# pyannote/pyannote-video

Hardware: AMD Instinct MI355X
Metric: frames/sec end-to-end detect->embed->cluster, 1080p@25fps (higher is better)
Workload: dtype f32 (detector scores, embedder) / f64 (tracker, clustering) / u8 frames; an f16 screening pass with a proven error bound decides which windows the detector's exact f32 chain is evaluated for -- results identical to dense f32 scoring (`dense_scoring`)

## Files before the change

### include/pvface.h

```cpp
#ifndef PVFACE_H
#define PVFACE_H
#include <stdint.h>
#include <stddef.h>

#ifdef __cplusplus
extern "C" {
#endif

typedef uint64_t pvf_handle;
typedef struct { int32_t left, top, right, bottom; } pvf_rect_i32;

const char* pvf_last_error(void);
int32_t pvf_version(void);
int32_t pvf_device_count(int32_t* n);
int32_t pvf_ctx_create(int32_t device, pvf_handle* ctx);
int32_t pvf_ctx_create_prio(int32_t device, int32_t priority_class, pvf_handle* ctx);
int32_t pvf_ctx_destroy(pvf_handle ctx);
int32_t pvf_sync(pvf_handle ctx);

int32_t pvf_load_detector(pvf_handle ctx, const char* path);
int32_t pvf_load_shape_predictor(pvf_handle ctx, const char* path);
int32_t pvf_load_embedder(pvf_handle ctx, const char* path);
int32_t pvf_model_tensor(const char* path, int32_t kind, const char* name, void* out, int64_t cap_bytes, int64_t* nbytes);
int32_t pvf_set_tracker_tables(pvf_handle ctx, const double* mask64, const double* mask_scale, const double* tw64,
                               const double* tw32, double alpha_pow_m16, double ln_alpha);

int32_t pvf_frame_upload(pvf_handle ctx, const uint8_t* rgb, int32_t h, int32_t w, int64_t row_stride_bytes, pvf_handle* frame);
int32_t pvf_frame_wrap_device(pvf_handle ctx, const void* dev_rgb, int32_t h, int32_t w, pvf_handle* frame);
int32_t pvf_frame_release(pvf_handle ctx, pvf_handle frame);
int32_t pvf_frame_release_many(pvf_handle ctx, const pvf_handle* frames, int32_t n);
int32_t pvf_frame_pool_trim(pvf_handle ctx, int64_t keep_bytes, int64_t* pooled_bytes);
int32_t pvf_mem_info(pvf_handle ctx, int64_t* free_bytes, int64_t* total_bytes);
int32_t pvf_frame_device_ptr(pvf_handle ctx, pvf_handle frame, const void** dev_rgb);

int32_t pvf_ingest_create(pvf_handle ctx, int32_t h, int32_t w, int32_t depth, pvf_handle* ring);
int32_t pvf_ingest_destroy(pvf_handle ctx, pvf_handle ring);
int32_t pvf_ingest_acquire(pvf_handle ctx, pvf_handle ring, int32_t* slot, uint8_t** host_rgb);
int32_t pvf_ingest_submit(pvf_handle ctx, pvf_handle ring, int32_t slot, pvf_handle* frame);
int32_t pvf_ingest_wait(pvf_handle ctx, pvf_handle ring);
#define PVF_YUV_BT709 1
#define PVF_YUV_FULL_RANGE 2
int32_t pvf_ingest_create_yuv(pvf_handle ctx, int32_t h, int32_t w, int32_t depth, int32_t layout, int32_t flags, pvf_handle* ring);
int32_t pvf_frame_from_yuv(pvf_handle ctx, const uint8_t* y, int64_t y_pitch, const uint8_t* u, const uint8_t* v, int64_t c_pitch,
                           int32_t c_step, int32_t h, int32_t w, int32_t layout, int32_t flags, pvf_handle* frame);
int32_t pvf_frame_resize(pvf_handle ctx, pvf_handle frame, int32_t out_w, int32_t out_h, pvf_handle* out);

#define PVF_PRIM_RECT 0
#define PVF_PRIM_LINE 1
#define PVF_PRIM_TEXT 2
#define PVF_RENDER_MAX_PRIMS 4096
#define PVF_RENDER_MAX_RUN 64
#define PVF_RENDER_MAX_TEXT (1 << 20)
#define PVF_RENDER_MAX_SCALE 64
#define PVF_RENDER_MAX_BATCH 1024
typedef struct { int32_t type, a, b, c, d; uint32_t colour; int32_t scale, reserved; } pvf_prim;
int32_t pvf_render_batch(pvf_handle ctx, const pvf_handle* frames, int32_t n, int32_t out_w, int32_t out_h, int32_t flags,
                         const int32_t* start, const pvf_prim* prims, const uint8_t* text, int64_t text_bytes,
                         uint8_t* out, int32_t out_on_device);
int32_t pvf_egress_create(pvf_handle ctx, int32_t out_w, int32_t out_h, int32_t depth, int32_t flags, pvf_handle* ring);
int32_t pvf_egress_destroy(pvf_handle ctx, pvf_handle ring);
int32_t pvf_egress_submit(pvf_handle ctx, pvf_handle ring, pvf_handle frame, const pvf_prim* prims, int32_t n_prims,
                          const uint8_t* text, int64_t text_bytes, int32_t* slot);
int32_t pvf_egress_wait(pvf_handle ctx, pvf_handle ring, int32_t slot, const uint8_t** host_planes);
int32_t pvf_egress_release(pvf_handle ctx, pvf_handle ring, int32_t slot);
int32_t pvf_debug_render_rgb(pvf_handle ctx, pvf_handle frame, int32_t out_w, int32_t out_h, const pvf_prim* prims, int32_t n_prims,
                             const uint8_t* text, int64_t text_bytes, uint8_t* rgb);

int32_t pvf_detect(pvf_handle ctx, pvf_handle frame, int32_t upsample, double adjust_threshold,
                   pvf_rect_i32* out, float* scores, int32_t cap, int32_t* n);
int32_t pvf_detect_batch(pvf_handle ctx, const pvf_handle* frames, int32_t n_frames, int32_t upsample,
                         double adjust_threshold, pvf_rect_i32* out, float* scores, int32_t* counts,
                         int32_t cap_per_frame);
int32_t pvf_detect_many(pvf_handle ctx, const pvf_handle* frames, int32_t n_frames, int32_t batch, int32_t upsample,
                        double adjust_threshold, pvf_rect_i32* out, float* scores, int32_t* counts, int32_t cap);

int32_t pvf_detector_screening(pvf_handle ctx, int32_t on, int32_t list_cap);
int32_t pvf_detector_screening_stats(pvf_handle ctx, int64_t* batches, int64_t* listed, int64_t* retries, double* bounds, double* pipe_err);

int32_t pvf_embedder_split(pvf_handle ctx, int32_t on);
int32_t pvf_embedder_split_stats(pvf_handle ctx, int64_t* faces, int64_t* reruns, double* pipe_err);

int32_t pvf_tracker_create(pvf_handle ctx, pvf_handle* trk);
int32_t pvf_tracker_create_many(pvf_handle ctx, int32_t n, pvf_handle* trks);
int32_t pvf_tracker_destroy_many(pvf_handle ctx, const pvf_handle* trks, int32_t n);
int32_t pvf_tracker_clone_many(pvf_handle ctx, const pvf_handle* src, int32_t n, pvf_handle* dst);
int32_t pvf_tracker_destroy(pvf_handle ctx, pvf_handle trk);
int32_t pvf_tracker_start(pvf_handle ctx, pvf_handle trk, pvf_handle frame, const double box[4]);
int32_t pvf_tracker_update(pvf_handle ctx, pvf_handle trk, pvf_handle frame, double* psr);
int32_t pvf_tracker_position(pvf_handle ctx, pvf_handle trk, double box[4]);
int32_t pvf_tracker_start_many(pvf_handle ctx, const pvf_handle* trks, const pvf_handle* frames,
                               const double* boxes , int32_t n);
int32_t pvf_tracker_update_many(pvf_handle ctx, const pvf_handle* trks, const pvf_handle* frames, int32_t n,
                                double* psr , double* boxes_out );
int32_t pvf_tracker_update_many_deferred(pvf_handle ctx, const pvf_handle* trks, const pvf_handle* frames, int32_t n,
                                         double* psr, double* boxes_out);
int32_t pvf_tracker_commit_many(pvf_handle ctx, const pvf_handle* trks, const pvf_handle* frames, int32_t n);

int32_t pvf_overlap_matrix(const double* a, int32_t na, const double* b, int32_t nb, double ratio, double* out);
int32_t pvf_associate(const double* trackers, int32_t n_trackers, const double* detections, int32_t n_detections,
                      double min_overlap_ratio, int32_t* det_of_tracker);
int32_t pvf_munkres(const double* cost, int32_t n, int32_t* row_to_col);

int32_t pvf_landmarks(pvf_handle ctx, const pvf_handle* frames, const pvf_rect_i32* boxes, int32_t n,
                      int32_t* pts );
int32_t pvf_embed(pvf_handle ctx, const pvf_handle* frames, const int32_t* pts , int32_t n,
                  float* out );
int32_t pvf_landmarks_embed(pvf_handle ctx, const pvf_handle* frames, const pvf_rect_i32* boxes, int32_t n,
                            int32_t* pts , float* out );
int32_t pvf_embed_chips(pvf_handle ctx, const uint8_t* chips, int32_t n, float* out );
int32_t pvf_face_chips(pvf_handle ctx, const pvf_handle* frames, const int32_t* pts, int32_t n, uint8_t* chips );

int32_t pvf_pair_mean_dist(pvf_handle ctx, const double* X, int32_t N, int32_t dim, const int32_t* row_start,
                           int32_t T, double* D);
int32_t pvf_pair_mean_dist_metric(pvf_handle ctx, const double* X, int32_t N, int32_t dim, const int32_t* row_start,
                                  int32_t T, int32_t metric, double* D);
int32_t pvf_lane_create(int32_t n_frames, const int32_t* det_counts , const double* det_boxes ,
                        int32_t direction, double min_confidence, double min_overlap_ratio, int32_t deferring, pvf_handle* lane);
int32_t pvf_lane_destroy(pvf_handle lane);
int32_t pvf_lane_feed_plan(pvf_handle lane, int32_t p0, int32_t n_p, const uint8_t* has_update, const uint64_t* handles, const double* psr,
                           const double* pos);
int32_t pvf_lane_advance(pvf_handle lane, const double* reply_psr, const double* reply_pos, int32_t n_reply, int32_t* request,
                         uint64_t* req_handles, int32_t* req_frames, int32_t cap, int32_t* n_req, int32_t* plan_from);
int32_t pvf_lane_take_dead(pvf_handle lane, uint64_t* out, int32_t cap, int32_t* n);
int32_t pvf_lane_edges(pvf_handle lane, int32_t* n_edges, int32_t* u_frame_kind, double* u_box, int32_t* v_frame_kind, double* v_box,
                       double* conf, int32_t cap);
int32_t pvf_shot_tracks(pvf_handle lane_forward, pvf_handle lane_backward, const double* times, int32_t n_frames, double max_gap,
                        int32_t* rows, int32_t cap, int32_t* n_rows, int32_t* track_start, int32_t track_cap, int32_t* n_tracks);
int32_t pvf_track_rows(const int32_t* boxes, int64_t n, int32_t det_width, int32_t det_height, int32_t width, int32_t height,
                       double* file_box, int32_t* pixel_box);
int32_t pvf_round_decimals(const double* in, int64_t n, int32_t decimals, double* out);

int32_t pvf_pair_mean_dist_rows(pvf_handle ctx, const double* X, int32_t N, int32_t dim, const int32_t* row_start, int32_t T,
                                int32_t track0, int32_t track1, double* D);
int32_t pvf_pair_upper_rows(pvf_handle ctx, const double* X, int32_t N, int32_t dim, const int32_t* row_start, int32_t T,
                            int32_t track0, int32_t track1, double* D);
int32_t pvf_cluster_dist(pvf_handle ctx, const double* D, const int32_t* row_start, int32_t T, double threshold,
                         int32_t* labels, double* merge_log, int32_t* n_merges);
int32_t pvf_cluster_upper(pvf_handle ctx, const double* U, int32_t on_device, const int32_t* row_start, int32_t T, double threshold,
                          int32_t* labels, double* merge_log, int32_t* n_merges);
int32_t pvf_cluster_tracks(pvf_handle ctx, const double* X, int32_t N, int32_t dim, const int32_t* row_start,
                           int32_t T, double threshold, int32_t* labels, double* merge_log, int32_t* n_merges);
int32_t pvf_cluster_tracks_f32(pvf_handle ctx, const float* emb, int64_t row_stride_bytes, int32_t n_src, int32_t emb_on_device,
                               const int32_t* order, int32_t N, int32_t decimals, const int32_t* row_start, int32_t T, int32_t metric,
                               double threshold, int32_t* labels, double* merge_log, int32_t* n_merges);
int32_t pvf_pair_upper_rows_f32(pvf_handle ctx, const float* emb, int64_t row_stride_bytes, int32_t n_src, int32_t emb_on_device,
                                const int32_t* order, int32_t N, int32_t decimals, const int32_t* row_start, int32_t T,
                                int32_t track0, int32_t track1, double* rows_out, int32_t out_on_device);

int32_t pvf_format_rows(const double* t, const int64_t* identifier, const double* values, int64_t n_rows, int32_t n_cols,
                        int32_t decimals, char* out, int64_t cap, int64_t* written);

int32_t pvf_round_rows(const float* x, int64_t n, int32_t decimals, double* out);

int32_t pvf_parse_rows(const char* text, int64_t len, double* out, int64_t cap, int64_t* n_rows, int32_t* n_cols);

int32_t pvf_prof_enable(pvf_handle ctx, int32_t on);
int32_t pvf_prof_reset(pvf_handle ctx);
int32_t pvf_prof_get(pvf_handle ctx, const char* family, double* total_ms, int64_t* launches);

int32_t pvf_debug_pyramid_level(pvf_handle ctx, pvf_handle frame, int32_t upsample, int32_t level,
                                uint8_t* out, int32_t* h, int32_t* w);
int32_t pvf_debug_pyramid_batch(pvf_handle ctx, const pvf_handle* frames, int32_t n, int32_t upsample);
int32_t pvf_debug_level_features(pvf_handle ctx, pvf_handle frame, int32_t upsample, int32_t level,
                                 float* out, int32_t* fh, int32_t* fw);
int32_t pvf_debug_level_plan(pvf_handle ctx, pvf_handle frame, int32_t upsample, int32_t level, int32_t* out8);
int32_t pvf_debug_fhog(pvf_handle ctx, const uint8_t* img, int32_t h, int32_t w, int32_t cell, int32_t pad_r,
                       int32_t pad_c, float* out, int32_t* fh, int32_t* fw);
int32_t pvf_debug_detect_raw(pvf_handle ctx, pvf_handle frame, int32_t upsample, double adjust, float* scores,
                             int32_t* meta , int32_t cap, int32_t* n);
int32_t pvf_debug_detect_raw_many(pvf_handle ctx, const pvf_handle* frames, int32_t n_frames, int32_t batch, int32_t upsample,
                                  double adjust, int32_t* counts, int32_t* rows, int64_t cap, int64_t* total);
int32_t pvf_debug_extract_chip(pvf_handle ctx, pvf_handle frame, const double rect[4], double cs, double sn,
                               int32_t rows, int32_t cols, uint8_t* out);
int32_t pvf_debug_tracker_state(pvf_handle ctx, pvf_handle trk, double* F, double* A, double* B);
int32_t pvf_debug_tracker_scale_state(pvf_handle ctx, pvf_handle trk, double* As, double* Bs);
int32_t pvf_debug_embed_stage(pvf_handle ctx, const uint8_t* chips, int32_t n, int32_t split, int32_t stage, float* out, int32_t dims[3],
                              int32_t* flags);
int32_t pvf_debug_conv(pvf_handle ctx, const int32_t geom[18], const float* in, const float* w, const float* bias, const float* gamma,
                       const float* beta, const float* skip, int32_t split, int32_t force_generic, float* out, int32_t* flags);
int32_t pvf_debug_embed_head(pvf_handle ctx, const float* x, int32_t n, int32_t hw, float* out);

int32_t pvf_shot_dfd(pvf_handle ctx, const pvf_handle* frames, int32_t n, int32_t width, int32_t height, const float* tables,
                     double* dfd, uint8_t* gray_out, float* flow_out);

int32_t pvf_orb_extract(pvf_handle ctx, const pvf_handle* frames, int32_t n, int32_t width, int32_t height, int32_t cap,
                        int32_t* counts, float* keypoints, uint8_t* descriptors);
int32_t pvf_orb_match_counts(pvf_handle ctx, const uint8_t* descriptors, const int32_t* rows, int32_t n_sets, int32_t cap,
                             const int32_t* pairs, int64_t n_pairs, int32_t* counts);

#ifdef __cplusplus
}
#endif
#endif
```

### pyannote-video_amd/csrc/api.hip

```cpp
#include "pvf_internal.h"
#include <algorithm>
#include <cmath>
#include <cstdlib>
#include <string>
#include <thread>

#define API_BEGIN try {
#define API_END                                                        \
    return 0;                                                          \
    }                                                                  \
    catch (const std::exception& e) { pvf_set_error(e.what()); return -1; } \
    catch (...) { pvf_set_error("unknown error"); return -2; }

#define ENTER(c, h)                                                \
    Ctx* c = pvf_ctx(h);                                           \
    std::lock_guard<std::recursive_mutex> _api_lock(c->api_mu);    \
    HIP_CHECK(hipSetDevice(c->device))
#define ENTER_DET(c, h)                                            \
    Ctx* c = pvf_ctx(h);                                           \
    std::lock_guard<std::recursive_mutex> _det_lock(c->det_mu);    \
    HIP_CHECK(hipSetDevice(c->device))
#define ENTER_BOTH(c, h)                                           \
    Ctx* c = pvf_ctx(h);                                           \
    std::lock_guard<std::recursive_mutex> _det_lock(c->det_mu);    \
// ... 47 lines not shown
extern "C" int32_t pvf_embedder_split(pvf_handle h, int32_t on)
{
    API_BEGIN
    ENTER(c, h);
    c->emb_split = on != 0;
    API_END
}

extern "C" int32_t pvf_embedder_split_stats(pvf_handle h, int64_t* faces, int64_t* reruns, double* pipe_err)
{
    API_BEGIN
    ENTER(c, h);
    if (faces) *faces = c->emb_split_faces;
    if (reruns) *reruns = c->emb_reruns;
    if (pipe_err) *pipe_err = c->emb_pipe_err;
    API_END
}

extern "C" int32_t pvf_detect_batch(pvf_handle h, const pvf_handle* frames, int32_t n_frames, int32_t upsample, double adjust,
                                    pvf_rect_i32* out, float* scores, int32_t* counts, int32_t cap)
{
    API_BEGIN
    ENTER_DET(c, h);
    PVF_REQUIRE(n_frames > 0 && frames && out && counts && cap > 0, "pvf_detect_batch: bad arguments");
    PVF_REQUIRE(upsample >= 0 && upsample <= 2, "pvf_detect_batch: upsample must be 0..2");
    std::vector<Frame> fr(n_frames);
    for (int i = 0; i < n_frames; ++i) fr[i] = c->frame(frames[i]);
    std::vector<std::vector<RawDet>> raw;
    with_candidate_room(c, [&]() { det_run_batch(c, fr, upsample, adjust, raw); });
    std::vector<RawDet> kept;
    for (int i = 0; i < n_frames; ++i) {
        det_nms(c->det, raw[i], kept);
        const int n = std::min<int>((int)kept.size(), cap);
        counts[i] = n;
        for (int k = 0; k < n; ++k) {
            out[(size_t)i * cap + k] = pvf_rect_i32{kept[k].l, kept[k].t, kept[k].rr, kept[k].b};
            if (scores) scores[(size_t)i * cap + k] = kept[k].score;
        }
    }
    API_END
}

extern "C" int32_t pvf_detect_many(pvf_handle h, const pvf_handle* frames, int32_t n_frames, int32_t batch, int32_t upsample, double adjust,
                                   pvf_rect_i32* out, float* scores, int32_t* counts, int32_t cap)
{
    API_BEGIN
    ENTER_DET(c, h);
    PVF_REQUIRE(n_frames > 0 && batch > 0 && frames && out && counts && cap > 0, "pvf_detect_many: bad arguments");
    PVF_REQUIRE(upsample >= 0 && upsample <= 2, "pvf_detect_many: upsample must be 0..2");
    std::vector<Frame> fr(n_frames);
    for (int i = 0; i < n_frames; ++i) fr[i] = c->frame(frames[i]);
    std::vector<std::vector<RawDet>> kept_all;
    with_candidate_room(c, [&]() { det_run_many(c, fr, batch, upsample, adjust, kept_all, true); });
    for (int i = 0; i < n_frames; ++i) {
        const std::vector<RawDet>& kept = kept_all[i];
        const int n = std::min<int>((int)kept.size(), cap);
        counts[i] = n;
        for (int k = 0; k < n; ++k) {
            out[(size_t)i * cap + k] = pvf_rect_i32{kept[k].l, kept[k].t, kept[k].rr, kept[k].b};
            if (scores) scores[(size_t)i * cap + k] = kept[k].score;
        }
    }
    API_END
}

extern "C" int32_t pvf_detect(pvf_handle h, pvf_handle frame, int32_t upsample, double adjust, pvf_rect_i32* out, float* scores,
                              int32_t cap, int32_t* n)
{
    int32_t cnt = 0;
    const int32_t rc = pvf_detect_batch(h, &frame, 1, upsample, adjust, out, scores, &cnt, cap);
    if (rc == 0 && n) *n = cnt;
    return rc;
}

extern "C" int32_t pvf_debug_detect_raw(pvf_handle h, pvf_handle frame, int32_t upsample, double adjust, float* scores, int32_t* meta,
                                        int32_t cap, int32_t* n)
{
    API_BEGIN
    ENTER_DET(c, h);
    std::vector<Frame> fr{c->frame(frame)};
    std::vector<std::vector<RawDet>> raw;
    with_candidate_room(c, [&]() { det_run_batch(c, fr, upsample, adjust, raw); });
    const int k = std::min<int>((int)raw[0].size(), cap);
    *n = (int)raw[0].size();
    for (int i = 0; i < k; ++i) {
        const RawDet& d = raw[0][i];
        scores[i] = d.score;
        int32_t* m = meta + (size_t)i * 8;
        m[0] = d.filter; m[1] = d.level; m[2] = d.r; m[3] = d.c; m[4] = d.l; m[5] = d.t; m[6] = d.rr; m[7] = d.b;
    }
    API_END
}

extern "C" int32_t pvf_debug_detect_raw_many(pvf_handle h, const pvf_handle* frames, int32_t n_frames, int32_t batch, int32_t upsample, double adjust,
                                             int32_t* counts, int32_t* rows, int64_t cap, int64_t* total)
{
    API_BEGIN
    ENTER_DET(c, h);
    PVF_REQUIRE(n_frames > 0 && batch > 0 && frames && counts && total && (rows || cap == 0), "pvf_debug_detect_raw_many: bad arguments");
    PVF_REQUIRE(upsample >= 0 && upsample <= 2, "pvf_debug_detect_raw_many: upsample must be 0..2");
    std::vector<Frame> fr(n_frames);
    for (int i = 0; i < n_frames; ++i) fr[i] = c->frame(frames[i]);
    std::vector<std::vector<RawDet>> raw;
    with_candidate_room(c, [&]() { det_run_many(c, fr, batch, upsample, adjust, raw, false); });
    int64_t k = 0;
    for (int i = 0; i < n_frames; ++i) {
        counts[i] = (int32_t)raw[i].size();
        for (const RawDet& d : raw[i]) {
            if (k < cap) {
                int32_t* m = rows + (size_t)k * 5;
                m[0] = d.level; m[1] = d.filter; m[2] = d.r; m[3] = d.c;
                memcpy(&m[4], &d.score, 4);
            }
            ++k;
        }
    }
    *total = k;
    API_END
}

extern "C" int32_t pvf_debug_pyramid_level(pvf_handle h, pvf_handle frame, int32_t upsample, int32_t level, uint8_t* out, int32_t* oh,
                                           int32_t* ow)
{
    API_BEGIN
    ENTER_DET(c, h);
    std::vector<uint8_t> buf;
    int hh = 0, ww = 0;
    det_pyramid_level(c, c->frame(frame), upsample, level, out ? &buf : nullptr, &hh, &ww);
    *oh = hh; *ow = ww;
    if (out) memcpy(out, buf.data(), buf.size());
    API_END
}

extern "C" int32_t pvf_debug_pyramid_batch(pvf_handle h, const pvf_handle* frames, int32_t n, int32_t upsample)
{
    API_BEGIN
    ENTER_DET(c, h);
    PVF_REQUIRE(frames && n > 0, "pvf_debug_pyramid_batch: bad arguments");
    std::vector<Frame> fr;
    for (int i = 0; i < n; ++i) fr.push_back(c->frame(frames[i]));
    det_pyramid_batch(c, fr, upsample);
    API_END
}

extern "C" int32_t pvf_debug_level_features(pvf_handle h, pvf_handle frame, int32_t upsample, int32_t level, float* out, int32_t* fh, int32_t* fw)
{
    API_BEGIN
    ENTER_DET(c, h);
    std::vector<float> buf;
    int a = 0, b = 0;
    det_level_features(c, c->frame(frame), upsample, level, out ? &buf : nullptr, &a, &b);
    *fh = a; *fw = b;
    if (out) memcpy(out, buf.data(), buf.size() * sizeof(float));
    API_END
}

extern "C" int32_t pvf_debug_level_plan(pvf_handle h, pvf_handle frame, int32_t upsample, int32_t level, int32_t* out8)
{
    API_BEGIN
    ENTER_DET(c, h);
    PVF_REQUIRE(out8 != nullptr, "pvf_debug_level_plan: out8 is NULL");
    det_level_plan(c, c->frame(frame), upsample, level, out8);
    API_END
}

extern "C" int32_t pvf_debug_fhog(pvf_handle h, const uint8_t* img, int32_t ih, int32_t iw, int32_t cell, int32_t pad_r, int32_t pad_c,
                                  float* out, int32_t* fh, int32_t* fw)
{
    API_BEGIN
    ENTER_BOTH(c, h);
    int a = 0, b = 0;
    if (!out) { fhog_dims(ih, iw, cell, pad_r, pad_c, &a, &b); *fh = a; *fw = b; return 0; }
    std::vector<float> buf;
    fhog_debug(c, img, ih, iw, cell, pad_r, pad_c, buf, &a, &b);
    *fh = a; *fw = b;
    memcpy(out, buf.data(), buf.size() * sizeof(float));
    API_END
}

static pvf_handle tracker_new(Ctx* c)
{
    std::unique_ptr<Tracker> t(new Tracker());
    const uint64_t id = c->next_id++;
    c->trackers[id] = std::move(t);
    return id;
}

extern "C" int32_t pvf_tracker_create(pvf_handle h, pvf_handle* trk)
{
    API_BEGIN
    ENTER(c, h);
    *trk = tracker_new(c);
    API_END
}

extern "C" int32_t pvf_tracker_create_many(pvf_handle h, int32_t n, pvf_handle* trks)
{
    API_BEGIN
    ENTER(c, h);
    PVF_REQUIRE(n >= 0, "negative count");
    for (int i = 0; i < n; ++i) trks[i] = tracker_new(c);
    API_END
}

extern "C" int32_t pvf_tracker_clone_many(pvf_handle h, const pvf_handle* src, int32_t n, pvf_handle* dst)
{
    API_BEGIN
    ENTER(c, h);
    PVF_REQUIRE(n >= 0, "negative count");
    std::vector<Tracker*> s(n), d(n);
    for (int i = 0; i < n; ++i) s[i] = &c->tracker(src[i]);
    for (int i = 0; i < n; ++i) { dst[i] = tracker_new(c); d[i] = &c->tracker(dst[i]); }
    dsst_clone_many(c, s, d);
    API_END
}

static const size_t TRACKER_POOL_KEEP = 4096;
static void pool_tracker_state(Ctx* c, Tracker& t)
{
    double* d_state = t.d_state;
    t.d_state = nullptr;
    if (t.share) {
        int* sh = t.share;
        t.share = nullptr;
        if (--*sh > 0) return;
        delete sh;
    }
    if (!d_state) return;
    if (c->tracker_pool.size() < TRACKER_POOL_KEEP) { c->tracker_pool.push_back(d_state); return; }
    HIP_CHECK(hipStreamSynchronize(c->stream));
    HIP_CHECK(hipFree(d_state));
}

extern "C" int32_t pvf_tracker_destroy_many(pvf_handle h, const pvf_handle* trks, int32_t n)
{
    API_BEGIN
    ENTER(c, h);
    for (int i = 0; i < n; ++i) {
        auto it = c->trackers.find(trks[i]);
        PVF_REQUIRE(it != c->trackers.end(), "unknown tracker handle");
        pool_tracker_state(c, *it->second);
        c->trackers.erase(it);
    }
    API_END
}

extern "C" int32_t pvf_tracker_destroy(pvf_handle h, pvf_handle trk)
{
    API_BEGIN
    ENTER(c, h);
    auto it = c->trackers.find(trk);
    PVF_REQUIRE(it != c->trackers.end(), "unknown tracker handle");
    pool_tracker_state(c, *it->second);
    c->trackers.erase(it);
    API_END
}
extern "C" int32_t pvf_tracker_start_many(pvf_handle h, const pvf_handle* trks, const pvf_handle* frames, const double* boxes, int32_t n)
{
    API_BEGIN
    ENTER(c, h);
    std::vector<Tracker*> t(n);
    std::vector<Frame> f(n);
    PVF_REQUIRE(n >= 0 && (n == 0 || (trks && frames && boxes)), "tracker.start_track: bad arguments");
    for (int i = 0; i < n; ++i) {
        const double* b = boxes + 4 * (size_t)i;
        PVF_REQUIRE(std::isfinite(b[0]) && std::isfinite(b[1]) && std::isfinite(b[2]) && std::isfinite(b[3]),
                    "tracker.start_track: box with a non-finite coordinate");
        PVF_REQUIRE(b[2] - b[0] != 0.0 && b[3] - b[1] != 0.0, "tracker.start_track: box of zero width or height");
    }
    for (int i = 0; i < n; ++i) { t[i] = &c->tracker(trks[i]); f[i] = c->frame(frames[i]); }
    dsst_start_many(c, t, f, boxes);
    API_END
}
extern "C" int32_t pvf_tracker_update_many(pvf_handle h, const pvf_handle* trks, const pvf_handle* frames, int32_t n, double* psr,
                                           double* boxes_out)
{
    API_BEGIN
    ENTER(c, h);
    std::vector<Tracker*> t(n);
    std::vector<Frame> f(n);
    for (int i = 0; i < n; ++i) { t[i] = &c->tracker(trks[i]); f[i] = c->frame(frames[i]); }
    dsst_update_many(c, t, f, psr, boxes_out);
    API_END
}
extern "C" int32_t pvf_tracker_start(pvf_handle h, pvf_handle trk, pvf_handle frame, const double box[4])
{
    return pvf_tracker_start_many(h, &trk, &frame, box, 1);
}
extern "C" int32_t pvf_tracker_update_many_deferred(pvf_handle h, const pvf_handle* trks, const pvf_handle* frames, int32_t n, double* psr,
                                                    double* boxes_out)
{
    API_BEGIN
    ENTER(c, h);
    std::vector<Tracker*> t(n);
    std::vector<Frame> f(n);
    for (int i = 0; i < n; ++i) { t[i] = &c->tracker(trks[i]); f[i] = c->frame(frames[i]); }
    dsst_update_many(c, t, f, psr, boxes_out, 1);
    API_END
}

extern "C" int32_t pvf_tracker_commit_many(pvf_handle h, const pvf_handle* trks, const pvf_handle* frames, int32_t n)
{
    API_BEGIN
    ENTER(c, h);
    std::vector<Tracker*> t(n);
    std::vector<Frame> f(n);
// ... 689 lines not shown
```

### pyannote-video_amd/csrc/ctx.hip

```cpp
#include "pvf_internal.h"
#include "detect_ml.h"
#include <cmath>
#include <fstream>
#include <mutex>
#include <dlfcn.h>

static thread_local std::string g_err;
void pvf_set_error(const char* msg) { g_err = msg ? msg : ""; }
extern "C" const char* pvf_last_error(void) { return g_err.c_str(); }

static std::mutex g_ctx_mu;
static std::unordered_map<uint64_t, std::unique_ptr<Ctx>> g_ctxs;
static uint64_t g_next_ctx = 0x1000;

Ctx* pvf_ctx(pvf_handle h)
{
    std::lock_guard<std::mutex> lk(g_ctx_mu);
    auto it = g_ctxs.find(h);
    if (it == g_ctxs.end()) throw PvfError("unknown context handle");
    return it->second.get();
}

std::map<std::string, Tensor> pvf_read_container(const char* path)
{
// ... 80 lines not shown
        d.d_bmfma4 = upload<float>(b4.data(), b4.size());
    }
    screen_prepare_model(d, w.f32());
    d.loaded = true;
}

static void load_shape(Ctx* c, const char* path)
{
    auto m = pvf_read_model(path, 1);
    const int32_t* q = need(m, "sp.meta").i32();
    ShapeModel& s = c->shape;
    s.n_cascades = q[0]; s.n_trees = q[1]; s.n_parts = q[2]; s.n_pix = q[3]; s.depth = q[4];
    PVF_REQUIRE(s.n_parts == 68, "shape predictor: 68 parts expected");
    PVF_REQUIRE(s.depth >= 1 && s.depth <= 6, "shape predictor: tree depth 1..6");
    PVF_REQUIRE(s.n_pix >= 1 && s.n_pix <= 1024, "shape predictor: 1..1024 feature pixels per cascade");
    PVF_REQUIRE(s.n_cascades >= 1 && s.n_trees >= 1, "shape predictor: no cascades / trees");
    {
        const size_t splits = (size_t)s.n_cascades * s.n_trees * (((size_t)1 << s.depth) - 1), leaves = (size_t)s.n_cascades * s.n_trees * ((size_t)1 << s.depth);
        PVF_REQUIRE(need(m, "sp.initial_shape").numel() == 136 && need(m, "sp.anchor_idx").numel() == (size_t)s.n_cascades * s.n_pix &&
                    need(m, "sp.deltas").numel() == (size_t)s.n_cascades * s.n_pix * 2 && need(m, "sp.split_idx1").numel() == splits &&
                    need(m, "sp.split_idx2").numel() == splits && need(m, "sp.split_thresh").numel() == splits &&
                    need(m, "sp.leaves").numel() == leaves * 136, "shape predictor: tensor sizes do not match sp.meta");
        const int32_t* a = need(m, "sp.anchor_idx").i32();
        for (size_t k = 0; k < (size_t)s.n_cascades * s.n_pix; ++k) PVF_REQUIRE(a[k] >= 0 && a[k] < s.n_parts, "shape predictor: anchor index out of range");
        const int32_t* i1 = need(m, "sp.split_idx1").i32();
        const int32_t* i2 = need(m, "sp.split_idx2").i32();
        for (size_t k = 0; k < splits; ++k)
            PVF_REQUIRE(i1[k] >= 0 && i1[k] < s.n_pix && i2[k] >= 0 && i2[k] < s.n_pix, "shape predictor: split feature index out of range");
    }
    auto up_f = [&](const char* k) { const Tensor& t = need(m, k); return upload<float>(t.f32(), t.numel()); };
    auto up_i = [&](const char* k) { const Tensor& t = need(m, k); return upload<int32_t>(t.i32(), t.numel()); };
    s.d_initial = up_f("sp.initial_shape");
    s.d_anchor = up_i("sp.anchor_idx");
    s.d_deltas = up_f("sp.deltas");
    s.d_idx1 = up_i("sp.split_idx1");
    s.d_idx2 = up_i("sp.split_idx2");
    s.d_thresh = up_f("sp.split_thresh");
    s.d_leaves = up_f("sp.leaves");
    s.loaded = true;
}

static const int UNITS[14][3] = {{32, 32, 0}, {32, 32, 0}, {32, 32, 0}, {32, 64, 1}, {64, 64, 0}, {64, 64, 0}, {64, 64, 0},
                                 {64, 128, 1}, {128, 128, 0}, {128, 128, 0}, {128, 256, 1}, {256, 256, 0}, {256, 256, 0}, {256, 256, 1}};

static void load_embedder(Ctx* c, const char* path)
{
    auto m = pvf_read_model(path, 2);
    EmbedModel& e = c->emb;
    e.chip_size = need(m, "emb.meta").i32()[0];
    e.chip_padding = need(m, "emb.padding").f64()[0];
    PVF_REQUIRE(e.chip_size == 150, "embedder: 150x150 chips expected");
    const Tensor& ms = need(m, "emb.mean_shape");
    PVF_REQUIRE(ms.numel() == 102, "emb.mean_shape must be 51x2");
    e.mean_shape.assign(ms.f32(), ms.f32() + 102);
    const Tensor& blob = need(m, "emb.blob");
    const float* p = blob.f32();
    const float* end = p + blob.numel();
    for (ConvLayer& L : e.convs) {
        if (L.d_frag) { (void)hipFree(L.d_frag); L.d_frag = nullptr; }
        if (L.d_wsplit) { (void)hipFree(L.d_wsplit); L.d_wsplit = nullptr; }
    }
    e.convs.clear();
    if (e.d_stem) { (void)hipFree(e.d_stem); e.d_stem = nullptr; }
    auto add_conv = [&](int cin, int cout, int k, int stride, int pad) {
        ConvLayer L{cin, cout, k, stride, pad, nullptr, nullptr, nullptr, nullptr, nullptr};
        const size_t nw = (size_t)cout * cin * k * k;
        PVF_REQUIRE(p + nw + 3 * (size_t)cout <= end, "emb.blob too short");
        conv_layer_upload(L, p, p + nw, p + nw + cout, p + nw + 2 * (size_t)cout);
        p += nw + 3 * (size_t)cout;
        e.convs.push_back(L);
    };
    add_conv(3, 32, 7, 2, 0);
    for (int u = 0; u < 14; ++u) {
        const int cin = UNITS[u][0], n = UNITS[u][1], down = UNITS[u][2];
        add_conv(cin, n, 3, down ? 2 : 1, down ? 0 : 1);
        add_conv(n, n, 3, 1, 1);
    }
    PVF_REQUIRE(p + 256 * 128 == end, "emb.blob size mismatch");
    e.d_fc = upload<float>(p, 256 * 128);
    e.loaded = true;
}

namespace {
struct Roctx {
    int (*push)(const char*) = nullptr;
    int (*pop)() = nullptr;
    Roctx()
    {
        const char* e = getenv("PVF_ROCTX");
        if (!e || strcmp(e, "1") != 0) return;
        void* h = dlopen("librocprofiler-sdk-roctx.so", RTLD_NOW | RTLD_GLOBAL);
        if (!h) h = dlopen("librocprofiler-sdk-roctx.so.1", RTLD_NOW | RTLD_GLOBAL);
        if (!h) h = dlopen("libroctx64.so", RTLD_NOW | RTLD_GLOBAL);
        if (!h) h = dlopen("libroctx64.so.4", RTLD_NOW | RTLD_GLOBAL);
        if (!h) return;
        push = reinterpret_cast<int (*)(const char*)>(dlsym(h, "roctxRangePushA"));
        pop = reinterpret_cast<int (*)()>(dlsym(h, "roctxRangePop"));
        if (!push || !pop) push = nullptr, pop = nullptr;
    }
};
const Roctx& roctx() { static const Roctx r; return r; }
}

ProfScope::ProfScope(Ctx* ctx, const char* family, hipStream_t on) : c(ctx), s(on ? on : ctx->stream)
{
    if (roctx().push) { roctx().push(family); ranged = true; }
    if (!c->prof_on) return;
    {
        std::lock_guard<std::mutex> lk(c->prof_mu);
        f = &c->prof[family];
        auto get = [&]() {
            hipEvent_t e;
            if (!c->event_pool.empty()) { e = c->event_pool.back(); c->event_pool.pop_back(); }
            else HIP_CHECK(hipEventCreate(&e));
            return e;
        };
        a = get(); b = get();
    }
    HIP_CHECK(hipEventRecord(a, s));
}
ProfScope::~ProfScope()
{
    if (ranged) roctx().pop();
    if (!f) return;
    (void)hipEventRecord(b, s);
    std::lock_guard<std::mutex> lk(c->prof_mu);
    f->pending.emplace_back(a, b);
    f->launches += 1;
}

static void prof_drain(Ctx* c)
{
    HIP_CHECK(hipStreamSynchronize(c->stream));
    HIP_CHECK(hipStreamSynchronize(c->det_stream));
    std::lock_guard<std::mutex> lk(c->prof_mu);
    for (auto& kv : c->prof) {
        for (auto& pr : kv.second.pending) {
            float ms = 0;
            if (hipEventElapsedTime(&ms, pr.first, pr.second) == hipSuccess) kv.second.total_ms += ms;
            c->event_pool.push_back(pr.first);
            c->event_pool.push_back(pr.second);
        }
        kv.second.pending.clear();
    }
}

#define API_BEGIN try {
#define API_END                                                        \
    return 0;                                                          \
    }                                                                  \
    catch (const std::exception& e) { pvf_set_error(e.what()); return -1; } \
    catch (...) { pvf_set_error("unknown error"); return -2; }

extern "C" int32_t pvf_version(void) { return 500; }

extern "C" int32_t pvf_device_count(int32_t* n)
{
    API_BEGIN
    int k = 0;
    hipError_t e = hipGetDeviceCount(&k);
    if (e != hipSuccess) k = 0;
    *n = k;
    API_END
}

extern "C" int32_t pvf_ctx_create_prio(int32_t device, int32_t priority_class, pvf_handle* out)
{
    API_BEGIN
    int k = 0;
    if (hipGetDeviceCount(&k) != hipSuccess || k <= 0) throw PvfError("no HIP device visible: libpvface has no CPU fallback");
    PVF_REQUIRE(device >= 0 && device < k, "device index out of range");
    HIP_CHECK(hipSetDevice(device));
    hipDeviceProp_t prop;
    HIP_CHECK(hipGetDeviceProperties(&prop, device));
    if (strncmp(prop.gcnArchName, "gfx950", 6) != 0)
        throw PvfError(std::string("libpvface is built for gfx950 (MI355X) only; device is ") + prop.gcnArchName);
    std::unique_ptr<Ctx> c(new Ctx());
    c->device = device;
    c->n_cu = prop.multiProcessorCount;
    {
        int lo = 0, hi = 0;
        HIP_CHECK(hipDeviceGetStreamPriorityRange(&lo, &hi));
        int prio = priority_class < 0 ? lo : hi;
        if (const char* e = getenv("PVF_MAIN_STREAM_PRIO")) prio = (strcmp(e, "low") == 0) ? lo : hi;
        HIP_CHECK(hipStreamCreateWithPriority(&c->stream, hipStreamNonBlocking, priority_class == 2 ? lo : prio));
        HIP_CHECK(hipStreamCreateWithPriority(&c->det_stream, hipStreamNonBlocking, priority_class == 2 ? hi : lo));
    }
    if (const char* e = getenv("PVF_DETECTOR_SCREENING")) c->det_screen = atoi(e) != 0;
    if (const char* e = getenv("PVF_EMBEDDER_SPLIT")) c->emb_split = atoi(e) != 0;
    std::lock_guard<std::mutex> lk(g_ctx_mu);
    uint64_t id = g_next_ctx++;
    g_ctxs[id] = std::move(c);
    *out = id;
    API_END
}

extern "C" int32_t pvf_ctx_create(int32_t device, pvf_handle* out) { return pvf_ctx_create_prio(device, 0, out); }

extern "C" int32_t pvf_ctx_destroy(pvf_handle h)
{
    API_BEGIN
    Ctx* c = pvf_ctx(h);
    HIP_CHECK(hipSetDevice(c->device));
    (void)hipStreamSynchronize(c->stream);
    (void)hipStreamSynchronize(c->det_stream);
    for (auto& kv : c->frames) if (kv.second.owned) (void)hipFree((void*)kv.second.d);
    for (auto& kv : c->trackers) {
        Tracker& t = *kv.second;
        if (t.share) { if (--*t.share > 0) continue; delete t.share; t.share = nullptr; }
        if (t.d_state) (void)hipFree(t.d_state);
    }
    for (auto p : c->tracker_pool) (void)hipFree(p);
    for (int k = 0; k < 2; ++k) if (c->det_ev[k]) (void)hipEventDestroy(c->det_ev[k]);
    ml_plans_free(c);
    ingest_free_all(c);
    render_free_all(c);
    for (auto& kv : c->frame_pool) for (auto q : kv.second) {
        if (q.free_after) (void)hipEventDestroy(q.free_after);
        if (q.free_after_det) (void)hipEventDestroy(q.free_after_det);
        (void)hipFree(q.p);
    }
    if (c->d_orient_lut) (void)hipFree(c->d_orient_lut);
    if (c->d_wrap_lut) (void)hipFree(c->d_wrap_lut);
    (void)hipStreamDestroy(c->stream);
    (void)hipStreamDestroy(c->det_stream);
    std::lock_guard<std::mutex> lk(g_ctx_mu);
    g_ctxs.erase(h);
    API_END
}

extern "C" int32_t pvf_sync(pvf_handle h)
{
    API_BEGIN
    Ctx* c = pvf_ctx(h);
    std::lock_guard<std::recursive_mutex> det_lock(c->det_mu);
    std::lock_guard<std::recursive_mutex> api_lock(c->api_mu);
    HIP_CHECK(hipStreamSynchronize(c->det_stream));
    HIP_CHECK(hipStreamSynchronize(c->stream));
    API_END
}

extern "C" int32_t pvf_load_detector(pvf_handle h, const char* path)
{
    API_BEGIN
    Ctx* c = pvf_ctx(h);
    std::lock_guard<std::recursive_mutex> det_lock(c->det_mu);
    std::lock_guard<std::recursive_mutex> api_lock(c->api_mu);
    HIP_CHECK(hipSetDevice(c->device));
    PVF_REQUIRE(path != nullptr, "pvf_load_detector: path is NULL (the Python layer passes the packaged default)");
    load_detector(c, path);
    API_END
}
extern "C" int32_t pvf_load_shape_predictor(pvf_handle h, const char* path)
{
    API_BEGIN
    Ctx* c = pvf_ctx(h);
    std::lock_guard<std::recursive_mutex> api_lock(c->api_mu);
    HIP_CHECK(hipSetDevice(c->device));
    PVF_REQUIRE(path != nullptr, "path is NULL");
    load_shape(c, path);
    API_END
}
extern "C" int32_t pvf_load_embedder(pvf_handle h, const char* path)
{
    API_BEGIN
    Ctx* c = pvf_ctx(h);
    std::lock_guard<std::recursive_mutex> api_lock(c->api_mu);
    HIP_CHECK(hipSetDevice(c->device));
    PVF_REQUIRE(path != nullptr, "path is NULL");
    load_embedder(c, path);
    API_END
}

extern "C" int32_t pvf_model_tensor(const char* path, int32_t kind, const char* name, void* out, int64_t cap_bytes, int64_t* nbytes)
{
    API_BEGIN
    PVF_REQUIRE(path && name && nbytes, "pvf_model_tensor: bad arguments");
    auto m = pvf_read_model(path, kind);
    const Tensor& t = need(m, name);
    *nbytes = (int64_t)t.data.size();
    if (out) {
        PVF_REQUIRE(cap_bytes >= (int64_t)t.data.size(), "pvf_model_tensor: buffer too small");
        memcpy(out, t.data.data(), t.data.size());
    }
    API_END
}

extern "C" int32_t pvf_set_tracker_tables(pvf_handle h, const double* mask64, const double* mask_scale, const double* tw64,
                                          const double* tw32, double alpha_pow_m16, double ln_alpha)
{
    API_BEGIN
    Ctx* c = pvf_ctx(h);
    std::lock_guard<std::recursive_mutex> api_lock(c->api_mu);
    HIP_CHECK(hipSetDevice(c->device));
    TrackerTables& t = c->ttab;
    if (!t.d_mask64) {
        HIP_CHECK(hipMalloc((void**)&t.d_mask64, 64 * 64 * 8));
        HIP_CHECK(hipMalloc((void**)&t.d_mask_scale, 32 * 8));
        HIP_CHECK(hipMalloc((void**)&t.d_tw64, 64 * 8));
        HIP_CHECK(hipMalloc((void**)&t.d_tw32, 32 * 8));
    }
    HIP_CHECK(hipMemcpy(t.d_mask64, mask64, 64 * 64 * 8, hipMemcpyHostToDevice));
    HIP_CHECK(hipMemcpy(t.d_mask_scale, mask_scale, 32 * 8, hipMemcpyHostToDevice));
    HIP_CHECK(hipMemcpy(t.d_tw64, tw64, 64 * 8, hipMemcpyHostToDevice));
    HIP_CHECK(hipMemcpy(t.d_tw32, tw32, 32 * 8, hipMemcpyHostToDevice));
    t.alpha_pow_m16 = alpha_pow_m16; t.ln_alpha = ln_alpha;
    t.set = true;
// ... 154 lines not shown
```

### pyannote-video_amd/csrc/detect.hip

```cpp
#include "detect_ml.h"
#include <algorithm>
#include <thread>
#include <cmath>
#include <cstdlib>

#define RESIZE_MAXS 22
struct RowTab { int32_t top, bottom; double tb, tb1, pad; };
struct ColTab { int32_t left, pad; double lr, lr1, pad2; };

template <int RS, int NSTRIP>
__global__ void __launch_bounds__(256) resize_rows_k(const uint8_t* const* __restrict__ in_ptrs, const uint8_t* __restrict__ in_base,
                                                     size_t in_stride, int in_rb, int ih, int iw, uint8_t* __restrict__ out,
                                                     size_t out_stride, int out_rb, int oh, int ow,
                                                     const RowTab* __restrict__ rows, const ColTab* __restrict__ cols)
{
    constexpr int MAXS = (RS == 16) ? RESIZE_MAXS : (RS * 5) / 4 + 3;
    __shared__ uint32_t s_rows[4][MAXS][64];
    __shared__ uint32_t s_out[4][64];
    const int lane = threadIdx.x & 63;
    const int wave = __builtin_amdgcn_readfirstlane(threadIdx.x >> 6);
    const int c0 = blockIdx.x * 256 + wave * 64;
    const int b = blockIdx.z;
    if (c0 >= ow) return;
    const int c = min(c0 + lane, ow - 1);
// ... 164 lines not shown
}

static void pyramid_up_dims(int ih, int iw, int* oh, int* ow)
{
    const double right = ((iw - 1) + 1.25) * 2.0;
    const double bottom = ((ih - 1) + 0.75) * 2.0;
    *ow = (int)std::floor(right + 0.5) + 1;
    *oh = (int)std::floor(bottom + 0.5) + 1;
}


static inline long iround(double v) { return (long)std::floor(v + 0.5); }
static void rect_down6(long r[4]) { const double ratio = (6 - 1.0) / 6; for (int i = 0; i < 4; ++i) r[i] = iround((r[i] - 0.3) * ratio + 0.3); }
static void rect_up6(long r[4]) { const double ratio = 6 / (6 - 1.0); for (int i = 0; i < 4; ++i) r[i] = iround((r[i] - 0.3) * ratio + 0.3); }
static void rect_down2i(long r[4])
{
    r[0] = iround(r[0] / 2.0 - 1.25); r[1] = iround(r[1] / 2.0 - 0.75);
    r[2] = iround(r[2] / 2.0 - 1.25); r[3] = iround(r[3] / 2.0 - 0.75);
}
static int detector_levels(int h, int w, const DetectorModel& m)
{
    long r[4] = {0, 0, w - 1, h - 1};
    int levels = 0;
    do { rect_down6(r); ++levels; } while ((r[2] - r[0] + 1) >= m.min_w && (r[3] - r[1] + 1) >= m.min_h && levels < m.max_levels);
    return levels;
}
static void fhog_to_image(long px, long py, int cell, int pad_r, int pad_c, long* ox, long* oy)
{
    long x = (px + 1 - (pad_c - 1) / 2) * cell + 1;
    long y = (py + 1 - (pad_r - 1) / 2) * cell + 1;
    x += (x >= 0) ? cell / 2 : -(cell / 2);
    y += (y >= 0) ? cell / 2 : -(cell / 2);
    *ox = x; *oy = y;
}

struct LevelDims { int h, w; };
static std::vector<LevelDims> level_schedule(int h, int w, int upsample, const DetectorModel& m, std::vector<LevelDims>* ups)
{
    int ch = h, cw = w;
    for (int u = 0; u < upsample; ++u) {
        int nh, nw;
        pyramid_up_dims(ch, cw, &nh, &nw);
        ch = nh; cw = nw;
        if (ups) ups->push_back({ch, cw});
    }
    const int levels = detector_levels(ch, cw, m);
    std::vector<LevelDims> out;
    out.push_back({ch, cw});
    for (int l = 1; l < levels; ++l) { ch = (5 * ch) / 6; cw = (5 * cw) / 6; out.push_back({ch, cw}); }
    return out;
}

static void upload_frame_ptrs(Ctx* c, const std::vector<Frame>& frames, const uint8_t*** d_ptrs)
{
    DevBuf& d = c->s_fptr[c->det_slot & 1];
    HostBuf& h = c->h_fptr[c->det_slot & 1];
    d.ensure(frames.size() * sizeof(void*));
    h.ensure(frames.size() * sizeof(void*));
    const uint8_t** hp = h.as<const uint8_t*>();
    for (size_t i = 0; i < frames.size(); ++i) hp[i] = frames[i].d;
    HIP_CHECK(hipMemcpyAsync(d.p, hp, frames.size() * sizeof(void*), hipMemcpyHostToDevice, c->det_stream));
    *d_ptrs = d.as<const uint8_t*>();
}


__device__ __forceinline__ int ml_block(const MlStarts& st) { return (int)blockIdx.x; }
static inline int ml_grid(int total) { return total; }

__device__ __forceinline__ int ml_level(const MlStarts& st, int g)
{
    int l = 0;
    while (l + 1 < st.nl && g >= st.b0[l + 1]) ++l;
    return l;
}

#define FUSED_OUT 61
__device__ __forceinline__ uint32_t from_next_lane(uint32_t v) { return (uint32_t)__builtin_amdgcn_update_dpp(0, (int)v, 0x130, 0xf, 0xf, true); }
__device__ __forceinline__ uint32_t from_prev_lane(uint32_t v) { return (uint32_t)__builtin_amdgcn_update_dpp(0, (int)v, 0x138, 0xf, 0xf, true); }

#define FS_PAIRS 4
#define FS_COLS 65
#define FS_SLOT_DW (8 * FS_COLS * 2)
#define FS_BINS_DW (2 * 18 * 64)
#define FS_FLAG_DW (4 * 64)
#define FS_LDS_BYTES (FS_PAIRS * (FS_BINS_DW + 2 * FS_SLOT_DW + FS_FLAG_DW) * 4)
static_assert(FS_COLS * 8 == 520, "the ring's column pitch is written into the instruction strings below");
typedef __attribute__((address_space(3))) uint32_t* lds_u32;
__device__ __forceinline__ uint32_t lds_addr(const void* p) { return (uint32_t)(uintptr_t)(lds_u32)p; }

__device__ __forceinline__ void ring_write(uint32_t data_at, uint32_t flag_at, const u32x2* v, uint32_t row1)
{
    asm volatile("ds_write_b64 %0, %2\n\tds_write_b64 %0, %3 offset:520\n\tds_write_b64 %0, %4 offset:1040\n\tds_write_b64 %0, %5 offset:1560\n\t"
                 "ds_write_b64 %0, %6 offset:2080\n\tds_write_b64 %0, %7 offset:2600\n\tds_write_b64 %0, %8 offset:3120\n\t"
                 "ds_write_b64 %0, %9 offset:3640\n\tds_write_b32 %1, %10"
                 :: "v"(data_at), "v"(flag_at), "v"(v[0]), "v"(v[1]), "v"(v[2]), "v"(v[3]), "v"(v[4]), "v"(v[5]), "v"(v[6]), "v"(v[7]), "v"(row1) : "memory");
}
__device__ __forceinline__ uint32_t ring_read(uint32_t data_at, uint32_t flag_at, u32x2* own, u32x2* nb)
{
    uint32_t ready;
    asm volatile("ds_read_b32 %0, %18\n\t"
                 "ds_read_b64 %1, %17\n\tds_read_b64 %9, %17 offset:8\n\tds_read_b64 %2, %17 offset:520\n\tds_read_b64 %10, %17 offset:528\n\t"
                 "ds_read_b64 %3, %17 offset:1040\n\tds_read_b64 %11, %17 offset:1048\n\tds_read_b64 %4, %17 offset:1560\n\tds_read_b64 %12, %17 offset:1568\n\t"
                 "ds_read_b64 %5, %17 offset:2080\n\tds_read_b64 %13, %17 offset:2088\n\tds_read_b64 %6, %17 offset:2600\n\tds_read_b64 %14, %17 offset:2608\n\t"
                 "ds_read_b64 %7, %17 offset:3120\n\tds_read_b64 %15, %17 offset:3128\n\tds_read_b64 %8, %17 offset:3640\n\tds_read_b64 %16, %17 offset:3648\n\t"
                 "s_waitcnt lgkmcnt(0)"
                 : "=&v"(ready), "=&v"(own[0]), "=&v"(own[1]), "=&v"(own[2]), "=&v"(own[3]), "=&v"(own[4]), "=&v"(own[5]), "=&v"(own[6]), "=&v"(own[7]),
                   "=&v"(nb[0]), "=&v"(nb[1]), "=&v"(nb[2]), "=&v"(nb[3]), "=&v"(nb[4]), "=&v"(nb[5]), "=&v"(nb[6]), "=&v"(nb[7])
                 : "v"(data_at), "v"(flag_at) : "memory");
    return ready;
}
__device__ __forceinline__ void flag_write(uint32_t flag_at, uint32_t v)
{
    asm volatile("ds_write_b32 %0, %1" :: "v"(flag_at), "v"(v) : "memory");
}

template <int A, int B> __device__ __forceinline__ uint32_t sub_into_upper(uint32_t acc, uint32_t x, uint32_t y);
#define PVF_SUBW1(A, B)                                                                                                                  \
    template <> __device__ __forceinline__ uint32_t sub_into_upper<A, B>(uint32_t acc, uint32_t x, uint32_t y)                           \
    {                                                                                                                                    \
        asm("v_sub_u32_sdwa %0, %1, %2 dst_sel:WORD_1 dst_unused:UNUSED_PRESERVE src0_sel:BYTE_" #A " src1_sel:BYTE_" #B "\n\ts_nop 0"   \
            : "+v"(acc) : "v"(x), "v"(y));                                                                                               \
        return acc;                                                                                                                      \
    }
PVF_SUBW1(0, 0) PVF_SUBW1(1, 1) PVF_SUBW1(2, 2) PVF_SUBW1(3, 3)
#undef PVF_SUBW1
typedef short s16x2 __attribute__((ext_vector_type(2)));

template <int P>
__device__ __forceinline__ u32x2 split_grad_px(const uint32_t* up, const uint32_t* ce, const uint32_t* dn, const __amdgpu_buffer_rsrc_t& lut_rs,
                                               bool valid)
{
    uint32_t pk[3];
    int cv[3];
#define PVF_CH(K)                                                                                                                         \
    {                                                                                                                                     \
        constexpr int IU = 4 + 3 * P + K, IL = 1 + 3 * P + K, IR = 7 + 3 * P + K;                                                         \
        const uint32_t cx = ((ce[IR >> 2] >> (8 * (IR & 3))) & 0xffu) - ((ce[IL >> 2] >> (8 * (IL & 3))) & 0xffu);                          \
        pk[K] = sub_into_upper<(IU & 3), (IU & 3)>(cx, dn[IU >> 2], up[IU >> 2]);                                                          \
        const s16x2 v = __builtin_bit_cast(s16x2, pk[K]);                                                                                 \
        cv[K] = __builtin_amdgcn_sdot2(v, v, 0, false);                                                                                   \
    }
    PVF_CH(0) PVF_CH(1) PVF_CH(2)
#undef PVF_CH
    const int bv = max(cv[0], max(cv[1], cv[2]));
    const uint32_t pb = (cv[0] == bv) ? pk[0] : ((cv[1] == bv) ? pk[1] : pk[2]);
    const uint32_t off = (pb & 7u) | ((pb >> 13) & 0xff8u) | ((pb << 9) & 0x3f000u);
    u32x2 r;
    r.y = (uint32_t)__builtin_amdgcn_raw_buffer_load_b8(lut_rs, off, 0, 0);
    const float m = sqrt_exact_small((float)bv);
    r.x = valid ? __float_as_uint(m) : 0u;
    return r;
}

__global__ void __launch_bounds__(512) __attribute__((amdgpu_waves_per_eu(4, 4)))
fhog_split_ml_k(MlStarts st, const LvDesc* __restrict__ lv, int B, const uint8_t* __restrict__ img_base, float* __restrict__ feat_base,
                const uint8_t* __restrict__ lutw, int oy, int ox)
{
    constexpr int RSRC_FLAGS = 0x00020000;
    extern __shared__ __attribute__((aligned(16))) uint32_t fs_lds[];
    const int lane = threadIdx.x & 63;
    const int wave = __builtin_amdgcn_readfirstlane(threadIdx.x >> 6);
    const int pair = wave & 3, role = wave >> 2;
    for (int i = threadIdx.x; i < FS_PAIRS * (2 * FS_SLOT_DW + FS_FLAG_DW); i += 512) fs_lds[FS_PAIRS * FS_BINS_DW + i] = 0u;
    __syncthreads();
    const int g = ml_block(st);
    if (g >= st.b0[st.nl]) return;
    const int l = ml_level(st, g);
    const LvDesc d = lv[l];
    const int task = (g - st.b0[l]) * FS_PAIRS + pair;
    if (task >= d.fused_tasks) return;
    const int sx = task % d.strips;
    const int t2 = task / d.strips;
    const int cy = t2 % d.chunks;
    const int b = t2 / d.chunks;
    const int y0 = cy * d.chunk_rows;
    const int R = min(d.chunk_rows, d.hog_nr - y0);
    const int g_first = y0 + 1, g_last = y0 + R + 3;
    const int y_begin = 8 * g_first - 12;
    const uint32_t ring_at = lds_addr(fs_lds + FS_PAIRS * FS_BINS_DW + pair * 2 * FS_SLOT_DW) + 8u * lane;
    uint32_t* const flags = fs_lds + FS_PAIRS * (FS_BINS_DW + 2 * FS_SLOT_DW) + pair * FS_FLAG_DW + lane;
    const uint32_t flag_at = lds_addr(flags);

    if (role == 0) {
        const int hx = FUSED_OUT * sx + 1 + lane;
        const int x_first = 8 * hx - 12;
        const uint8_t* im = img_base + d.img_off + (size_t)b * d.img_stride;
        const int rb = d.rb;
        unsigned xmask = 0;
#pragma unroll
        for (int p = 0; p < 8; ++p) if (x_first + p >= 1 && x_first + p < d.visible_nc) xmask |= 1u << p;
        const bool strip_inside = __builtin_amdgcn_ballot_w64(xmask != 0xffu) == 0;
        const int voff = 3 * x_first - 4, voff2 = voff + 16;
        const __amdgpu_buffer_rsrc_t lut_rs = __builtin_amdgcn_make_buffer_rsrc((void*)lutw, 0, 1 << 18, RSRC_FLAGS);
        uint32_t rw[4][8];
        auto load_row = [&](int yi, uint32_t* dst) {
            const int bytes = (yi >= 0 && yi < d.h) ? rb : 0;
            const int yc = min(max(yi, 0), d.h - 1);
            const __amdgpu_buffer_rsrc_t rs = __builtin_amdgcn_make_buffer_rsrc((void*)(im + (size_t)yc * rb), 0, bytes, RSRC_FLAGS);
            const u32x4 a = __builtin_amdgcn_raw_buffer_load_b128(rs, voff, 0, 0);
            const u32x4 c = __builtin_amdgcn_raw_buffer_load_b128(rs, voff2, 0, 0);
            dst[0] = a.x; dst[1] = a.y; dst[2] = a.z; dst[3] = a.w; dst[4] = c.x; dst[5] = c.y; dst[6] = c.z; dst[7] = c.w;
        };
#pragma unroll
        for (int q = 0; q < 4; ++q) load_row(y_begin - 1 + q, rw[q]);
        const int nrows = 8 * (g_last - g_first + 1);
        for (int k0 = 0; k0 < nrows; k0 += 4) {
#pragma unroll
            for (int i = 0; i < 4; ++i) {
                const int k = k0 + i, y = y_begin + k;
                const uint32_t* up = rw[i & 3];
                const uint32_t* ce = rw[(i + 1) & 3];
                const uint32_t* dn = rw[(i + 2) & 3];
                const int freed = (int)__hip_atomic_load(flags + 128 + 64 * (i & 1), __ATOMIC_RELAXED, __HIP_MEMORY_SCOPE_WORKGROUP);
                const bool ok = (y >= 1 && y < d.visible_nr);
                u32x2 mb[8];
                if (strip_inside && ok) {
                    mb[0] = split_grad_px<0>(up, ce, dn, lut_rs, true); mb[1] = split_grad_px<1>(up, ce, dn, lut_rs, true);
                    mb[2] = split_grad_px<2>(up, ce, dn, lut_rs, true); mb[3] = split_grad_px<3>(up, ce, dn, lut_rs, true);
                    mb[4] = split_grad_px<4>(up, ce, dn, lut_rs, true); mb[5] = split_grad_px<5>(up, ce, dn, lut_rs, true);
                    mb[6] = split_grad_px<6>(up, ce, dn, lut_rs, true); mb[7] = split_grad_px<7>(up, ce, dn, lut_rs, true);
                } else {
                    mb[0] = split_grad_px<0>(up, ce, dn, lut_rs, ok && (xmask & 1u));
                    mb[1] = split_grad_px<1>(up, ce, dn, lut_rs, ok && (xmask & 2u));
                    mb[2] = split_grad_px<2>(up, ce, dn, lut_rs, ok && (xmask & 4u));
                    mb[3] = split_grad_px<3>(up, ce, dn, lut_rs, ok && (xmask & 8u));
                    mb[4] = split_grad_px<4>(up, ce, dn, lut_rs, ok && (xmask & 16u));
                    mb[5] = split_grad_px<5>(up, ce, dn, lut_rs, ok && (xmask & 32u));
                    mb[6] = split_grad_px<6>(up, ce, dn, lut_rs, ok && (xmask & 64u));
                    mb[7] = split_grad_px<7>(up, ce, dn, lut_rs, ok && (xmask & 128u));
                }
                load_row(y + 3, rw[i & 3]);
                int fr = freed;
                while (fr < k - 1) {
                    __builtin_amdgcn_s_sleep(1);
                    fr = (int)__hip_atomic_load(flags + 128 + 64 * (i & 1), __ATOMIC_RELAXED, __HIP_MEMORY_SCOPE_WORKGROUP);
                }
                ring_write(ring_at + (i & 1) * 4 * FS_SLOT_DW, flag_at + 256 * (i & 1), mb, (uint32_t)(k + 1));
            }
        }
        return;
    }

    float* accE = reinterpret_cast<float*>(fs_lds) + pair * FS_BINS_DW + lane;
    float* accO = accE + 18 * 64;
#pragma unroll
    for (int k = 0; k < 18; ++k) { accE[64 * k] = 0.0f; accO[64 * k] = 0.0f; }
    float hprev[18];
    float e0 = 0.f, e1 = 0.f, e2 = 0.f;
#pragma unroll
    for (int k = 0; k < 18; ++k) hprev[k] = 0.f;
    int krow = 0;
    auto band = [&](int gb, float* accU, float* accL) {
#pragma unroll
        for (int i = 0; i < 8; ++i) {
            u32x2 own[8], nb[8];
            for (;;) {
                const int ready = (int)ring_read(ring_at + (i & 1) * 4 * FS_SLOT_DW, flag_at + 256 * (i & 1), own, nb);
                if (__builtin_amdgcn_readfirstlane(ready) > krow) break;
                __builtin_amdgcn_s_sleep(1);
            }
            ++krow;
            flag_write(flag_at + 512 + 256 * (i & 1), (uint32_t)krow);
            const float fy = ((float)i + 0.5f) / 8.0f;
#pragma unroll
            for (int j = 0; j < 16; ++j) {
                const int p = j & 7;
                const u32x2 v = (j < 8) ? own[p] : nb[p];
                const float mv = __uint_as_float(v.x);
                const int bv = (int)(v.y << 8);
                const float fx = ((float)p + 0.5f) / 8.0f;
                const float wx = (j < 8) ? fx : 1.0f - fx;
                float* const pl = reinterpret_cast<float*>(reinterpret_cast<char*>(accL) + bv);
                float* const pu = reinterpret_cast<float*>(reinterpret_cast<char*>(accU) + bv);
                const float vl = *pl, vu = *pu;
                *pl = vl + ((1.0f - fy) * wx) * mv;
                *pu = vu + (fy * wx) * mv;
            }
        }
        const int c = gb - 1;
        float e = 0.0f;
#pragma unroll
        for (int o = 0; o < 9; ++o) { const float s2 = accL[64 * o] + accL[64 * (o + 9)]; e = e + s2 * s2; }
        e2 = e1; e1 = e0; e0 = e;
        if (c >= y0 + 3) {
            float n[9];
            n[1] = e2; n[4] = e1; n[7] = e0;
            n[0] = __uint_as_float(from_prev_lane(__float_as_uint(e2))); n[2] = __uint_as_float(from_next_lane(__float_as_uint(e2)));
            n[3] = __uint_as_float(from_prev_lane(__float_as_uint(e1))); n[5] = __uint_as_float(from_next_lane(__float_as_uint(e1)));
            n[6] = __uint_as_float(from_prev_lane(__float_as_uint(e0))); n[8] = __uint_as_float(from_next_lane(__float_as_uint(e0)));
            const int x = FUSED_OUT * sx + lane - 1, yh = c - 3;
            if (lane >= 1 && lane <= FUSED_OUT && x < d.hog_nc) {
                float4* dst = reinterpret_cast<float4*>(feat_base + d.feat_off + (size_t)b * d.feat_stride + feat_at(yh + oy, 0, x + ox, d.fwp));
                const size_t step = (size_t)d.fwp;
                const float eps = 0.0001f;
                const float z1[4] = {n[4], n[1], n[3], n[0]}, z2[4] = {n[5], n[2], n[4], n[1]}, z3[4] = {n[7], n[4], n[6], n[3]}, z4[4] = {n[8], n[5], n[7], n[4]};
                float nn[4], nv[4], t[4] = {0.f, 0.f, 0.f, 0.f};
#pragma unroll
                for (int k = 0; k < 4; ++k) {
                    nn[k] = 0.2f * sqrtf((((z1[k] + z2[k]) + z3[k]) + z4[k]) + eps);
                    nv[k] = 0.1f / nn[k];
                }
                float o[20];
#pragma unroll
                for (int g = 0; g < 18; g += 3) {
                    float hh[3][4];
#pragma unroll
                    for (int j = 0; j < 3; ++j) {
#pragma unroll
                        for (int k = 0; k < 4; ++k) hh[j][k] = fminf(hprev[g + j], nn[k]) * nv[k];
                        o[g + j] = (hh[j][0] + hh[j][1]) + (hh[j][2] + hh[j][3]);
                    }
#pragma unroll
                    for (int k = 0; k < 4; ++k) t[k] = t[k] + ((hh[0][k] + hh[1][k]) + hh[2][k]);
                    if (g == 3) { *dst = make_float4(o[0], o[1], o[2], o[3]); dst += step; __builtin_amdgcn_sched_barrier(0); }
                    if (g == 6) { *dst = make_float4(o[4], o[5], o[6], o[7]); dst += step; __builtin_amdgcn_sched_barrier(0); }
                    if (g == 9) { *dst = make_float4(o[8], o[9], o[10], o[11]); dst += step; __builtin_amdgcn_sched_barrier(0); }
                    if (g == 15) { *dst = make_float4(o[12], o[13], o[14], o[15]); dst += step; __builtin_amdgcn_sched_barrier(0); }
                }
                float ci[9];
#pragma unroll
                for (int g = 0; g < 9; ++g) {
                    const float s2 = hprev[g] + hprev[g + 9];
                    float hh[4];
#pragma unroll
                    for (int k = 0; k < 4; ++k) hh[k] = fminf(s2, nn[k]) * nv[k];
                    ci[g] = (hh[0] + hh[1]) + (hh[2] + hh[3]);
                    if (g == 1) { *dst = make_float4(o[16], o[17], ci[0], ci[1]); dst += step; __builtin_amdgcn_sched_barrier(0); }
                    if (g == 5) { *dst = make_float4(ci[2], ci[3], ci[4], ci[5]); dst += step; __builtin_amdgcn_sched_barrier(0); }
                }
                const float tscale = (float)(2 * 0.2357);
#pragma unroll
                for (int k = 0; k < 4; ++k) t[k] = t[k] * tscale;
                *dst = make_float4(ci[6], ci[7], ci[8], t[0]); dst += step;
                *dst = make_float4(t[1], t[2], t[3], 0.0f);
            }
        }
#pragma unroll
        for (int k = 0; k < 18; ++k) { hprev[k] = accL[64 * k]; accL[64 * k] = 0.0f; }
    };
    for (int gb = g_first; gb <= g_last; ++gb) {
        if (gb & 1) band(gb, accO, accE);
        else band(gb, accE, accO);
    }
}

__global__ void __launch_bounds__(256) feat_ring_zero_k(MlStarts st, const LvDesc* __restrict__ lv, int B, float* __restrict__ feat_base, int oy, int ox)
{
    const int g = ml_block(st);
    if (g >= st.b0[st.nl]) return;
    const int l = ml_level(st, g);
    const LvDesc d = lv[l];
    const int local = g - st.b0[l];
    const int xb = local % d.feat_bx;
    const int py = (local / d.feat_bx) % d.fh;
    const int b = local / (d.feat_bx * d.fh);
    const int px = xb * 256 + threadIdx.x;
    if (px >= d.fwp) return;
    const int x = px - ox, y = py - oy;
    if (x >= 0 && y >= 0 && x < d.hog_nc && y < d.hog_nr) return;
    float4* dst = reinterpret_cast<float4*>(feat_base + d.feat_off + (size_t)b * d.feat_stride + feat_at(py, 0, px, d.fwp));
#pragma unroll
    for (int k = 0; k < 8; ++k) dst[(size_t)k * d.fwp] = make_float4(0.f, 0.f, 0.f, 0.f);
}

__global__ void __launch_bounds__(128) __attribute__((amdgpu_waves_per_eu(2, 2)))
score_roll_k(MlStarts st, const LvDesc* __restrict__ lv, int B, const float* __restrict__ feat_base,
             const float4* __restrict__ Bg4, ScoreParams sp, int* __restrict__ counts, CandRec* __restrict__ cands)
{
    constexpr int FR = 10, FC = 10, NK = 12, PITCH = 31, MT = 2, WCOLS = MT * 48, SEG = WCOLS + 11, R = 5;
    constexpr int LAST_STEPS = 93 - 8 * (NK - 1);
    constexpr int NSTW = (SEG * 8 + 127) / 128;
    constexpr int SLAB = (SEG * PITCH + 3) / 4 * 4;
    constexpr int RSRC_FLAGS = 0x00020000;
    extern __shared__ __attribute__((aligned(16))) float s_seg[];
    const int lane = threadIdx.x & 63;
    const int wave = __builtin_amdgcn_readfirstlane(threadIdx.x >> 6);
    const int g = (int)blockIdx.x;
    if (g >= st.b0[st.nl]) return;
    const int l = ml_level(st, g);
    const LvDesc d = lv[l];
    const int local = g - st.b0[l];
    const int bx = local % d.score_bx;
    const int sg = (local / d.score_bx) % d.roll_nseg;
    const int b = __builtin_amdgcn_readfirstlane(local / (d.score_bx * d.roll_nseg));
    const int fw = d.fw;
    const int c_base = bx * WCOLS;
    const int c1 = fw - (FC - FC / 2 - 1);
    const int r_base = sg * d.roll_rows;
    const int out_rows = min(d.roll_rows, d.fh - (FR - 1) - r_base);
    const int fh = out_rows + FR - 1;
    const int fwp = d.fwp;
    const float* fb = feat_base + d.feat_off + (size_t)b * d.feat_stride + feat_at(r_base, 0, c_base, fwp);
    const int seg_cells = (fw - c_base < SEG) ? fw - c_base : SEG;
    const int i = lane & 15, kq = lane >> 4;
    const int lane16 = lane * 16;
    const bool two_tiles = (c_base + 48 + FC / 2 < c1);
    const __amdgpu_buffer_rsrc_t brs = __builtin_amdgcn_make_buffer_rsrc((void*)Bg4, 0, FR * NK * 2 * 64 * 16, RSRC_FLAGS);
    f32x4 acc[R][MT];
#pragma unroll
    for (int q = 0; q < R; ++q)
#pragma unroll
        for (int tt = 0; tt < MT; ++tt) acc[q][tt] = (f32x4){0.f, 0.f, 0.f, 0.f};
    constexpr int NH = 4;
    static_assert(NSTW <= 8 && SEG <= 128, "one cell per thread");
    u32x4 sv[NH];
    const int tid16 = (int)threadIdx.x * 16;
    auto load_part = [&](int fr, int half) {
        const int bytes = (fr < fh) ? seg_cells * 16 : 0;
#pragma unroll
        for (int u = 0; u < NH; ++u) {
            const __amdgpu_buffer_rsrc_t rs = __builtin_amdgcn_make_buffer_rsrc((void*)(fb + ((size_t)fr * 8 + half * NH + u) * fwp * 4), 0, bytes, RSRC_FLAGS);
            sv[u] = __builtin_amdgcn_raw_buffer_load_b128(rs, tid16, 0, 0);
        }
    };
    auto fill_part = [&](float* seg, int half) {
        if ((int)threadIdx.x < SEG) {
#pragma unroll
            for (int u = 0; u < NH; ++u) {
                const int q = half * NH + u;
                uint32_t* dd = reinterpret_cast<uint32_t*>(seg + (int)threadIdx.x * PITCH + 4 * q);
                dd[0] = sv[u].x; dd[1] = sv[u].y; dd[2] = sv[u].z;
                if (q != 7) dd[3] = sv[u].w;
            }
        }
    };
    auto emit = [&](int r_out, const f32x4 (&a)[MT]) {
        const int jc = lane & 15;
        if (jc < 15) {
            const int sft = jc / 5, f = jc % 5;
            const float th = sp.thresh[f];
            const int r = r_base + r_out + FR / 2;
#pragma unroll
            for (int tt = 0; tt < MT; ++tt)
#pragma unroll
                for (int reg = 0; reg < 4; ++reg) {
                    const int pos = 4 * (lane >> 4) + reg;
                    const int cc = c_base + tt * 48 + 3 * pos + sft + FC / 2;
                    const float v = a[tt][reg];
                    if (cc < c1 && v >= th && (tt == 0 || two_tiles)) {
                        const int idx = atomicAdd(&counts[b], 1);
                        if (idx < sp.cap) {
                            CandRec rec;
                            rec.score = v - th; rec.filter = f; rec.level = l; rec.r = r; rec.c = cc;
                            cands[(size_t)b * sp.cap + idx] = rec;
                        }
                    }
                }
        }
    };
    load_part(0, 0); fill_part(s_seg, 0);
    load_part(0, 1); fill_part(s_seg, 1);
    __syncthreads();
    for (int s = 0; s < fh; ++s) {
        const float* seg = s_seg + (s & 1) * SLAB;
        float* nxt = s_seg + ((s + 1) & 1) * SLAB;
        load_part(s + 1, 0);
        const int p = (s - wave) & 1;
        const int r0 = s - p;
        bool on[R];
        bool all_on = two_tiles, any_on = false;
#pragma unroll
        for (int q = 0; q < R; ++q) {
            const int r = r0 - 2 * q;
            on[q] = (r >= 0 && r < out_rows);
            all_on = all_on && on[q];
            any_on = any_on || on[q];
        }
        if (any_on) {
            const int bop = p * NK * 2048;
            const float* a0 = seg + (3 * i) * PITCH + kq;
            u32x4 bn[R][2];
            float an[8 * MT];
#pragma unroll
            for (int q = 0; q < R; ++q) {
                bn[q][0] = __builtin_amdgcn_raw_buffer_load_b128(brs, lane16, bop + 2 * q * NK * 2048, 0);
                bn[q][1] = __builtin_amdgcn_raw_buffer_load_b128(brs, lane16, bop + 2 * q * NK * 2048 + 1024, 0);
            }
#pragma unroll
            for (int pq = 0; pq < 8; ++pq)
#pragma unroll
                for (int tt = 0; tt < MT; ++tt) an[pq * MT + tt] = a0[(tt * 48) * PITCH + 4 * pq];
#pragma unroll
            for (int n = 0; n < NK; ++n) {
                float ac[8 * MT];
                float bc[R][8];
#pragma unroll
                for (int x = 0; x < 8 * MT; ++x) ac[x] = an[x];
#pragma unroll
                for (int q = 0; q < R; ++q)
#pragma unroll
                    for (int h = 0; h < 2; ++h) {
                        const uint32_t b0 = bn[q][h].x, b1 = bn[q][h].y, b2 = bn[q][h].z, b3 = bn[q][h].w;
                        bc[q][4 * h] = __uint_as_float(b0); bc[q][4 * h + 1] = __uint_as_float(b1);
                        bc[q][4 * h + 2] = __uint_as_float(b2); bc[q][4 * h + 3] = __uint_as_float(b3);
                    }
                if (n + 1 < NK) {
#pragma unroll
                    for (int q = 0; q < R; ++q) {
                        bn[q][0] = __builtin_amdgcn_raw_buffer_load_b128(brs, lane16, bop + (2 * q * NK + n + 1) * 2048, 0);
                        bn[q][1] = __builtin_amdgcn_raw_buffer_load_b128(brs, lane16, bop + (2 * q * NK + n + 1) * 2048 + 1024, 0);
                    }
#pragma unroll
                    for (int pq = 0; pq < 8; ++pq)
#pragma unroll
                        for (int tt = 0; tt < MT; ++tt) an[pq * MT + tt] = a0[(tt * 48) * PITCH + 32 * (n + 1) + 4 * pq];
                }
                if (n == NK / 2) { fill_part(nxt, 0); load_part(s + 1, 1); }
                __builtin_amdgcn_sched_barrier(0);
                const int steps = (n == NK - 1) ? LAST_STEPS : 8;
                if (all_on) {
#pragma unroll
                    for (int pq = 0; pq < steps; ++pq)
#pragma unroll
                        for (int q = 0; q < R; ++q)
#pragma unroll
                            for (int tt = 0; tt < MT; ++tt)
                                acc[q][tt] = __builtin_amdgcn_mfma_f32_16x16x4f32(ac[pq * MT + tt], bc[q][pq], acc[q][tt], 0, 0, 0);
                } else {
#pragma unroll
                    for (int q = 0; q < R; ++q) {
                        if (!on[q]) continue;
                        if (two_tiles) {
#pragma unroll
                            for (int pq = 0; pq < steps; ++pq)
#pragma unroll
                                for (int tt = 0; tt < MT; ++tt)
                                    acc[q][tt] = __builtin_amdgcn_mfma_f32_16x16x4f32(ac[pq * MT + tt], bc[q][pq], acc[q][tt], 0, 0, 0);
                        } else {
#pragma unroll
                            for (int pq = 0; pq < steps; ++pq)
                                acc[q][0] = __builtin_amdgcn_mfma_f32_16x16x4f32(ac[pq * MT], bc[q][pq], acc[q][0], 0, 0, 0);
                        }
                    }
                }
                __builtin_amdgcn_sched_barrier(0);
            }
        }
        else { fill_part(nxt, 0); load_part(s + 1, 1); }
        if (p == 1) {
            if (on[R - 1]) emit(r0 - 2 * (R - 1), acc[R - 1]);
#pragma unroll
            for (int q = R - 1; q > 0; --q)
#pragma unroll
                for (int tt = 0; tt < MT; ++tt) acc[q][tt] = acc[q - 1][tt];
#pragma unroll
            for (int tt = 0; tt < MT; ++tt) acc[0][tt] = (f32x4){0.f, 0.f, 0.f, 0.f};
        }
        fill_part(nxt, 1);
        __syncthreads();
    }
}

struct MlPlan {
    int h = 0, w = 0, upsample = -1, B = 0;
    std::vector<LvDesc> lv;
    std::vector<LevelDims> ups;
    MlStarts feat, fused, walk;
    int feat_blocks = 0, fused_blocks = 0, walk_blocks = 0;
    size_t img_bytes = 0, feat_floats = 0, up_bytes = 0;
    LvDesc* d_lv = nullptr;
    RowTab* d_rowtab = nullptr;
    ColTab* d_coltab = nullptr;
    std::vector<size_t> up_tab, lv_tab;
    std::vector<size_t> up_ctab, lv_ctab;
    const void* ring_valid_for = nullptr;
    ScreenPlan screen;
    bool screen_built = false;
    ~MlPlan() { if (d_lv) (void)hipFree(d_lv); if (d_rowtab) (void)hipFree(d_rowtab); if (d_coltab) (void)hipFree(d_coltab); }
    MlPlan() = default;
    MlPlan(const MlPlan&) = delete;
    MlPlan& operator=(const MlPlan&) = delete;
};

struct MlPlanCache {
    std::map<std::vector<int>, std::unique_ptr<MlPlan>> plans;
    int dpp_probe = -1;
    int sqrt_probe = -1;
};
void ml_plans_free(Ctx* c)
{
    delete c->ml_plans;
    c->ml_plans = nullptr;
}

static MlPlan* ml_plan(Ctx* c, int h, int w, int upsample, int B)
{
    if (!c->ml_plans) c->ml_plans = new MlPlanCache();
    const std::vector<int> key{h, w, upsample, B};
    auto it = c->ml_plans->plans.find(key);
    if (it != c->ml_plans->plans.end()) return it->second.get();
    const DetectorModel& m = c->det;
    std::unique_ptr<MlPlan> pp(new MlPlan());
    MlPlan& p = *pp;
    p.h = h; p.w = w; p.upsample = upsample; p.B = B;
    std::vector<LevelDims> dims = level_schedule(h, w, upsample, m, &p.ups);
    PVF_REQUIRE((int)dims.size() <= ML_MAX, "too many pyramid levels");
    auto al = [](size_t v, size_t a) { return (v + a - 1) / a * a; };
    for (size_t u = 0; u + 1 < p.ups.size(); ++u) p.up_bytes = std::max(p.up_bytes, (size_t)p.ups[u].h * al((size_t)p.ups[u].w * 3, 64) * B);
    p.feat.nl = p.fused.nl = p.walk.nl = (int)dims.size();
    int chunk_big = 8;
    for (int cand : {160, 128, 96, 64, 48, 32, 24, 16}) {
        long long tasks = 0;
        for (const LevelDims& ld : dims) {
            const int hog_nr = (int)((double)ld.h / 8.0 + 0.5) - 2, hog_nc = (int)((double)ld.w / 8.0 + 0.5) - 2;
            if (hog_nr > 0 && hog_nc > 0) tasks += (long long)((hog_nc + FUSED_OUT - 1) / FUSED_OUT) * std::max(2, (hog_nr + cand - 1) / cand) * B;
        }
        if (tasks >= 2LL * c->n_cu * 2 * 4) { chunk_big = cand; break; }
    }
    if (getenv("PVF_FHOG_CHUNK") && atoi(getenv("PVF_FHOG_CHUNK")) > 0) chunk_big = atoi(getenv("PVF_FHOG_CHUNK"));
    for (size_t l = 0; l < dims.size(); ++l) {
        LvDesc d;
        memset(&d, 0, sizeof d);
        d.h = dims[l].h; d.w = dims[l].w;
        d.cells_nr = (int)((double)d.h / 8.0 + 0.5); d.cells_nc = (int)((double)d.w / 8.0 + 0.5);
        d.visible_nr = std::min(d.cells_nr * 8, d.h) - 1; d.visible_nc = std::min(d.cells_nc * 8, d.w) - 1;
        d.hog_nr = d.cells_nr - 2; d.hog_nc = d.cells_nc - 2;
        const bool feat_ok = d.hog_nr > 0 && d.hog_nc > 0;
        d.fh = feat_ok ? d.hog_nr + m.frows - 1 : 0; d.fw = feat_ok ? d.hog_nc + m.fcols - 1 : 0;
        d.valid_score = (d.fh >= m.frows && d.fw >= m.fcols) ? 1 : 0;
        d.rb = (int)al((size_t)d.w * 3, 64);
        d.img_off = (long long)p.img_bytes; d.img_stride = (long long)d.h * d.rb;
        p.img_bytes += (size_t)d.img_stride * B;
        d.fwp = feat_ok ? d.fw + FEAT_PAD_COLS : 0;
        d.feat_off = (long long)p.feat_floats; d.feat_stride = (long long)d.fh * d.fwp * PVF_FHOG_STRIDE;
        p.feat_floats += (size_t)d.feat_stride * B;
        d.feat_bx = feat_ok ? (d.fwp + 255) / 256 : 0;
        const int out_c = d.fw - 9;
        d.score_bx = d.valid_score ? (out_c + 95) / 96 : 0;
        d.strips = feat_ok ? (d.hog_nc + FUSED_OUT - 1) / FUSED_OUT : 0;
        {
            const int nch = std::max(2, (d.hog_nr + chunk_big - 1) / chunk_big);
            d.chunk_rows = std::max((d.hog_nr + nch - 1) / nch, 1);
        }
        d.chunks = feat_ok ? (d.hog_nr + d.chunk_rows - 1) / d.chunk_rows : 0;
        d.fused_tasks = d.strips * d.chunks * B;
        p.feat.b0[l] = p.feat_blocks; p.feat_blocks += d.feat_bx * d.fh * B;
        p.fused.b0[l] = p.fused_blocks; p.fused_blocks += (d.fused_tasks + 3) / 4;
        p.lv.push_back(d);
    }
    const int nl = (int)dims.size();
    {
        long long total = 0;
        for (const LvDesc& d : p.lv) if (d.valid_score) total += (long long)d.score_bx * (d.fh - 9 + 9) * B;
        const int slots = 4 * 256;
        int roll_max = (int)std::max<long long>(64, total / slots / 2);
        if (getenv("PVF_SCORE_SEG")) roll_max = std::max(2, atoi(getenv("PVF_SCORE_SEG")));
        for (int l = 0; l < nl; ++l) {
            LvDesc& d = p.lv[l];
            const int out_r = d.fh - 9;
            d.roll_nseg = d.valid_score ? (out_r + roll_max - 1) / roll_max : 0;
            d.roll_rows = d.valid_score ? ((out_r + d.roll_nseg - 1) / d.roll_nseg + 1) / 2 * 2 : 0;
            if (d.valid_score) d.roll_nseg = (out_r + d.roll_rows - 1) / d.roll_rows;
            p.walk.b0[l] = p.walk_blocks; p.walk_blocks += d.score_bx * d.roll_nseg * B;
        }
    }
    p.feat.b0[nl] = p.feat_blocks; p.walk.b0[nl] = p.walk_blocks;
    p.fused.b0[nl] = p.fused_blocks;
    HIP_CHECK(hipMalloc((void**)&p.d_lv, sizeof(LvDesc) * nl));
    HIP_CHECK(hipMemcpy(p.d_lv, p.lv.data(), sizeof(LvDesc) * nl, hipMemcpyHostToDevice));
    {
        std::vector<RowTab> tab;
        int ch = h;
        for (size_t u = 0; u < p.ups.size(); ++u) { p.up_tab.push_back(tab.size()); fill_row_table(tab, ch, p.ups[u].h); ch = p.ups[u].h; }
        p.lv_tab.push_back(0);
        for (int l = 1; l < nl; ++l) { p.lv_tab.push_back(tab.size()); fill_row_table(tab, p.lv[l - 1].h, p.lv[l].h); }
        HIP_CHECK(hipMalloc((void**)&p.d_rowtab, sizeof(RowTab) * std::max<size_t>(tab.size(), 1)));
        if (!tab.empty()) HIP_CHECK(hipMemcpy(p.d_rowtab, tab.data(), sizeof(RowTab) * tab.size(), hipMemcpyHostToDevice));
        std::vector<ColTab> ctab;
        int cw2 = w;
        for (size_t u = 0; u < p.ups.size(); ++u) { p.up_ctab.push_back(ctab.size()); fill_col_table(ctab, cw2, p.ups[u].w); cw2 = p.ups[u].w; }
        p.lv_ctab.push_back(0);
        for (int l = 1; l < nl; ++l) { p.lv_ctab.push_back(ctab.size()); fill_col_table(ctab, p.lv[l - 1].w, p.lv[l].w); }
        HIP_CHECK(hipMalloc((void**)&p.d_coltab, sizeof(ColTab) * std::max<size_t>(ctab.size(), 1)));
        if (!ctab.empty()) HIP_CHECK(hipMemcpy(p.d_coltab, ctab.data(), sizeof(ColTab) * ctab.size(), hipMemcpyHostToDevice));
    }
    MlPlan* raw = pp.get();
    c->ml_plans->plans[key] = std::move(pp);
    return raw;
}

static MlPlan* ml_build_pyramid(Ctx* c, const std::vector<Frame>& frames, int upsample)
{
    const int B = (int)frames.size();
    const int h = frames[0].h, w = frames[0].w;
    for (auto& f : frames) PVF_REQUIRE(f.h == h && f.w == w, "batched frames must share one size");
    MlPlan* p = ml_plan(c, h, w, upsample, B);
    c->s_pyr.ensure(p->img_bytes + p->up_bytes + 256);
    uint8_t* base = c->s_pyr.as<uint8_t>();
    uint8_t* up_tmp = base + ((p->img_bytes + 63) / 64) * 64;
    const uint8_t** d_ptrs = nullptr;
    upload_frame_ptrs(c, frames, &d_ptrs);
    ProfScope ps(c, "pyramid", c->det_stream);
    auto al = [](size_t v, size_t a) { return (v + a - 1) / a * a; };
    const uint8_t* cur = nullptr;
    int ch = h, cw = w, crb = w * 3;
    size_t cstride = 0;
    for (size_t u = 0; u < p->ups.size(); ++u) {
        const bool last = (u + 1 == p->ups.size());
        uint8_t* dst = last ? base + p->lv[0].img_off : up_tmp;
        const int drb = (int)al((size_t)p->ups[u].w * 3, 64);
        const size_t dstride = (size_t)p->ups[u].h * drb;
        launch_resize_rows(c, cur ? nullptr : d_ptrs, cur, cstride, crb, ch, cw, dst, dstride, drb, p->ups[u].h, p->ups[u].w, B, p->d_rowtab + p->up_tab[u], p->d_coltab + p->up_ctab[u]);
        cur = dst; cstride = dstride; crb = drb; ch = p->ups[u].h; cw = p->ups[u].w;
    }
    if (!cur) {
        for (int b = 0; b < B; ++b)
            HIP_CHECK(hipMemcpy2DAsync(base + p->lv[0].img_off + (size_t)b * p->lv[0].img_stride, (size_t)p->lv[0].rb, frames[b].d, (size_t)w * 3,
                                       (size_t)w * 3, (size_t)h, hipMemcpyDeviceToDevice, c->det_stream));
    }
    for (size_t l = 1; l < p->lv.size(); ++l)
        launch_resize_rows(c, nullptr, base + p->lv[l - 1].img_off, (size_t)p->lv[l - 1].img_stride, p->lv[l - 1].rb, p->lv[l - 1].h, p->lv[l - 1].w,
                           base + p->lv[l].img_off, (size_t)p->lv[l].img_stride, p->lv[l].rb, p->lv[l].h, p->lv[l].w, B, p->d_rowtab + p->lv_tab[l], p->d_coltab + p->lv_ctab[l]);
    return p;
}

__global__ void dpp_probe_k(int* out)
{
    const int lane = threadIdx.x;
    out[lane] = (int)from_next_lane((uint32_t)(lane + 100));
    out[64 + lane] = (int)from_prev_lane((uint32_t)(lane + 100));
}
#define SQRT_PROBE_N (2 * 255 * 255 + 1)
__global__ void sqrt_probe_k(float* out)
{
    const int i = blockIdx.x * blockDim.x + threadIdx.x;
    if (i < SQRT_PROBE_N) out[i] = sqrt_exact_small((float)i);
}
static void check_dpp_direction(Ctx* c)
{
    MlPlanCache* pc = c->ml_plans;
    if (pc->dpp_probe < 0) {
        int* d = nullptr;
        HIP_CHECK(hipMalloc((void**)&d, 128 * sizeof(int) + SQRT_PROBE_N * sizeof(float)));
        float* ds = reinterpret_cast<float*>(d + 128);
        hipLaunchKernelGGL(dpp_probe_k, dim3(1), dim3(64), 0, c->det_stream, d);
        hipLaunchKernelGGL(sqrt_probe_k, dim3((SQRT_PROBE_N + 255) / 256), dim3(256), 0, c->det_stream, ds);
        int h[128];
        std::vector<float> hs(SQRT_PROBE_N);
        HIP_CHECK(hipMemcpyAsync(h, d, sizeof h, hipMemcpyDeviceToHost, c->det_stream));
        HIP_CHECK(hipMemcpyAsync(hs.data(), ds, SQRT_PROBE_N * sizeof(float), hipMemcpyDeviceToHost, c->det_stream));
        HIP_CHECK(hipStreamSynchronize(c->det_stream));
        (void)hipFree(d);
        bool ok = true;
        for (int i = 0; i < 64; ++i) {
            ok = ok && h[i] == (i < 63 ? i + 101 : 0);
            ok = ok && h[64 + i] == (i > 0 ? i + 99 : 0);
        }
        pc->dpp_probe = ok ? 1 : 0;
        bool sq = true;
        for (int i = 0; i < SQRT_PROBE_N; ++i) sq = sq && hs[i] == (float)std::sqrt((double)i);
        pc->sqrt_probe = sq ? 1 : 0;
    }
    PVF_REQUIRE(pc->dpp_probe == 1, "v_mov_b32_dpp wave_shl / wave_shr do not move data as the FHOG kernel expects on this device");
    PVF_REQUIRE(pc->sqrt_probe == 1, "v_sqrt_f32 is not within one step below the correctly rounded root on this device: the FHOG kernel's one-sided correction does not hold");
}

static MlPlan* ml_features(Ctx* c, const std::vector<Frame>& frames, int upsample)
{
    const DetectorModel& m = c->det;
    const int B = (int)frames.size();
    MlPlan* p = ml_build_pyramid(c, frames, upsample);
    const int oy = (m.frows - 1) / 2, ox = (m.fcols - 1) / 2;
    const void* feat_before = c->s_feat.p;
    c->s_feat.ensure(p->feat_floats * sizeof(float) + 64);
    if (p->fused_blocks == 0) return p;
    check_dpp_direction(c);
    ProfScope ps(c, "fhog", c->det_stream);
    if (c->s_feat.p != feat_before || c->feat_ring_owner != (const void*)p) {
        hipLaunchKernelGGL(feat_ring_zero_k, dim3(ml_grid(p->feat_blocks)), dim3(256), 0, c->det_stream, p->feat, p->d_lv, B, c->s_feat.as<float>(), oy, ox);
        c->feat_ring_owner = (const void*)p;
    }
    static std::atomic<uint64_t> attr_set{0};
    const uint64_t bit = 1ull << (c->device & 63);
    if (!(attr_set.load() & bit)) {
        HIP_CHECK(hipFuncSetAttribute(reinterpret_cast<const void*>(fhog_split_ml_k), hipFuncAttributeMaxDynamicSharedMemorySize, FS_LDS_BYTES));
        attr_set.fetch_or(bit);
    }
    hipLaunchKernelGGL(fhog_split_ml_k, dim3(ml_grid(p->fused_blocks)), dim3(512), FS_LDS_BYTES, c->det_stream, p->fused, p->d_lv, B,
                       c->s_pyr.as<uint8_t>(), c->s_feat.as<float>(), orientation_lut_wrapped(c), oy, ox);
    return p;
}

static void det_run_batch_ml(Ctx* c, const std::vector<Frame>& frames, int upsample, const ScoreParams& sp0, int* d_counts, CandRec* d_cands)
{
    const DetectorModel& m = c->det;
    const int B = (int)frames.size();
    MlPlan* p = ml_features(c, frames, upsample);
    if (p->walk_blocks == 0) return;
    if (c->det_screen && !c->det_screen_suspended) {
        if (!p->screen_built) { screen_plan_build(p->screen, p->lv, B); p->screen_built = true; }
        if (p->screen.usable) {
            ProfScope ps(c, "score_screened", c->det_stream);
            screen_launch(c, p->screen, p->d_lv, B, c->s_feat.as<float>(), sp0, d_counts, d_cands, d_counts + B);
            ++c->screen_batches;
            return;
        }
    }
    ProfScope ps(c, "score", c->det_stream);
    const size_t lds = (size_t)2 * (((2 * 48 + 11) * 31 + 3) / 4 * 4) * sizeof(float);
    const float4* b4 = reinterpret_cast<const float4*>(m.d_bmfma4);
    hipLaunchKernelGGL(score_roll_k, dim3(p->walk_blocks), dim3(128), lds, c->det_stream, p->walk, p->d_lv, B, c->s_feat.as<float>(), b4, sp0, d_counts, d_cands);
}

void det_pyramid_level(Ctx* c, const Frame& f, int upsample, int level, std::vector<uint8_t>* out, int* oh, int* ow)
{
    PVF_REQUIRE(c->det.loaded, "detector not loaded");
    std::vector<Frame> fr{f};
    MlPlan* p = ml_build_pyramid(c, fr, upsample);
    PVF_REQUIRE(level >= 0 && level < (int)p->lv.size(), "pyramid level out of range");
    *oh = p->lv[level].h; *ow = p->lv[level].w;
    if (out) {
        out->resize((size_t)(*oh) * (*ow) * 3);
        HIP_CHECK(hipMemcpy2DAsync(out->data(), (size_t)(*ow) * 3, c->s_pyr.as<uint8_t>() + p->lv[level].img_off, (size_t)p->lv[level].rb,
                                   (size_t)(*ow) * 3, (size_t)(*oh), hipMemcpyDeviceToHost, c->det_stream));
    }
    HIP_CHECK(hipStreamSynchronize(c->det_stream));
}

void det_pyramid_batch(Ctx* c, const std::vector<Frame>& frames, int upsample)
{
    PVF_REQUIRE(c->det.loaded, "detector not loaded");
    PVF_REQUIRE(!frames.empty(), "pyramid batch: no frames");
    (void)ml_build_pyramid(c, frames, upsample);
    HIP_CHECK(hipStreamSynchronize(c->det_stream));
}

void det_level_features(Ctx* c, const Frame& f, int upsample, int level, std::vector<float>* out, int* fh, int* fw)
{
    PVF_REQUIRE(c->det.loaded, "detector not loaded");
    std::vector<Frame> fr{f};
    MlPlan* p = ml_features(c, fr, upsample);
    PVF_REQUIRE(level >= 0 && level < (int)p->lv.size(), "pyramid level out of range");
    const LvDesc& d = p->lv[level];
    *fh = d.fh; *fw = d.fw;
    if (out) {
        out->resize((size_t)d.fh * d.fw * PVF_FHOG_STRIDE);
        std::vector<float> dev((size_t)d.feat_stride);
        if (!dev.empty())
            HIP_CHECK(hipMemcpyAsync(dev.data(), c->s_feat.as<float>() + d.feat_off, dev.size() * sizeof(float), hipMemcpyDeviceToHost, c->det_stream));
        HIP_CHECK(hipStreamSynchronize(c->det_stream));
        for (int y = 0; y < d.fh; ++y)
            for (int j = 0; j < 8; ++j)
                for (int x = 0; x < d.fw; ++x)
                    memcpy(out->data() + ((size_t)y * d.fw + x) * PVF_FHOG_STRIDE + 4 * j, dev.data() + feat_at(y, j, x, d.fwp), 4 * sizeof(float));
    }
    HIP_CHECK(hipStreamSynchronize(c->det_stream));
}

void det_level_plan(Ctx* c, const Frame& f, int upsample, int level, int32_t out[8])
{
    PVF_REQUIRE(c->det.loaded, "detector not loaded");
    MlPlan* p = ml_plan(c, f.h, f.w, upsample, 1);
    PVF_REQUIRE(level >= 0 && level < (int)p->lv.size(), "pyramid level out of range");
    const LvDesc& d = p->lv[level];
    const int32_t v[8] = {d.h, d.w, d.hog_nr, d.hog_nc, d.chunk_rows, d.chunks, d.roll_rows, d.roll_nseg};
    memcpy(out, v, sizeof v);
}

static bool raw_less(const RawDet& x, const RawDet& y)
{
    if (x.score != y.score) return x.score > y.score;
    if (x.filter != y.filter) return x.filter < y.filter;
    if (x.level != y.level) return x.level < y.level;
    if (x.r != y.r) return x.r < y.r;
    return x.c < y.c;
}

static void decode_candidates(const DetectorModel& m, int upsample, const CandRec* q, int n, std::vector<RawDet>& v);

static void screen_verdict(Ctx* c, const int* ctl)
{
    if (!c->det_screen || c->det_screen_suspended) return;
    c->screen_listed += std::min(ctl[SCR_FLAGGED], c->screen_list_cap);
    if (ctl[SCR_FLAGGED] > c->screen_list_cap || ctl[SCR_VIOLATION] != 0) {
        HIP_CHECK(hipStreamSynchronize(c->det_stream));
        throw ScreenRetry();
    }
}

void det_run_batch(Ctx* c, const std::vector<Frame>& frames, int upsample, double adjust, std::vector<std::vector<RawDet>>& raw_sorted)
{
    const DetectorModel& m = c->det;
    PVF_REQUIRE(m.loaded, "detector not loaded");
    PVF_REQUIRE(!frames.empty(), "no frames");
    const int B = (int)frames.size();
    const int cap = c->det_cand_cap;
    const size_t cnt_bytes = (((size_t)(B + SCR_CTL_INTS) * sizeof(int) + 63) / 64) * 64;
    c->s_cand.ensure((size_t)B * cap * sizeof(CandRec) + cnt_bytes + 64);
    int* d_counts = c->s_cand.as<int>();
    CandRec* d_cands = reinterpret_cast<CandRec*>(c->s_cand.as<uint8_t>() + cnt_bytes);
    HIP_CHECK(hipMemsetAsync(d_counts, 0, (size_t)(B + SCR_CTL_INTS) * sizeof(int), c->det_stream));
    ScoreParams sp;
    for (int f = 0; f < 8; ++f) sp.thresh[f] = f < m.n_filters ? (float)((double)m.thresh[f] + adjust) : 3.0e38f;
    sp.n_filters = m.n_filters; sp.cap = cap;
    det_run_batch_ml(c, frames, upsample, sp, d_counts, d_cands);
    HIP_CHECK(hipGetLastError());
    c->h_cand.ensure((size_t)B * cap * sizeof(CandRec) + cnt_bytes + 64);
    int* h_counts = c->h_cand.as<int>();
    CandRec* h_cands = reinterpret_cast<CandRec*>(c->h_cand.as<uint8_t>() + cnt_bytes);
    HIP_CHECK(hipMemcpyAsync(h_counts, d_counts, (size_t)(B + SCR_CTL_INTS) * sizeof(int), hipMemcpyDeviceToHost, c->det_stream));
    HIP_CHECK(hipStreamSynchronize(c->det_stream));
    screen_verdict(c, h_counts + B);
    raw_sorted.assign(B, {});
    for (int b = 0; b < B; ++b) {
        const int n = h_counts[b];
        if (n > cap) throw CandOverflow(n);
        if (n == 0) continue;
        HIP_CHECK(hipMemcpyAsync(h_cands + (size_t)b * cap, d_cands + (size_t)b * cap, (size_t)n * sizeof(CandRec), hipMemcpyDeviceToHost,
                                 c->det_stream));
    }
    HIP_CHECK(hipStreamSynchronize(c->det_stream));
    for (int b = 0; b < B; ++b) decode_candidates(m, upsample, h_cands + (size_t)b * cap, h_counts[b], raw_sorted[b]);
}

static const int DET_PREFETCH = 512;

static void decode_candidates(const DetectorModel& m, int upsample, const CandRec* q, int n, std::vector<RawDet>& v)
{
    const int bw = m.fcols - 2 * m.padding, bh = m.frows - 2 * m.padding;
    v.resize(n);
    for (int i = 0; i < n; ++i) {
        long rect[4];
        const long cl = q[i].c - bw / 2, ct = q[i].r - bh / 2;
        fhog_to_image(cl, ct, m.cell, m.frows, m.fcols, &rect[0], &rect[1]);
        fhog_to_image(cl + bw - 1, ct + bh - 1, m.cell, m.frows, m.fcols, &rect[2], &rect[3]);
        for (int k = 0; k < q[i].level; ++k) rect_up6(rect);
        for (int u = 0; u < upsample; ++u) rect_down2i(rect);
        v[i] = RawDet{q[i].score, q[i].filter, q[i].level, q[i].r, q[i].c, (int32_t)rect[0], (int32_t)rect[1], (int32_t)rect[2], (int32_t)rect[3]};
    }
    std::sort(v.begin(), v.end(), raw_less);
}

void det_run_many(Ctx* c, const std::vector<Frame>& frames, int batch, int upsample, double adjust,
                  std::vector<std::vector<RawDet>>& raw_sorted, bool nms)
{
    const DetectorModel& m = c->det;
    PVF_REQUIRE(m.loaded, "detector not loaded");
    PVF_REQUIRE(!frames.empty() && batch > 0, "no frames");
    const int N = (int)frames.size();
    raw_sorted.assign(N, {});
    {
        const int nb = (N + batch - 1) / batch;
        batch = (N + nb - 1) / nb;
    }
    const int cap = c->det_cand_cap, PF = DET_PREFETCH;
    ScoreParams sp;
    for (int f = 0; f < 8; ++f) sp.thresh[f] = f < m.n_filters ? (float)((double)m.thresh[f] + adjust) : 3.0e38f;
    sp.n_filters = m.n_filters; sp.cap = cap;
    const size_t cnt_bytes = (((size_t)(batch + SCR_CTL_INTS) * sizeof(int) + 63) / 64) * 64;
    for (int k = 0; k < 2; ++k) {
        c->s_cand2[k].ensure(cnt_bytes + (size_t)batch * cap * sizeof(CandRec));
        c->h_cand2[k].ensure(cnt_bytes + (size_t)batch * PF * sizeof(CandRec));
        if (!c->det_ev[k]) HIP_CHECK(hipEventCreateWithFlags(&c->det_ev[k], hipEventDisableTiming));
    }
    auto submit = [&](int o, int slot) {
        std::vector<Frame> fr(frames.begin() + o, frames.begin() + std::min(N, o + batch));
        const int B = (int)fr.size();
        int* d_counts = c->s_cand2[slot].as<int>();
        CandRec* d_cands = reinterpret_cast<CandRec*>(c->s_cand2[slot].as<uint8_t>() + cnt_bytes);
        HIP_CHECK(hipMemsetAsync(d_counts, 0, (size_t)(B + SCR_CTL_INTS) * sizeof(int), c->det_stream));
        c->det_slot = slot;
        det_run_batch_ml(c, fr, upsample, sp, d_counts, d_cands);
        HIP_CHECK(hipGetLastError());
        uint8_t* hb = c->h_cand2[slot].as<uint8_t>();
        HIP_CHECK(hipMemcpyAsync(hb, d_counts, (size_t)(B + SCR_CTL_INTS) * sizeof(int), hipMemcpyDeviceToHost, c->det_stream));
        HIP_CHECK(hipMemcpy2DAsync(hb + cnt_bytes, (size_t)PF * sizeof(CandRec), d_cands, (size_t)cap * sizeof(CandRec),
                                   (size_t)PF * sizeof(CandRec), (size_t)B, hipMemcpyDeviceToHost, c->det_stream));
        HIP_CHECK(hipEventRecord(c->det_ev[slot], c->det_stream));
    };
    auto collect = [&](int o, int slot) {
        const int B = std::min(N, o + batch) - o;
        HIP_CHECK(hipEventSynchronize(c->det_ev[slot]));
        const uint8_t* hb = c->h_cand2[slot].as<uint8_t>();
        const int* h_counts = reinterpret_cast<const int*>(hb);
        const CandRec* h_cands = reinterpret_cast<const CandRec*>(hb + cnt_bytes);
        const CandRec* d_cands = reinterpret_cast<const CandRec*>(c->s_cand2[slot].as<uint8_t>() + cnt_bytes);
        screen_verdict(c, h_counts + B);
        for (int b = 0; b < B; ++b)
            if (h_counts[b] > cap) {
                HIP_CHECK(hipStreamSynchronize(c->det_stream));
                throw CandOverflow(h_counts[b]);
            }
        std::vector<std::vector<CandRec>> big(B);
        bool any_big = false;
        for (int b = 0; b < B; ++b)
            if (h_counts[b] > PF) {
                big[b].resize(h_counts[b]);
                HIP_CHECK(hipMemcpyAsync(big[b].data(), d_cands + (size_t)b * cap, (size_t)h_counts[b] * sizeof(CandRec), hipMemcpyDeviceToHost, c->det_stream));
                any_big = true;
            }
        if (any_big) HIP_CHECK(hipStreamSynchronize(c->det_stream));
        auto frames_of = [&](int b0, int b1) {
            std::vector<RawDet> sorted_raw;
            for (int b = b0; b < b1; ++b) {
                const int n = h_counts[b];
                std::vector<RawDet>& dst = nms ? sorted_raw : raw_sorted[o + b];
                decode_candidates(m, upsample, n <= PF ? h_cands + (size_t)b * PF : big[b].data(), n, dst);
// ... 43 lines not shown
```

### pyannote-video_amd/csrc/detect_ml.h

```cpp
#pragma once
#include "pvf_internal.h"
#include "fhog_dev.h"

#define ML_MAX 32
struct LvDesc {
    int h, w, rb;
    int cells_nr, cells_nc, visible_nr, visible_nc;
    int fh, fw, hog_nr, hog_nc;
    int fwp;
    int feat_bx, score_bx;
    int valid_score;
    int roll_nseg, roll_rows;
    int strips, chunks, chunk_rows, fused_tasks;
    long long img_off, img_stride;
    long long feat_off, feat_stride;
};
struct MlStarts { int nl; int b0[ML_MAX + 1]; };

#define FEAT_PAD_COLS 52
__host__ __device__ __forceinline__ size_t feat_at(int row, int j, int col, int fwp) { return (((size_t)row * 8 + j) * fwp + col) * 4; }

struct ScoreParams { float thresh[8]; int n_filters; int level; int cap; };
struct CandRec { float score; int32_t filter, level, r, c; };

#define SCR_SG 4
#define SCR_GROUP_COLS 48
#define SCR_TAIL_CELLS 9
#define SCR_FILTER_COLS 10
static_assert((SCR_GROUP_COLS - 1) + SCR_TAIL_CELLS - (SCR_FILTER_COLS - 1) <= FEAT_PAD_COLS,
              "FEAT_PAD_COLS: the screening pass's tail read leaves a feature row's zero columns");
struct ScreenItem { int32_t lv, b, c_base, r_base, out_rows, ng; };
enum { SCR_CURSOR = 0, SCR_FLAGGED = 1, SCR_VIOLATION = 2, SCR_CTL_INTS = 4 };

struct ScreenPlan {
    ScreenItem* d_items = nullptr;
    int n_items = 0;
    bool usable = false;
    ~ScreenPlan() { if (d_items) (void)hipFree(d_items); }
    ScreenPlan() = default;
    ScreenPlan(const ScreenPlan&) = delete;
    ScreenPlan& operator=(const ScreenPlan&) = delete;
};
void screen_plan_build(ScreenPlan& sp, const std::vector<LvDesc>& lv, int B);
void screen_launch(Ctx* c, const ScreenPlan& sp, const LvDesc* d_lv, int B, const float* feat, const ScoreParams& thr, int* d_counts,
                   CandRec* d_cands, int* ctl);
void screen_prepare_model(DetectorModel& d, const float* w);
```

### pyannote-video_amd/csrc/pvf_internal.h

```cpp
#pragma once
#include <hip/hip_runtime.h>
#include <cstdint>
#include <cstdio>
#include <cstring>
#include <deque>
#include <map>
#include <atomic>
#include <memory>
#include <mutex>
#include <stdexcept>
#include <string>
#include <unordered_map>
#include <vector>
#include "../../include/pvface.h"

#define PVF_FHOG_STRIDE 32

struct PvfError : std::runtime_error { using std::runtime_error::runtime_error; };
struct CandOverflow : PvfError { int needed; explicit CandOverflow(int n) : PvfError("detector: candidate buffer overflow"), needed(n) {} };
struct ScreenRetry : PvfError { ScreenRetry() : PvfError("detector: screening pass gave up") {} };

#define HIP_CHECK(expr)                                                                              \
    do {                                                                                             \
        hipError_t _e = (expr);                                                                      \
// ... 56 lines not shown
        if (busy[cur]) { HIP_CHECK(hipEventSynchronize(ev[cur])); busy[cur] = false; }
        buf[cur].ensure(bytes);
        return buf[cur].p;
    }
    void sent(hipStream_t st)
    {
        if (!ev[cur]) HIP_CHECK(hipEventCreateWithFlags(&ev[cur], hipEventDisableTiming));
        HIP_CHECK(hipEventRecord(ev[cur], st));
        busy[cur] = true;
    }
    ~StageRing() { for (auto e : ev) if (e) (void)hipEventDestroy(e); }
};

struct Tensor {
    std::string name;
    int dtype = 0;
    std::vector<int64_t> dims;
    std::vector<uint8_t> data;
    size_t numel() const { size_t n = 1; for (auto d : dims) n *= (size_t)d; return n; }
    const float* f32() const { return reinterpret_cast<const float*>(data.data()); }
    const int32_t* i32() const { return reinterpret_cast<const int32_t*>(data.data()); }
    const double* f64() const { return reinterpret_cast<const double*>(data.data()); }
};
std::map<std::string, Tensor> pvf_read_container(const char* path);
std::map<std::string, Tensor> pvf_read_model(const char* path, int kind);

struct Frame {
    const uint8_t* d = nullptr;
    int h = 0, w = 0;
    bool owned = false;
    bool pooled = false;
    hipEvent_t ready = nullptr;
};

struct ProfFamily {
    std::vector<std::pair<hipEvent_t, hipEvent_t>> pending;
    double total_ms = 0;
    int64_t launches = 0;
};

struct DetectorModel {
    bool loaded = false;
    int n_filters = 0, frows = 0, fcols = 0, cell = 0, padding = 0, win_w = 0, win_h = 0, min_w = 0, min_h = 0, max_levels = 0;
    double nms_iou = 0, nms_covered = 0;
    std::vector<float> thresh;
    float* d_w = nullptr;
    float* d_bmfma4 = nullptr;
    uint16_t* d_bscreen = nullptr;
    double screen_scale = 1.0;
    double screen_bound[8] = {0, 0, 0, 0, 0, 0, 0, 0};
};

struct ShapeModel {
    bool loaded = false;
    int n_cascades = 0, n_trees = 0, n_parts = 0, n_pix = 0, depth = 0;
    float* d_initial = nullptr;
    int32_t* d_anchor = nullptr;
    float* d_deltas = nullptr;
    int32_t* d_idx1 = nullptr;
    int32_t* d_idx2 = nullptr;
    float* d_thresh = nullptr;
    float* d_leaves = nullptr;
};

struct ConvLayer {
    int cin, cout, k, stride, pad;
    float* d_w;
    float* d_bias;
    float* d_gamma;
    float* d_beta;
    float* d_frag = nullptr;
    int w_exp = 0;
    uint32_t* d_wsplit = nullptr;
};

struct EmbedModel {
    bool loaded = false;
    int chip_size = 150;
    double chip_padding = 0.25;
    std::vector<float> mean_shape;
    std::vector<ConvLayer> convs;
    float* d_fc = nullptr;
    float* d_blob = nullptr;
    float* d_stem = nullptr;
};

struct TrackerTables {
    bool set = false;
    double* d_mask64 = nullptr;
    double* d_mask_scale = nullptr;
    double* d_tw64 = nullptr;
    double* d_tw32 = nullptr;
    double alpha_pow_m16 = 0, ln_alpha = 0;
};

struct Tracker {
    double* d_state = nullptr;
    int* share = nullptr;
    double pos[4] = {0, 0, 0, 0};
    double prev_pos[4] = {0, 0, 0, 0};
    bool started = false;
    bool pending = false;
};
constexpr size_t TRK_A = 0;
constexpr size_t TRK_B = TRK_A + (size_t)32 * 64 * 64 * 2;
constexpr size_t TRK_AS = TRK_B + (size_t)64 * 64;
constexpr size_t TRK_BS = TRK_AS + (size_t)512 * 32 * 2;
constexpr size_t TRK_POS = TRK_BS + 32;
constexpr size_t TRK_DOUBLES = TRK_POS + 4;
constexpr size_t TRKF_PLANE = (size_t)64 * 64;
constexpr size_t TRKF_A = 5 * TRKF_PLANE * sizeof(float);
constexpr size_t TRKF_BYTES = TRKF_A + TRKF_PLANE;
#define TRKF_SLOT(q) ((((q) & 511) << 3) | ((q) >> 9))

struct ChipJob {
    const uint8_t* img; int h, w;
    int bx0, by0, sw, sh, levels;
    double m[4], b[2];
    int rows, cols;
    bool empty;
};
struct ChipDetails { double l, t, r, b, cs, sn; int rows, cols; };

struct Ctx {
    int device = 0;
    hipStream_t stream = nullptr;
    hipStream_t det_stream = nullptr;
    DetectorModel det;
    ShapeModel shape;
    EmbedModel emb;
    TrackerTables ttab;
    std::unordered_map<uint64_t, Frame> frames;
    std::unordered_map<uint64_t, std::unique_ptr<Tracker>> trackers;
    std::vector<double*> tracker_pool;
    std::atomic<uint64_t> next_id{1};
    std::recursive_mutex api_mu;
    std::recursive_mutex det_mu;
    std::mutex frames_mu;
    std::mutex prof_mu;
    bool prof_on = false;
    std::map<std::string, ProfFamily> prof;
    std::vector<hipEvent_t> event_pool;
    DevBuf s_grad, s_pyr, s_hist, s_norm, s_feat, s_cand, s_misc, s_chip, s_chip_pyr, s_act0, s_act1, s_act2, s_trk0, s_trk1, s_trk2, s_trkfeat, s_clu0, s_clu1;
    HostBuf h_cand, h_misc;
    StageRing stage;
    DevBuf s_cand2[2], s_fptr[2];
    HostBuf h_cand2[2], h_fptr[2];
    hipEvent_t det_ev[2] = {nullptr, nullptr};
    int det_slot = 0;
    int det_cand_cap = 8192;
    bool det_screen = true, det_screen_suspended = false, screen_attr_set = false;
    int screen_list_cap = 1 << 20;
    DevBuf s_screen;
    int64_t screen_batches = 0, screen_listed = 0, screen_retries = 0;
    double screen_pipe_err = -1;
    bool screen_pipe_flushes_subnormals = false;
    bool emb_split = true, emb_probe_done = false;
    DevBuf s_emb_flags, s_emb_redo;
    int64_t emb_split_faces = 0, emb_reruns = 0;
    double emb_pipe_err = -1;
    int n_cu = 256;
    struct PoolBuf { uint8_t* p; hipEvent_t free_after; hipEvent_t free_after_det; };
    std::map<size_t, std::deque<PoolBuf>> frame_pool;
    size_t frame_pool_bytes = 0;
    void* ingest_rings = nullptr;
    void* render_state = nullptr;
    struct MlPlanCache* ml_plans = nullptr;
    std::map<std::vector<int>, std::unique_ptr<DevBuf>> resize_tabs;
    const void* feat_ring_owner = nullptr;
    uint8_t* d_orient_lut = nullptr;
    uint8_t* d_wrap_lut = nullptr;
    DevBuf s_orb_set, s_orb_work;
    int orb_n = 0, orb_cap = 0;

    Frame frame(uint64_t id)
    {
        std::lock_guard<std::mutex> lk(frames_mu);
        auto it = frames.find(id);
        if (it == frames.end()) throw PvfError("unknown frame handle");
        Frame& f = it->second;
        if (f.ready) {
            HIP_CHECK(hipStreamWaitEvent(stream, f.ready, 0));
            HIP_CHECK(hipStreamWaitEvent(det_stream, f.ready, 0));
            (void)hipEventDestroy(f.ready);
            f.ready = nullptr;
        }
        return f;
    }
    uint8_t* take_frame_buffer(size_t bytes, hipStream_t writer)
    {
        PoolBuf b{nullptr, nullptr, nullptr};
        {
            std::lock_guard<std::mutex> lk(frames_mu);
            auto& v = frame_pool[bytes];
            if (!v.empty()) { b = v.front(); v.pop_front(); frame_pool_bytes -= bytes; }
        }
        if (!b.p) {
            HIP_CHECK(hipMalloc((void**)&b.p, bytes));
            return b.p;
        }
        for (hipEvent_t e : {b.free_after, b.free_after_det}) {
            if (!e) continue;
            if (writer) HIP_CHECK(hipStreamWaitEvent(writer, e, 0));
            else HIP_CHECK(hipEventSynchronize(e));
            (void)hipEventDestroy(e);
        }
        return b.p;
    }
    void pool_give(uint8_t* p, size_t bytes)
    {
        hipEvent_t e = nullptr, e2 = nullptr;
        HIP_CHECK(hipEventCreateWithFlags(&e, hipEventDisableTiming));
        HIP_CHECK(hipEventRecord(e, stream));
        HIP_CHECK(hipEventCreateWithFlags(&e2, hipEventDisableTiming));
        HIP_CHECK(hipEventRecord(e2, det_stream));
        frame_pool[bytes].push_back(PoolBuf{p, e, e2});
        frame_pool_bytes += bytes;
    }
    uint64_t add_frame(const Frame& f)
    {
        const uint64_t id = next_id++;
        std::lock_guard<std::mutex> lk(frames_mu);
        frames[id] = f;
        return id;
    }
    Tracker& tracker(uint64_t id)
    {
        auto it = trackers.find(id);
        if (it == trackers.end()) throw PvfError("unknown tracker handle");
        return *it->second;
    }
};

struct ProfScope {
    Ctx* c; ProfFamily* f = nullptr; hipEvent_t a = nullptr, b = nullptr; hipStream_t s = nullptr; bool ranged = false;
    ProfScope(Ctx* ctx, const char* family, hipStream_t on = nullptr);
    ~ProfScope();
};

Ctx* pvf_ctx(pvf_handle h);
void pvf_set_error(const char* msg);

struct RawDet { float score; int32_t filter, level, r, c, l, t, rr, b; };
void det_run_batch(Ctx* c, const std::vector<Frame>& frames, int upsample, double adjust,
                   std::vector<std::vector<RawDet>>& raw_sorted);
void det_run_many(Ctx* c, const std::vector<Frame>& frames, int batch, int upsample, double adjust,
                  std::vector<std::vector<RawDet>>& raw_sorted, bool nms = false);
void ml_plans_free(Ctx* c);
void ingest_free_all(Ctx* c);
struct ResizeTab { std::vector<int32_t> idx; std::vector<int16_t> coef; };
ResizeTab linear_table(int in, int out);
void render_free_all(Ctx* c);
void det_nms(const DetectorModel& m, const std::vector<RawDet>& sorted, std::vector<RawDet>& out);
void det_pyramid_level(Ctx* c, const Frame& f, int upsample, int level, std::vector<uint8_t>* out, int* h, int* w);
void det_level_features(Ctx* c, const Frame& f, int upsample, int level, std::vector<float>* out, int* fh, int* fw);
void det_level_plan(Ctx* c, const Frame& f, int upsample, int level, int32_t out[8]);
void det_pyramid_batch(Ctx* c, const std::vector<Frame>& frames, int upsample);
void fhog_debug(Ctx* c, const uint8_t* himg, int h, int w, int cell, int pad_r, int pad_c, std::vector<float>& out, int* fh, int* fw);
void fhog_device(Ctx* c, const uint8_t* d_img, int n, int h, int w, int cell, int pad_r, int pad_c, float* d_feat,
                 DevBuf& hist, DevBuf& norm, size_t img_stride_in = 0);
void fhog1_compact(Ctx* c, const uint8_t* d_chips, int n, uint8_t* d_rec);
void fhog_scale_chips(Ctx* c, const uint8_t* d_chips, int n, float* d_feat);
void fhog_dims(int ih, int iw, int cell, int pad_r, int pad_c, int* fh, int* fw);
ChipJob chip_plan(const Frame& f, const ChipDetails& d);
void chip_extract_batch(Ctx* c, const std::vector<ChipJob>& jobs, uint8_t* d_out );
void transform_batch(Ctx* c, const std::vector<ChipJob>& jobs, uint8_t* d_out);
void ert_run(Ctx* c, const std::vector<Frame>& frames, const pvf_rect_i32* boxes, int n, int32_t* pts);
void face_chip_details(const EmbedModel& m, const int32_t* pts68, ChipDetails* out);
void resnet_forward(Ctx* c, const uint8_t* d_chips, int n, float* h_out);
void conv_layer_upload(ConvLayer& L, const float* w, const float* bias, const float* gamma, const float* beta);
void conv_layer_free(ConvLayer& L);
#define EMB_STAGES 30
struct EmbedTap { int stage; float* h_out; int dims[3]; };
void resnet_debug_stage(Ctx* c, const uint8_t* d_chips, int n, bool split, EmbedTap* tap, int* h_flags);
void resnet_debug_conv(Ctx* c, const int32_t* geom, const float* in, const float* w, const float* bias, const float* gamma, const float* beta,
                       const float* skip, bool split, bool force_generic, float* out, int32_t* flags);
void resnet_debug_head(Ctx* c, const float* x, int n, int hw, float* out);
void dsst_start_many(Ctx* c, const std::vector<Tracker*>& t, const std::vector<Frame>& f, const double* boxes);
void dsst_clone_many(Ctx* c, const std::vector<Tracker*>& src, const std::vector<Tracker*>& dst);
double* tracker_state_alloc(Ctx* c);
void shot_dfd(Ctx* c, const std::vector<Frame>& frames, int ow, int oh, const float* tables22, double* dfd, uint8_t* gray_out, float* flow_out);
std::vector<int> orb_level_quota();
void orb_extract(Ctx* c, const std::vector<Frame>& frames, int ow, int oh, int cap, int32_t* counts, float* kp_out, uint8_t* desc_out);
void orb_match_counts(Ctx* c, const uint8_t* desc, const int32_t* nrows, int n_sets, int cap, const int32_t* pairs, int64_t n_pairs, int32_t* out);
void dsst_update_many(Ctx* c, const std::vector<Tracker*>& t, const std::vector<Frame>& f, double* psr, double* boxes_out, int mode = 0);
void overlap_matrix_host(const double* a, int na, const double* b, int nb, double ratio, double* out);
void munkres_host(const double* cost, int n, int32_t* row_to_col);
struct PairInput {
    const double* X = nullptr;
    const float* emb = nullptr; int64_t emb_stride = 0; int n_src = 0; const int32_t* order = nullptr; int decimals = -1; bool emb_on_device = false;
};
struct PairOutput { double* out = nullptr; bool on_device = false; bool compact = false; };
void pair_mean_dist_dev(Ctx* c, const PairInput& in, int N, int dim, const int32_t* row_start, int T, const PairOutput& out, double** d_D_keep,
                        int t0, int t1, int metric, bool mirror);
void mirror_upper_dev(Ctx* c, double* dD, int T);
int hac_dev(Ctx* c, double* d_D, const int32_t* row_start, int T, double threshold, int32_t* labels, double* merge_log);
```

### pyannote-video_amd/csrc/screen.hip

```cpp
#include "detect_ml.h"
#include <algorithm>
#include <cmath>
#include <cstring>

typedef _Float16 f16x8 __attribute__((ext_vector_type(8)));
typedef _Float16 f16x2 __attribute__((ext_vector_type(2)));

struct ScreenParams { float flag_at[8]; float lim_lo, lim_hi; int n_items, list_cap; };

#define SCR_B_BYTES (10 * 12 * 64 * 16)
#define SCR_M_STRIDE (12 * 64 * 16)

__device__ __forceinline__ uint32_t pk_f16(float a, float b)
{
    return __builtin_bit_cast(uint32_t, __builtin_amdgcn_cvt_pkrtz(a, b));
}

template <int NG>
__device__ __forceinline__ void screen_walk(const ScreenItem t, const LvDesc* __restrict__ lv, const float* __restrict__ feat_base,
                                            const uint8_t* s_b, const float th_lane, int* __restrict__ ctl, uint2* __restrict__ list,
                                            const int list_cap, u32x4& mx)
{
    constexpr int RSRC_FLAGS = 0x00020000;
    constexpr int FR = 10, FC = 10;
    static_assert(FC == SCR_FILTER_COLS, "detect_ml.h: SCR_FILTER_COLS is this kernel's filter width");
    const int lane = threadIdx.x & 63, i = lane & 15, kq = lane >> 4;
    const int fw = lv[t.lv].fw;
    const long long feat_off = lv[t.lv].feat_off, feat_stride = lv[t.lv].feat_stride;
    const int fwp = lv[t.lv].fwp;
    const float* fb = feat_base + feat_off + (size_t)t.b * feat_stride + feat_at(t.r_base, 0, t.c_base, fwp);
    const int row_bytes = (8 * fwp - t.c_base) * 16;
    const int fh_in = t.out_rows + FR - 1;
    const int c1 = fw - (FC - FC / 2 - 1);
    const int voff = i * 48 + kq * 2 * fwp * 16;
    const int voff2 = voff + fwp * 16;
    const int voff_t = i < 3 ? voff : 0x40000000, voff2_t = i < 3 ? voff2 : 0x40000000;
    f32x4 acc[10][NG];
#pragma unroll
    for (int q = 0; q < 10; ++q)
#pragma unroll
        for (int g = 0; g < NG; ++g) acc[q][g] = (f32x4){0.f, 0.f, 0.f, 0.f};
    const uint8_t* b_lo = s_b + lane * 16;
    const uint8_t* b_hi = s_b + lane * 16 + 5 * SCR_M_STRIDE;
    auto load_cls = [&](int row, int cls, u32x4 (&raw)[NG + 1][2]) {
        const __amdgpu_buffer_rsrc_t rs = __builtin_amdgcn_make_buffer_rsrc((void*)(fb + (size_t)row * 8 * fwp * 4), 0,
                                                                            row < fh_in ? row_bytes : 0, RSRC_FLAGS);
#pragma unroll
        for (int g = 0; g <= NG; ++g) {
            raw[g][0] = __builtin_amdgcn_raw_buffer_load_b128(rs, (g < NG ? voff : voff_t) + cls * 16 + g * 768, 0, 0);
            raw[g][1] = __builtin_amdgcn_raw_buffer_load_b128(rs, (g < NG ? voff2 : voff2_t) + cls * 16 + g * 768, 0, 0);
        }
    };
    auto cvt_frag = [&](const u32x4 (&r)[2]) -> u32x4 {
        u32x4 o;
        o.x = pk_f16(__uint_as_float(r[0].x), __uint_as_float(r[0].y)); o.y = pk_f16(__uint_as_float(r[0].z), __uint_as_float(r[0].w));
        o.z = pk_f16(__uint_as_float(r[1].x), __uint_as_float(r[1].y)); o.w = pk_f16(__uint_as_float(r[1].z), __uint_as_float(r[1].w));
#pragma unroll
        for (int k = 0; k < 4; ++k) mx[k] = __builtin_bit_cast(uint32_t, __builtin_elementwise_max(__builtin_bit_cast(f16x2, mx[k]), __builtin_bit_cast(f16x2, o[k])));
        return o;
    };
    auto shift_bases = [&](u32x4 (&a)[NG + 1]) {
#pragma unroll
        for (int g = 0; g <= NG; ++g) {
#pragma unroll
            for (int e = 0; e < 4; ++e) {
                int fill = 0;
                if (g < NG) fill = __builtin_amdgcn_update_dpp(0, (int)a[g + 1][e], 0x11F , 0xf, 0xf, true);
                a[g][e] = (uint32_t)__builtin_amdgcn_update_dpp(fill, (int)a[g][e], 0x101 , 0xf, 0xf, false);
            }
        }
    };
    auto emit = [&](const f32x4 (&a)[NG], int r_out) {
        float vm = a[0][0];
#pragma unroll
        for (int g = 0; g < NG; ++g)
#pragma unroll
            for (int e = 0; e < 4; ++e) vm = fmaxf(vm, a[g][e]);
        const bool hit = vm >= th_lane;
        if (r_out >= 0 && __builtin_amdgcn_ballot_w64(hit) != 0) {
            const int jc = lane & 15;
            const int sft = jc / 5, f = jc % 5;
            const int r = t.r_base + r_out + FR / 2;
#pragma unroll
            for (int g = 0; g < NG; ++g)
#pragma unroll
                for (int e = 0; e < 4; ++e) {
                    const int cc = t.c_base + 48 * g + 3 * (4 * kq + e) + sft + FC / 2;
                    if (a[g][e] >= th_lane && cc < c1) {
                        const int idx = atomicAdd(&ctl[SCR_FLAGGED], 1);
                        if (idx < list_cap) list[idx] = make_uint2((uint32_t)t.b, ((uint32_t)t.lv << 27) | ((uint32_t)f << 24) | ((uint32_t)r << 12) | (uint32_t)cc);
                    }
                }
        }
    };

    u32x4 A[3][NG + 1];
    {
        u32x4 raw[NG + 1][2];
#pragma unroll
        for (int cls = 0; cls < 3; ++cls) {
            load_cls(0, cls, raw);
#pragma unroll
            for (int g = 0; g <= NG; ++g) A[cls][g] = cvt_frag(raw[g]);
        }
    }
    auto b_frag = [&](int q, int j) -> u32x4 {
        return *reinterpret_cast<const u32x4*>((q < 5 ? b_lo + q * SCR_M_STRIDE : b_hi + (q - 5) * SCR_M_STRIDE) + j * 1024);
    };
    u32x4 bn[10];
#pragma unroll
    for (int q = 0; q < 10; ++q) bn[q] = b_frag(q, 0);
    for (int s = 0; s < fh_in; ++s) {
        u32x4 An[3][NG + 1];
        u32x4 raw[NG + 1][2];
        f32x4 done[NG];
#pragma unroll
        for (int j = 0; j < 12; ++j) {
            const int cls = j % 3;
            if (j > 0 && cls == 0) {
#pragma unroll
                for (int k = 0; k < 3; ++k) shift_bases(A[k]);
            }
            if (j % 4 == 0) load_cls(s + 1, j / 4, raw);
            u32x4 bc[10];
#pragma unroll
            for (int q = 0; q < 10; ++q) bc[q] = bn[q];
#pragma unroll
            for (int q = 0; q < 10; ++q) bn[q] = b_frag(q, (j + 1) % 12);
#pragma unroll
            for (int q = 9; q >= 0; --q) {
#pragma unroll
                for (int g = 0; g < NG; ++g) {
                    const f32x4 v = __builtin_amdgcn_mfma_f32_16x16x32_f16(__builtin_bit_cast(f16x8, A[cls][g]), __builtin_bit_cast(f16x8, bc[q]), acc[q][g], 0, 0, 0);
                    if (j < 11) acc[q][g] = v;
                    else if (q == 9) done[g] = v;
                    else acc[q + 1][g] = v;
                }
            }
            if (j % 4 == 3) {
#pragma unroll
                for (int g = 0; g <= NG; ++g) An[j / 4][g] = cvt_frag(raw[g]);
            }
            __builtin_amdgcn_sched_barrier(0);
        }
#pragma unroll
        for (int g = 0; g < NG; ++g) acc[0][g] = (f32x4){0.f, 0.f, 0.f, 0.f};
        emit(done, s - (FR - 1));
#pragma unroll
        for (int cls = 0; cls < 3; ++cls)
#pragma unroll
            for (int g = 0; g <= NG; ++g) A[cls][g] = An[cls][g];
    }
}

__global__ void __launch_bounds__(256) __attribute__((amdgpu_waves_per_eu(1, 1)))
score_screen_k(const ScreenItem* __restrict__ items, const LvDesc* __restrict__ lv, const float* __restrict__ feat_base,
               const u32x4* __restrict__ Bh, ScreenParams sp, int* __restrict__ ctl, uint2* __restrict__ list)
{
    extern __shared__ __attribute__((aligned(16))) uint8_t s_b[];
    for (int k = threadIdx.x; k < SCR_B_BYTES / 16; k += 256) reinterpret_cast<u32x4*>(s_b)[k] = Bh[k];
    __syncthreads();
    const int lane = threadIdx.x & 63;
    const int jc = lane & 15, f = jc % 5;
    float th_lane = sp.flag_at[0];
    th_lane = f == 1 ? sp.flag_at[1] : th_lane;
    th_lane = f == 2 ? sp.flag_at[2] : th_lane;
    th_lane = f == 3 ? sp.flag_at[3] : th_lane;
    th_lane = f == 4 ? sp.flag_at[4] : th_lane;
    th_lane = jc < 15 ? th_lane : 3.0e38f;
    u32x4 mx = {0u, 0u, 0u, 0u};
    for (;;) {
        int it = 0;
        if (lane == 0) it = atomicAdd(&ctl[SCR_CURSOR], 1);
        it = __builtin_amdgcn_readfirstlane(it);
        if (it >= sp.n_items) break;
        ScreenItem t;
        t.lv = __builtin_amdgcn_readfirstlane(items[it].lv); t.b = __builtin_amdgcn_readfirstlane(items[it].b);
        t.c_base = __builtin_amdgcn_readfirstlane(items[it].c_base); t.r_base = __builtin_amdgcn_readfirstlane(items[it].r_base);
        t.out_rows = __builtin_amdgcn_readfirstlane(items[it].out_rows); t.ng = __builtin_amdgcn_readfirstlane(items[it].ng);
        switch (t.ng) {
        case 1: screen_walk<1>(t, lv, feat_base, s_b, th_lane, ctl, list, sp.list_cap, mx); break;
        case 2: screen_walk<2>(t, lv, feat_base, s_b, th_lane, ctl, list, sp.list_cap, mx); break;
        case 3: screen_walk<3>(t, lv, feat_base, s_b, th_lane, ctl, list, sp.list_cap, mx); break;
        default: screen_walk<4>(t, lv, feat_base, s_b, th_lane, ctl, list, sp.list_cap, mx); break;
        }
    }
    auto lo16 = [](uint32_t v) { return (float)__builtin_bit_cast(f16x2, v)[0]; };
    auto hi16 = [](uint32_t v) { return (float)__builtin_bit_cast(f16x2, v)[1]; };
    const float m_lo = fmaxf(fmaxf(lo16(mx.x), hi16(mx.x)), lo16(mx.y));
    const float m_hi = fmaxf(fmaxf(hi16(mx.y), fmaxf(lo16(mx.z), hi16(mx.z))), fmaxf(lo16(mx.w), hi16(mx.w)));
    const float lim_hi = (lane >> 4) == 3 ? sp.lim_hi : sp.lim_lo;
    if (m_lo > sp.lim_lo || m_hi > lim_hi) atomicOr(&ctl[SCR_VIOLATION], 1);
}

__global__ void __launch_bounds__(256) score_list_k(const uint2* __restrict__ list, const int* __restrict__ ctl, int list_cap,
                                                    const LvDesc* __restrict__ lv, const float* __restrict__ feat_base,
                                                    const float* __restrict__ W, ScoreParams sp, int* __restrict__ counts, CandRec* __restrict__ cands)
{
    constexpr int FR = 10, FC = 10;
    const int n = min(ctl[SCR_FLAGGED], list_cap);
    for (int e = blockIdx.x * 256 + threadIdx.x; e < n; e += gridDim.x * 256) {
        const uint2 q = list[e];
        const int b = (int)q.x;
        const int l = (int)(q.y >> 27), f = (int)((q.y >> 24) & 7), r = (int)((q.y >> 12) & 4095), cc = (int)(q.y & 4095);
        const int fwp = lv[l].fwp;
        const float* fp = feat_base + lv[l].feat_off + (size_t)b * lv[l].feat_stride + feat_at(r - FR / 2, 0, cc - FC / 2, fwp);
        const float* wp = W + (size_t)f * FR * FC * PVF_FHOG_STRIDE;
        float acc = 0.0f;
        for (int m = 0; m < FR; ++m)
            for (int nn = 0; nn < FC; ++nn) {
                const f32x4* fv = reinterpret_cast<const f32x4*>(fp + feat_at(m, 0, nn, fwp));
                const f32x4* wv = reinterpret_cast<const f32x4*>(wp + ((size_t)m * FC + nn) * PVF_FHOG_STRIDE);
#pragma unroll
                for (int k = 0; k < 8; ++k) {
                    const f32x4 a = fv[(size_t)k * fwp], w = wv[k];
                    acc = fmaf(a[0], w[0], acc); acc = fmaf(a[1], w[1], acc); acc = fmaf(a[2], w[2], acc);
                    if (k < 7) acc = fmaf(a[3], w[3], acc);
                }
            }
        const float th = sp.thresh[f];
        if (acc >= th) {
            const int idx = atomicAdd(&counts[b], 1);
            if (idx < sp.cap) {
                CandRec rec;
                rec.score = acc - th; rec.filter = f; rec.level = l; rec.r = r; rec.c = cc;
                cands[(size_t)b * sp.cap + idx] = rec;
            }
        }
    }
}

__global__ void screen_probe_k(const u32x4* __restrict__ a, const u32x4* __restrict__ b, int steps, float* __restrict__ d, int* __restrict__ moved)
{
    const int lane = threadIdx.x;
    f32x4 acc = {0.f, 0.f, 0.f, 0.f};
    for (int s = 0; s < steps; ++s)
        acc = __builtin_amdgcn_mfma_f32_16x16x32_f16(__builtin_bit_cast(f16x8, a[s * 64 + lane]), __builtin_bit_cast(f16x8, b[s * 64 + lane]), acc, 0, 0, 0);
    for (int e = 0; e < 4; ++e) d[lane * 4 + e] = acc[e];
    const int fill = __builtin_amdgcn_update_dpp(0, lane + 1000, 0x11F, 0xf, 0xf, false);
    moved[lane] = __builtin_amdgcn_update_dpp(fill, lane + 100, 0x101, 0xf, 0xf, false);
}

static uint16_t f32_to_f16_rne(float v)
{
    uint32_t x;
    memcpy(&x, &v, 4);
    const uint32_t sign = (x >> 16) & 0x8000u;
    const int32_t e = (int32_t)((x >> 23) & 0xff) - 127 + 15;
    uint32_t man = x & 0x7fffffu;
    if (((x >> 23) & 0xff) == 0xff) return (uint16_t)(sign | 0x7c00u | (man ? 0x200u : 0));
    if (e >= 31) return (uint16_t)(sign | 0x7c00u);
    if (e <= 0) {
        if (e < -10) return (uint16_t)sign;
        man |= 0x800000u;
        const int shift = 14 - e;
        const uint32_t half = man >> shift, rem = man & ((1u << shift) - 1), mid = 1u << (shift - 1);
        uint32_t h = half;
        if (rem > mid || (rem == mid && (half & 1))) ++h;
        return (uint16_t)(sign | h);
    }
    uint32_t h = ((uint32_t)e << 10) | (man >> 13);
    const uint32_t rem = man & 0x1fffu;
    if (rem > 0x1000u || (rem == 0x1000u && (h & 1))) ++h;
    return (uint16_t)(sign | h);
}
static double f16_to_f64(uint16_t h)
{
    const int s = (h >> 15) & 1, e = (h >> 10) & 31, m = h & 1023;
    double v;
    if (e == 0) v = std::ldexp((double)m, -24);
    else if (e == 31) v = INFINITY;
    else v = std::ldexp((double)(m | 1024), e - 25);
    return s ? -v : v;
}

static const double SCR_FM_LO = 0.4004, SCR_FM_HI = 0.8492;
static const float SCR_LIM_LO = 0.400146484375f , SCR_LIM_HI = 0.8486328125f ;

void screen_prepare_model(DetectorModel& d, const float* w)
{
    PVF_REQUIRE(d.n_filters == 5 && d.frows == 10 && d.fcols == 10, "screening: 5 filters of 10 x 10 cells");
    double wmax = 0;
    for (size_t k = 0; k < (size_t)d.n_filters * 10 * 10 * 32; ++k) wmax = std::max(wmax, std::fabs((double)w[k]));
    PVF_REQUIRE(std::isfinite(wmax), "detector weights are not finite");
    int sh = 0;
    if (wmax > 0) { int ex; (void)std::frexp(wmax, &ex); sh = 7 - ex; }
    sh = std::max(-100, std::min(100, sh));
    const double SCR_SCALE = std::ldexp(1.0, sh);
    d.screen_scale = SCR_SCALE;
    std::vector<uint16_t> bh((size_t)10 * 12 * 64 * 8, 0);
    for (int m = 0; m < 10; ++m)
        for (int j = 0; j < 12; ++j)
            for (int l = 0; l < 64; ++l) {
                const int jc = l & 15, kq = l >> 4;
                if (jc >= 15) continue;
                const int sft = jc / 5, f = jc % 5, n = j - sft;
                if (n < 0 || n >= 10) continue;
                for (int e = 0; e < 8; ++e) {
                    const int p = 8 * kq + e;
                    if (p >= 31) continue;
                    bh[(((size_t)m * 12 + j) * 64 + l) * 8 + e] = f32_to_f16_rne((float)((double)w[(((size_t)f * 10 + m) * 10 + n) * 32 + p] * SCR_SCALE));
                }
            }
    if (d.d_bscreen) (void)hipFree(d.d_bscreen);
    HIP_CHECK(hipMalloc((void**)&d.d_bscreen, bh.size() * sizeof(uint16_t)));
    HIP_CHECK(hipMemcpy(d.d_bscreen, bh.data(), bh.size() * sizeof(uint16_t), hipMemcpyHostToDevice));
    const double u = std::ldexp(1.0, -24);
    for (int f = 0; f < d.n_filters; ++f) {
        double e_w = 0, e_f = 0, e_sub = 0, a_h = 0, a_w = 0;
        for (int m = 0; m < 10; ++m)
            for (int n = 0; n < 10; ++n)
                for (int p = 0; p < 31; ++p) {
                    const double wv = (double)w[(((size_t)f * 10 + m) * 10 + n) * 32 + p];
                    const double wh = f16_to_f64(f32_to_f16_rne((float)(wv * SCR_SCALE))) / SCR_SCALE;
                    const double fm = p < 27 ? SCR_FM_LO : SCR_FM_HI;
                    e_w += fm * std::fabs(wh - wv);
                    e_f += std::fabs(wh) * std::max(fm * std::ldexp(1.0, -10), std::ldexp(1.0, -14));
                    a_h += fm * std::fabs(wh);
                    a_w += fm * std::fabs(wv);
                    if (wh != 0.0 && std::fabs(wh) * SCR_SCALE < std::ldexp(1.0, -14)) e_sub += fm * std::fabs(wh);
                }
        const double e_pipe = 3200.0 * std::ldexp(1.0, -22) * a_h * (1.0 + std::ldexp(1.0, -10));
        const double e_chain = 3100.0 * u / (1.0 - 3100.0 * u) * a_w;
        d.screen_bound[f] = 1.02 * (e_w + e_f + e_sub + e_pipe + e_chain) + 1e-6;
    }
}

void screen_plan_build(ScreenPlan& sp, const std::vector<LvDesc>& lv, int B)
{
    int seg = 16;
    for (int cand : {512, 160, 96, 64, 48, 32, 24}) {
        long long n = 0;
        for (const LvDesc& d : lv)
            if (d.valid_score) n += (long long)((d.fw - 9 + 48 * SCR_SG - 1) / (48 * SCR_SG)) * ((d.fh - 9 + cand - 1) / cand) * B;
        if (n >= 3 * 1024) { seg = cand; break; }
    }
    if (getenv("PVF_SCREEN_SEG") && atoi(getenv("PVF_SCREEN_SEG")) > 0) seg = std::max(2, atoi(getenv("PVF_SCREEN_SEG")));
    std::vector<ScreenItem> items;
    sp.usable = lv.size() <= 32;
    for (const LvDesc& d : lv) sp.usable = sp.usable && d.fh < 4096 && d.fw < 4096;
    if (!sp.usable) return;
    for (int l = 0; l < (int)lv.size(); ++l) {
        const LvDesc& d = lv[l];
        if (!d.valid_score) continue;
        const int out_c = d.fw - 9, out_r = d.fh - 9;
        const int nseg = (out_r + seg - 1) / seg, rows = (out_r + nseg - 1) / nseg;
        for (int c0 = 0; c0 < out_c; c0 += 48 * SCR_SG)
            for (int r0 = 0; r0 < out_r; r0 += rows)
                for (int b = 0; b < B; ++b)
                    items.push_back(ScreenItem{l, b, c0, r0, std::min(rows, out_r - r0), std::min(SCR_SG, (out_c - c0 + 47) / 48)});
    }
    for (const ScreenItem& it : items)
        PVF_REQUIRE(it.ng >= 1 && it.c_base + SCR_GROUP_COLS * it.ng + SCR_TAIL_CELLS - 1 < lv[it.lv].fwp,
                    "screening plan: a strip's tail read passes the FEAT_PAD_COLS zero columns of its feature row");
    std::stable_sort(items.begin(), items.end(), [](const ScreenItem& a, const ScreenItem& b) { return a.ng * (a.out_rows + 9) > b.ng * (b.out_rows + 9); });
    if (sp.d_items) (void)hipFree(sp.d_items);
    sp.d_items = nullptr;
    sp.n_items = (int)items.size();
    if (items.empty()) return;
    HIP_CHECK(hipMalloc((void**)&sp.d_items, items.size() * sizeof(ScreenItem)));
    HIP_CHECK(hipMemcpy(sp.d_items, items.data(), items.size() * sizeof(ScreenItem), hipMemcpyHostToDevice));
}

static void screen_probe(Ctx* c)
{
    const int steps = 100;
    const size_t nh = (size_t)steps * 64 * 8;
    std::vector<uint16_t> ha(nh), hb(nh);
    uint8_t* dev = nullptr;
    const size_t fb = nh * 2;
    HIP_CHECK(hipMalloc((void**)&dev, 2 * fb + 64 * 4 * sizeof(float) + 64 * sizeof(int)));
    float* d_d = reinterpret_cast<float*>(dev + 2 * fb);
    int* d_m = reinterpret_cast<int*>(dev + 2 * fb + 64 * 4 * sizeof(float));
    float hd[256];
    int hm[64];
    auto A = [&](int row, int K) -> uint16_t& { return ha[((size_t)(K >> 5) * 64 + ((K >> 3) & 3) * 16 + row) * 8 + (K & 7)]; };
    auto B = [&](int K, int col) -> uint16_t& { return hb[((size_t)(K >> 5) * 64 + ((K >> 3) & 3) * 16 + col) * 8 + (K & 7)]; };
    auto run = [&]() {
        HIP_CHECK(hipMemcpy(dev, ha.data(), fb, hipMemcpyHostToDevice));
        HIP_CHECK(hipMemcpy(dev + fb, hb.data(), fb, hipMemcpyHostToDevice));
        hipLaunchKernelGGL(screen_probe_k, dim3(1), dim3(64), 0, c->det_stream, reinterpret_cast<const u32x4*>(dev), reinterpret_cast<const u32x4*>(dev + fb),
                           steps, d_d, d_m);
        HIP_CHECK(hipMemcpyAsync(hd, d_d, sizeof hd, hipMemcpyDeviceToHost, c->det_stream));
        HIP_CHECK(hipMemcpyAsync(hm, d_m, sizeof hm, hipMemcpyDeviceToHost, c->det_stream));
        HIP_CHECK(hipStreamSynchronize(c->det_stream));
    };
    auto worst_rel = [&]() {
        double worst = 0;
        for (int l = 0; l < 64; ++l)
            for (int e = 0; e < 4; ++e) {
                const int col = l & 15, row = 4 * (l >> 4) + e;
                double sum = 0, mag = 0;
                for (int K = 0; K < 32 * steps; ++K) {
                    const double t = f16_to_f64(A(row, K)) * f16_to_f64(B(K, col));
                    sum += t; mag += std::fabs(t);
                }
                if (mag > 0) worst = std::max(worst, std::fabs((double)hd[l * 4 + e] - sum) / mag);
            }
        return worst;
    };
    uint32_t rs = 12345u;
    auto rnd = [&]() { rs = rs * 1664525u + 1013904223u; return (double)(rs >> 8) / 16777216.0; };
    double worst = 0;
    for (int s = 0; s < steps; ++s)
        for (int l = 0; l < 64; ++l)
            for (int e = 0; e < 8; ++e) {
                ha[((size_t)s * 64 + l) * 8 + e] = f32_to_f16_rne((float)(0.05 + 0.8 * rnd()));
                const double sgn = ((l & 15) < 8 || ((s + e) & 1)) ? 1.0 : -1.0;
                hb[((size_t)s * 64 + l) * 8 + e] = f32_to_f16_rne((float)(sgn * (1.0 + 25.0 * rnd())));
            }
    run();
    worst = std::max(worst, worst_rel());
    bool dpp_ok = true;
    for (int l = 0; l < 64; ++l) dpp_ok = dpp_ok && hm[l] == ((l & 15) < 15 ? l + 101 : l - 15 + 1000);
    for (int order = 0; order < 2; ++order) {
        std::vector<double> av(32 * steps), bv(32 * steps);
        for (int K = 0; K < 32 * steps; ++K) {
            av[K] = std::ldexp(1.0 + rnd(), -14 + (int)(rnd() * 21.999));
            bv[K] = std::ldexp(1.0 + rnd(), -14 + (int)(rnd() * 21.999));
        }
        std::vector<int> idx(32 * steps);
        for (int K = 0; K < 32 * steps; ++K) idx[K] = K;
        if (order == 1) std::sort(idx.begin(), idx.end(), [&](int x, int y) { return av[x] * bv[x] > av[y] * bv[y]; });
        for (int K = 0; K < 32 * steps; ++K)
            for (int r = 0; r < 16; ++r) {
                const int kk = idx[(K + 97 * r) % (32 * steps)], kr = idx[(32 * steps - 1 - K + 97 * r) % (32 * steps)];
                A(r, K) = f32_to_f16_rne((float)av[r < 8 ? kk : kr]);
                B(K, r) = f32_to_f16_rne((float)bv[r < 8 ? kk : kr]);
            }
        run();
        worst = std::max(worst, worst_rel());
    }
    {
        const DetectorModel& m = c->det;
        std::vector<float> w((size_t)5 * 10 * 10 * 32);
        HIP_CHECK(hipMemcpy(w.data(), m.d_w, w.size() * sizeof(float), hipMemcpyDeviceToHost));
        std::fill(ha.begin(), ha.end(), (uint16_t)0);
        std::fill(hb.begin(), hb.end(), (uint16_t)0);
        for (int K = 0; K < 3100; ++K) {
            const int cellp = K / 31, p = K % 31;
            const double fm = p < 27 ? (double)SCR_LIM_LO : (double)SCR_LIM_HI;
            for (int col = 0; col < 16; ++col)
                B(K, col) = f32_to_f16_rne((float)((double)w[((size_t)(col % 5) * 100 + cellp) * 32 + p] * m.screen_scale));
            for (int row = 0; row < 16; ++row) {
                double f;
                switch (row & 3) {
                case 0: f = fm; break;
                case 1: f = (K & 1) ? fm : 0.0; break;
                case 2: f = (K & 1) ? 0.0 : fm; break;
                default: f = fm * rnd(); break;
                }
                A(row, K) = f32_to_f16_rne((float)f);
            }
        }
        run();
        worst = std::max(worst, worst_rel());
    }
    {
        for (size_t i = 0; i < nh; ++i) { ha[i] = 0x3c00u ; hb[i] = 0x0010u ; }
        run();
        c->screen_pipe_flushes_subnormals = !(hd[0] > 0.0f);
        if (!c->screen_pipe_flushes_subnormals) worst = std::max(worst, worst_rel());
    }
    (void)hipFree(dev);
    c->screen_pipe_err = worst;
    PVF_REQUIRE(worst <= 3200.0 * std::ldexp(1.0, -22), "screening: v_mfma_f32_16x16x32_f16 does not accumulate as the error bound of the screening pass assumes on this device");
    PVF_REQUIRE(dpp_ok, "screening: v_mov_b32_dpp row_shl:1 / row_shr:15 do not move data as the screening kernel expects on this device");
}

void screen_launch(Ctx* c, const ScreenPlan& plan, const LvDesc* d_lv, int B, const float* feat, const ScoreParams& thr, int* d_counts,
                   CandRec* d_cands, int* ctl)
{
    const DetectorModel& m = c->det;
    if (plan.n_items == 0) return;
    if (!c->screen_attr_set) {
        screen_probe(c);
        HIP_CHECK(hipFuncSetAttribute(reinterpret_cast<const void*>(score_screen_k), hipFuncAttributeMaxDynamicSharedMemorySize, SCR_B_BYTES));
        c->screen_attr_set = true;
    }
    ScreenParams sp;
    for (int f = 0; f < 8; ++f) {
        if (f < m.n_filters) {
            const float at = (float)(((double)thr.thresh[f] - m.screen_bound[f]) * m.screen_scale);
            sp.flag_at[f] = std::nextafterf(at, -INFINITY);
        }
        else sp.flag_at[f] = 3.0e38f;
    }
    sp.lim_lo = SCR_LIM_LO; sp.lim_hi = SCR_LIM_HI;
    if (const char* e = getenv("PVF_SCREEN_LIMIT_SCALE")) {
        sp.lim_lo *= (float)atof(e); sp.lim_hi *= (float)atof(e);
    }
    sp.n_items = plan.n_items;
    sp.list_cap = c->screen_list_cap;
    c->s_screen.ensure((size_t)sp.list_cap * sizeof(uint2) + 64);
    uint2* list = c->s_screen.as<uint2>();
    const int grid = std::min(c->n_cu, (plan.n_items + 3) / 4);
    hipLaunchKernelGGL(score_screen_k, dim3(grid), dim3(256), SCR_B_BYTES, c->det_stream, plan.d_items, d_lv, feat,
                       reinterpret_cast<const u32x4*>(m.d_bscreen), sp, ctl, list);
    hipLaunchKernelGGL(score_list_k, dim3(256), dim3(256), 0, c->det_stream, list, ctl, sp.list_cap, d_lv, feat, m.d_w, thr, d_counts, d_cands);
}
```

### pyannote-video_amd/pyannote_video_amd/_lib.py

```python
import ctypes as C
import os
import numpy as np

_HERE = os.path.dirname(os.path.abspath(__file__))
LIB_PATH = os.environ.get("PVF_LIBRARY") or os.path.join(_HERE, "libpvface.so")

_lib = None


class PvfError(RuntimeError):
    pass


class OrbCapError(PvfError):

    def __init__(self, message, needed):
        PvfError.__init__(self, message)
        self.needed = int(needed)


class Rect(C.Structure):
    _fields_ = [("left", C.c_int32), ("top", C.c_int32), ("right", C.c_int32), ("bottom", C.c_int32)]


H = C.c_uint64
P = C.c_void_p
_SIGS = {
    "pvf_last_error": (C.c_char_p, []),
    "pvf_version": (C.c_int32, []),
    "pvf_device_count": (C.c_int32, [P]),
    "pvf_ctx_create": (C.c_int32, [C.c_int32, P]),
    "pvf_ctx_create_prio": (C.c_int32, [C.c_int32, C.c_int32, P]),
    "pvf_ctx_destroy": (C.c_int32, [H]),
    "pvf_sync": (C.c_int32, [H]),
    "pvf_load_detector": (C.c_int32, [H, C.c_char_p]),
    "pvf_load_shape_predictor": (C.c_int32, [H, C.c_char_p]),
    "pvf_load_embedder": (C.c_int32, [H, C.c_char_p]),
    "pvf_model_tensor": (C.c_int32, [C.c_char_p, C.c_int32, C.c_char_p, P, C.c_int64, P]),
    "pvf_set_tracker_tables": (C.c_int32, [H, P, P, P, P, C.c_double, C.c_double]),
    "pvf_frame_upload": (C.c_int32, [H, P, C.c_int32, C.c_int32, C.c_int64, P]),
    "pvf_frame_wrap_device": (C.c_int32, [H, P, C.c_int32, C.c_int32, P]),
    "pvf_frame_release": (C.c_int32, [H, H]),
    "pvf_frame_release_many": (C.c_int32, [H, P, C.c_int32]),
    "pvf_frame_pool_trim": (C.c_int32, [H, C.c_int64, P]),
    "pvf_mem_info": (C.c_int32, [H, P, P]),
    "pvf_frame_device_ptr": (C.c_int32, [H, H, P]),
    "pvf_ingest_create": (C.c_int32, [H, C.c_int32, C.c_int32, C.c_int32, P]),
    "pvf_ingest_destroy": (C.c_int32, [H, H]),
    "pvf_ingest_acquire": (C.c_int32, [H, H, P, P]),
    "pvf_ingest_submit": (C.c_int32, [H, H, C.c_int32, P]),
    "pvf_ingest_wait": (C.c_int32, [H, H]),
    "pvf_ingest_create_yuv": (C.c_int32, [H, C.c_int32, C.c_int32, C.c_int32, C.c_int32, C.c_int32, P]),
    "pvf_frame_from_yuv": (C.c_int32, [H, P, C.c_int64, P, P, C.c_int64, C.c_int32, C.c_int32, C.c_int32, C.c_int32, C.c_int32, P]),
    "pvf_frame_resize": (C.c_int32, [H, H, C.c_int32, C.c_int32, P]),
    "pvf_render_batch": (C.c_int32, [H, P, C.c_int32, C.c_int32, C.c_int32, C.c_int32, P, P, P, C.c_int64, P, C.c_int32]),
    "pvf_egress_create": (C.c_int32, [H, C.c_int32, C.c_int32, C.c_int32, C.c_int32, P]),
    "pvf_egress_destroy": (C.c_int32, [H, H]),
    "pvf_egress_submit": (C.c_int32, [H, H, H, P, C.c_int32, P, C.c_int64, P]),
    "pvf_egress_wait": (C.c_int32, [H, H, C.c_int32, P]),
    "pvf_egress_release": (C.c_int32, [H, H, C.c_int32]),
    "pvf_debug_render_rgb": (C.c_int32, [H, H, C.c_int32, C.c_int32, P, C.c_int32, P, C.c_int64, P]),
    "pvf_detect": (C.c_int32, [H, H, C.c_int32, C.c_double, P, P, C.c_int32, P]),
    "pvf_detect_batch": (C.c_int32, [H, P, C.c_int32, C.c_int32, C.c_double, P, P, P, C.c_int32]),
    "pvf_detect_many": (C.c_int32, [H, P, C.c_int32, C.c_int32, C.c_int32, C.c_double, P, P, P, C.c_int32]),
    "pvf_detector_screening": (C.c_int32, [H, C.c_int32, C.c_int32]),
    "pvf_detector_screening_stats": (C.c_int32, [H, P, P, P, P, P]),
    "pvf_embedder_split": (C.c_int32, [H, C.c_int32]),
    "pvf_embedder_split_stats": (C.c_int32, [H, P, P, P]),
    "pvf_tracker_create": (C.c_int32, [H, P]),
    "pvf_tracker_destroy": (C.c_int32, [H, H]),
    "pvf_tracker_create_many": (C.c_int32, [H, C.c_int32, P]),
    "pvf_tracker_destroy_many": (C.c_int32, [H, P, C.c_int32]),
    "pvf_tracker_clone_many": (C.c_int32, [H, P, C.c_int32, P]),
    "pvf_tracker_start": (C.c_int32, [H, H, H, P]),
    "pvf_tracker_update": (C.c_int32, [H, H, H, P]),
    "pvf_tracker_position": (C.c_int32, [H, H, P]),
    "pvf_tracker_start_many": (C.c_int32, [H, P, P, P, C.c_int32]),
    "pvf_tracker_update_many": (C.c_int32, [H, P, P, C.c_int32, P, P]),
    "pvf_tracker_update_many_deferred": (C.c_int32, [H, P, P, C.c_int32, P, P]),
    "pvf_tracker_commit_many": (C.c_int32, [H, P, P, C.c_int32]),
    "pvf_overlap_matrix": (C.c_int32, [P, C.c_int32, P, C.c_int32, C.c_double, P]),
    "pvf_munkres": (C.c_int32, [P, C.c_int32, P]),
    "pvf_associate": (C.c_int32, [P, C.c_int32, P, C.c_int32, C.c_double, P]),
    "pvf_landmarks": (C.c_int32, [H, P, P, C.c_int32, P]),
    "pvf_embed": (C.c_int32, [H, P, P, C.c_int32, P]),
    "pvf_landmarks_embed": (C.c_int32, [H, P, P, C.c_int32, P, P]),
    "pvf_embed_chips": (C.c_int32, [H, P, C.c_int32, P]),
    "pvf_face_chips": (C.c_int32, [H, P, P, C.c_int32, P]),
    "pvf_pair_mean_dist": (C.c_int32, [H, P, C.c_int32, C.c_int32, P, C.c_int32, P]),
    "pvf_pair_mean_dist_metric": (C.c_int32, [H, P, C.c_int32, C.c_int32, P, C.c_int32, C.c_int32, P]),
    "pvf_pair_mean_dist_rows": (C.c_int32, [H, P, C.c_int32, C.c_int32, P, C.c_int32, C.c_int32, C.c_int32, P]),
    "pvf_pair_upper_rows": (C.c_int32, [H, P, C.c_int32, C.c_int32, P, C.c_int32, C.c_int32, C.c_int32, P]),
    "pvf_lane_create": (C.c_int32, [C.c_int32, P, P, C.c_int32, C.c_double, C.c_double, C.c_int32, P]),
    "pvf_lane_destroy": (C.c_int32, [H]),
    "pvf_lane_feed_plan": (C.c_int32, [H, C.c_int32, C.c_int32, P, P, P, P]),
    "pvf_lane_advance": (C.c_int32, [H, P, P, C.c_int32, P, P, P, C.c_int32, P, P]),
    "pvf_lane_take_dead": (C.c_int32, [H, P, C.c_int32, P]),
    "pvf_lane_edges": (C.c_int32, [H, P, P, P, P, P, P, C.c_int32]),
    "pvf_shot_tracks": (C.c_int32, [H, H, P, C.c_int32, C.c_double, P, C.c_int32, P, P, C.c_int32, P]),
    "pvf_track_rows": (C.c_int32, [P, C.c_int64, C.c_int32, C.c_int32, C.c_int32, C.c_int32, P, P]),
    "pvf_round_decimals": (C.c_int32, [P, C.c_int64, C.c_int32, P]),
    "pvf_cluster_dist": (C.c_int32, [H, P, P, C.c_int32, C.c_double, P, P, P]),
    "pvf_cluster_tracks": (C.c_int32, [H, P, C.c_int32, C.c_int32, P, C.c_int32, C.c_double, P, P, P]),
    "pvf_cluster_upper": (C.c_int32, [H, P, C.c_int32, P, C.c_int32, C.c_double, P, P, P]),
    "pvf_cluster_tracks_f32": (C.c_int32, [H, P, C.c_int64, C.c_int32, C.c_int32, P, C.c_int32, C.c_int32, P, C.c_int32, C.c_int32, C.c_double, P, P, P]),
    "pvf_pair_upper_rows_f32": (C.c_int32, [H, P, C.c_int64, C.c_int32, C.c_int32, P, C.c_int32, C.c_int32, P, C.c_int32, C.c_int32, C.c_int32, P, C.c_int32]),
    "pvf_format_rows": (C.c_int32, [P, P, P, C.c_int64, C.c_int32, C.c_int32, P, C.c_int64, P]),
    "pvf_round_rows": (C.c_int32, [P, C.c_int64, C.c_int32, P]),
    "pvf_parse_rows": (C.c_int32, [C.c_char_p, C.c_int64, P, C.c_int64, P, P]),
    "pvf_prof_enable": (C.c_int32, [H, C.c_int32]),
    "pvf_prof_reset": (C.c_int32, [H]),
    "pvf_prof_get": (C.c_int32, [H, C.c_char_p, P, P]),
    "pvf_debug_pyramid_level": (C.c_int32, [H, H, C.c_int32, C.c_int32, P, P, P]),
    "pvf_debug_pyramid_batch": (C.c_int32, [H, P, C.c_int32, C.c_int32]),
    "pvf_debug_level_features": (C.c_int32, [H, H, C.c_int32, C.c_int32, P, P, P]),
    "pvf_debug_level_plan": (C.c_int32, [H, H, C.c_int32, C.c_int32, P]),
    "pvf_debug_fhog": (C.c_int32, [H, P, C.c_int32, C.c_int32, C.c_int32, C.c_int32, C.c_int32, P, P, P]),
    "pvf_debug_detect_raw": (C.c_int32, [H, H, C.c_int32, C.c_double, P, P, C.c_int32, P]),
    "pvf_debug_detect_raw_many": (C.c_int32, [H, P, C.c_int32, C.c_int32, C.c_int32, C.c_double, P, P, C.c_int64, P]),
    "pvf_debug_extract_chip": (C.c_int32, [H, H, P, C.c_double, C.c_double, C.c_int32, C.c_int32, P]),
    "pvf_debug_tracker_state": (C.c_int32, [H, H, P, P, P]),
    "pvf_debug_tracker_scale_state": (C.c_int32, [H, H, P, P]),
    "pvf_debug_embed_stage": (C.c_int32, [H, P, C.c_int32, C.c_int32, C.c_int32, P, P, P]),
    "pvf_debug_conv": (C.c_int32, [H, P, P, P, P, P, P, P, C.c_int32, C.c_int32, P, P]),
    "pvf_debug_embed_head": (C.c_int32, [H, P, C.c_int32, C.c_int32, P]),
    "pvf_shot_dfd": (C.c_int32, [H, P, C.c_int32, C.c_int32, C.c_int32, P, P, P, P]),
    "pvf_orb_extract": (C.c_int32, [H, P, C.c_int32, C.c_int32, C.c_int32, C.c_int32, P, P, P]),
    "pvf_orb_match_counts": (C.c_int32, [H, P, P, C.c_int32, C.c_int32, P, C.c_int64, P]),
}
EXPORTS = sorted(_SIGS)


def lib():
    global _lib
    if _lib is None:
        if not os.path.exists(LIB_PATH):
            raise PvfError("libpvface.so is not built (%s): run `python -c 'import __graft_entry__ as g; g.build()'`; "
                           "there is no CPU fallback" % LIB_PATH)
        l = C.CDLL(LIB_PATH)
        for name, (res, args) in _SIGS.items():
            fn = getattr(l, name)
            fn.restype = res
            fn.argtypes = args
        _lib = l
    return _lib


def check(rc):
    if rc != 0:
        raise PvfError(lib().pvf_last_error().decode("utf-8", "replace"))


def ptr(a):
    return a.ctypes.data_as(C.c_void_p) if a is not None else None


def handles(seq):
    return np.ascontiguousarray(np.asarray(seq, dtype=np.uint64))


def device_count():
    n = C.c_int32(0)
    check(lib().pvf_device_count(C.byref(n)))
    return n.value


def model_tensor(path, kind, name, dtype):
    n = C.c_int64(0)
    check(lib().pvf_model_tensor(str(path).encode(), int(kind), name.encode(), None, 0, C.byref(n)))
    out = np.zeros(n.value // np.dtype(dtype).itemsize, dtype)
    check(lib().pvf_model_tensor(str(path).encode(), int(kind), name.encode(), ptr(out), out.nbytes, C.byref(n)))
    return out


def overlap_matrix(a, b, ratio):
    a = np.ascontiguousarray(a, np.float64).reshape(-1, 4)
    b = np.ascontiguousarray(b, np.float64).reshape(-1, 4)
    out = np.zeros((len(a), len(b)), np.float64)
    check(lib().pvf_overlap_matrix(ptr(a), len(a), ptr(b), len(b), float(ratio), ptr(out)))
    return out


import threading as _threading
_assoc_tls = _threading.local()
_ASSOC_KEEP = 256


def associate(trackers, detections, ratio):
    na, nb = len(trackers), len(detections)
    key = (na, nb)
    cache = getattr(_assoc_tls, "buf", None)
    if cache is None:
        cache = _assoc_tls.buf = {}
    buf = cache.get(key)
    if buf is None:
        if len(cache) >= _ASSOC_KEEP:
            cache.clear()
        buf = cache[key] = ((C.c_double * (4 * na))(), (C.c_double * (4 * nb))(), (C.c_int32 * max(na, 1))())
    a, b, out = buf
    k = 0
    for box in trackers:
        a[k], a[k + 1], a[k + 2], a[k + 3] = box
        k += 4
    k = 0
    for box in detections:
        b[k], b[k + 1], b[k + 2], b[k + 3] = box
        k += 4
    check(lib().pvf_associate(a, na, b, nb, float(ratio), out))
    return [(t, d) for t, d in enumerate(out[:na]) if d >= 0]


def round_decimals(x, decimals):
    x = np.ascontiguousarray(x, np.float64)
    out = np.empty_like(x)
    if x.size:
        check(lib().pvf_round_decimals(ptr(x), x.size, int(decimals), ptr(out)))
    return out


def track_rows(boxes, det_width, det_height, width, height):
    b = np.ascontiguousarray(boxes, np.int32).reshape(-1, 4)
    fb = np.empty(b.shape, np.float64)
    pb = np.empty(b.shape, np.int32)
    if len(b):
        check(lib().pvf_track_rows(ptr(b), len(b), int(det_width), int(det_height), int(width), int(height), ptr(fb), ptr(pb)))
    return fb, pb


def format_rows(t, identifier, values, decimals=5):
    t = np.ascontiguousarray(t, np.float64)
    ident = np.ascontiguousarray(identifier, np.int64)
    v = np.ascontiguousarray(values, np.float64)
    v = v.reshape(len(t), -1) if len(t) else v.reshape(0, max(v.shape[-1], 1) if v.ndim else 1)
    cap = len(t) * (64 + 42 * v.shape[1])
    buf = np.empty(max(cap, 1), np.uint8)
    n = C.c_int64(0)
    check(lib().pvf_format_rows(ptr(t), ptr(ident), ptr(v), len(t), v.shape[1], int(decimals), ptr(buf), cap, C.byref(n)))
    return buf[:n.value].tobytes()


def round_rows(x, decimals=5):
    x = np.ascontiguousarray(x, np.float32)
    out = np.empty(x.shape, np.float64)
    check(lib().pvf_round_rows(ptr(x), x.size, int(decimals), ptr(out)))
    return out


def parse_rows(text):
    n = len(text)
    rows, cols = C.c_int64(0), C.c_int32(0)
    for cap in (n // 6 + 16, n // 2 + 1):
        out = np.empty(cap, np.float64)
        if lib().pvf_parse_rows(text, n, ptr(out), out.size, C.byref(rows), C.byref(cols)) == 0:
            return out[:rows.value * cols.value].reshape(rows.value, cols.value)
        if b"too small" not in lib().pvf_last_error():
            break
    raise PvfError(lib().pvf_last_error().decode("utf-8", "replace"))


def munkres(cost):
    cost = np.ascontiguousarray(cost, np.float64)
    n = cost.shape[0]
    assert cost.shape == (n, n)
    out = np.zeros(n, np.int32)
    check(lib().pvf_munkres(ptr(cost), n, ptr(out)))
    return [(i, int(out[i])) for i in range(n)]
```

### pyannote-video_amd/pyannote_video_amd/runtime.py

```python
import contextlib
import ctypes as C
import threading
import itertools
import operator
import numpy as np
from . import _lib
from ._lib import check, ptr, handles
from . import models as _models
from .y4m import YuvFrame, chroma_shape


class DeviceFrame(object):
    __slots__ = ("ctx", "handle", "height", "width", "keep", "transient", "__weakref__")

    def __init__(self, ctx, handle, height, width, keep=None, transient=False):
        self.ctx, self.handle, self.height, self.width, self.keep = ctx, handle, height, width, keep
        self.transient = transient

    @property
    def shape(self):
        return (self.height, self.width, 3)

    def release(self):
        if self.handle is not None and self.ctx._h is not None:
# ... 355 lines not shown
        from . import render as _render
        _, p, text = _render.pack_primitives([prims])
        out = np.empty((int(height), int(width), 3), np.uint8)
        check(self._l.pvf_debug_render_rgb(self._h, self.stage(frame).handle, int(width), int(height), ptr(p), len(p), ptr(text), len(text),
                                           ptr(out)))
        return out

    def frame_from_yuv_device(self, y_ptr, y_pitch, u_ptr, v_ptr, c_pitch, height, width, layout="420", matrix="601", full_range=False,
                              c_step=1):
        h = C.c_uint64(0)
        check(self._l.pvf_frame_from_yuv(self._h, C.c_void_p(int(y_ptr)), int(y_pitch), C.c_void_p(int(u_ptr)), C.c_void_p(int(v_ptr)),
                                         int(c_pitch), int(c_step), int(height), int(width), _yuv_layout(layout),
                                         _yuv_flags(matrix, full_range), C.byref(h)))
        return DeviceFrame(self, h.value, int(height), int(width))

    def frame_from_yuv_torch(self, y, u, v=None, layout="420", matrix="601", full_range=False):
        for t in (y, u) + (() if v is None else (v,)):
            assert t.is_cuda and t.element_size() == 1 and t.stride(-1) == 1
        if v is None:
            assert u.dim() == 3 and u.shape[2] == 2 and (u.shape[1] == 1 or u.stride(1) == 2)
            return self.frame_from_yuv_device(y.data_ptr(), y.stride(0), u.data_ptr(), u.data_ptr() + 1, u.stride(0), y.shape[0], y.shape[1],
                                              layout, matrix, full_range, c_step=2)
        assert u.dim() == 2 and v.dim() == 2 and u.shape == v.shape and u.stride(0) == v.stride(0)
        return self.frame_from_yuv_device(y.data_ptr(), y.stride(0), u.data_ptr(), v.data_ptr(), u.stride(0), y.shape[0], y.shape[1],
                                          layout, matrix, full_range)

    def stage(self, rgb):
        if isinstance(rgb, DeviceFrame):
            return rgb
        key = (id(rgb), rgb.__array_interface__["data"][0] if hasattr(rgb, "__array_interface__") else 0)
        with self._stage_mu:
            f = self._staged.get(key)
            if f is None or f.keep is not rgb:
                f = self.upload(rgb)
                f.keep = rgb
                self._staged[key] = f
                self._staged_order.append(key)
                if not self._hold:
                    self._trim()
            return f

    def _trim(self):
        with self._stage_mu:
            while len(self._staged_order) > self.stage_capacity:
                old = self._staged_order.pop(0)
                g = self._staged.pop(old, None)
                if g is not None:
                    g.release()

    @contextlib.contextmanager
    def _staging(self):
        with self._stage_mu:
            self._hold += 1
        try:
            yield
        finally:
            with self._stage_mu:
                self._hold -= 1
                if not self._hold:
                    self._trim()

    def _handles(self, frames):
        if isinstance(frames, np.ndarray) and frames.dtype == np.uint64:
            return np.ascontiguousarray(frames)
        try:
            return np.fromiter(map(_handle_of, frames), dtype=np.uint64, count=len(frames))
        except AttributeError:
            return handles([self.stage(f).handle for f in frames])

    def frame_handles(self, frames):
        return self._handles(frames)

    def unstage_all(self):
        for f in self._staged.values():
            f.release()
        self._staged.clear()
        self._staged_order = []

    def detect_batch(self, frames, upsample=1, adjust_threshold=0.0, cap=256):
        n = len(frames)
        out = np.zeros((n, cap, 4), np.int32)
        scores = np.zeros((n, cap), np.float32)
        counts = np.zeros(n, np.int32)
        with self._staging():
            hs = self._handles(frames)
            check(self._l.pvf_detect_batch(self._h, ptr(hs), n, int(upsample), float(adjust_threshold), ptr(out), ptr(scores), ptr(counts), cap))
        if int(counts.max(initial=0)) >= cap:
            return self.detect_batch(frames, upsample, adjust_threshold, cap * 8)
        return _boxes_and_scores(out, scores, counts)

    def detect_many(self, frames, batch, upsample=1, adjust_threshold=0.0, cap=64, arrays=False):
        n = len(frames)
        out = np.zeros((n, cap, 4), np.int32)
        scores = np.zeros((n, cap), np.float32)
        counts = np.zeros(n, np.int32)
        with self._staging():
            hs = self._handles(frames)
            check(self._l.pvf_detect_many(self._h, ptr(hs), n, int(batch), int(upsample), float(adjust_threshold), ptr(out), ptr(scores), ptr(counts), cap))
        if int(counts.max(initial=0)) >= cap:
            return self.detect_many(frames, batch, upsample, adjust_threshold, cap * 8, arrays)
        if arrays:
            m = int(counts.max(initial=0))
            return out[:, :m], scores[:, :m], counts
        return _boxes_and_scores(out, scores, counts)

    def detect(self, frame, upsample=1, adjust_threshold=0.0):
        return self.detect_batch([frame], upsample, adjust_threshold)[0]

    def detect_raw(self, frame, upsample=1, adjust_threshold=0.0, cap=65536):
        f = self.stage(frame)
        scores = np.zeros(cap, np.float32)
        meta = np.zeros((cap, 8), np.int32)
        n = C.c_int32(0)
        check(self._l.pvf_debug_detect_raw(self._h, f.handle, int(upsample), float(adjust_threshold), ptr(scores), ptr(meta), cap, C.byref(n)))
        k = min(n.value, cap)
        return [(float(scores[i]), int(meta[i, 0]), int(meta[i, 1]), int(meta[i, 2]), int(meta[i, 3]),
                 tuple(int(v) for v in meta[i, 4:8])) for i in range(k)]

    def detect_raw_many(self, frames, batch, upsample=1, adjust_threshold=0.0, cap=1 << 16):
        n = len(frames)
        counts = np.zeros(n, np.int32)
        total = C.c_int64(0)
        with self._staging():
            hs = self._handles(frames)
            while True:
                rows = np.zeros((cap, 5), np.int32)
                check(self._l.pvf_debug_detect_raw_many(self._h, ptr(hs), n, int(batch), int(upsample), float(adjust_threshold), ptr(counts), ptr(rows), cap, C.byref(total)))
                if total.value <= cap:
                    break
                cap = int(total.value)
        off = np.concatenate([[0], np.cumsum(counts)])
        return [rows[off[i]:off[i + 1]] for i in range(n)]

    def pyramid_batch(self, frames, upsample=1):
        with self._staging():
            hs = self._handles(frames)
            check(self._l.pvf_debug_pyramid_batch(self._h, ptr(hs), len(frames), int(upsample)))

    def pyramid_level(self, frame, upsample, level):
        f = self.stage(frame)
        oh, ow = C.c_int32(0), C.c_int32(0)
        check(self._l.pvf_debug_pyramid_level(self._h, f.handle, upsample, level, None, C.byref(oh), C.byref(ow)))
        out = np.zeros((oh.value, ow.value, 3), np.uint8)
        check(self._l.pvf_debug_pyramid_level(self._h, f.handle, upsample, level, ptr(out), C.byref(oh), C.byref(ow)))
        return out

    def level_features(self, frame, upsample, level):
        f = self.stage(frame)
        fh, fw = C.c_int32(0), C.c_int32(0)
        check(self._l.pvf_debug_level_features(self._h, f.handle, upsample, level, None, C.byref(fh), C.byref(fw)))
        out = np.zeros((fh.value, fw.value, 32), np.float32)
        if out.size:
            check(self._l.pvf_debug_level_features(self._h, f.handle, upsample, level, ptr(out), C.byref(fh), C.byref(fw)))
        return out

    def level_plan(self, frame, upsample, level):
        f = self.stage(frame)
        out = np.zeros(8, np.int32)
        check(self._l.pvf_debug_level_plan(self._h, f.handle, int(upsample), int(level), ptr(out)))
        return dict(zip(("h", "w", "hog_nr", "hog_nc", "chunk_rows", "chunks", "roll_rows", "roll_nseg"), (int(v) for v in out)))

    def fhog(self, img, cell, pad_r, pad_c):
        img = np.ascontiguousarray(img, np.uint8)
        fh, fw = C.c_int32(0), C.c_int32(0)
        check(self._l.pvf_debug_fhog(self._h, ptr(img), img.shape[0], img.shape[1], cell, pad_r, pad_c, None, C.byref(fh), C.byref(fw)))
        out = np.zeros((fh.value, fw.value, 32), np.float32)
        check(self._l.pvf_debug_fhog(self._h, ptr(img), img.shape[0], img.shape[1], cell, pad_r, pad_c, ptr(out), C.byref(fh), C.byref(fw)))
        return out

    def tracker_create(self):
        self.ensure_tracker_tables()
        h = C.c_uint64(0)
        check(self._l.pvf_tracker_create(self._h, C.byref(h)))
        return h.value

    def tracker_create_many(self, n, as_array=False):
        self.ensure_tracker_tables()
        out = np.zeros(int(n), np.uint64)
        if n:
            check(self._l.pvf_tracker_create_many(self._h, int(n), ptr(out)))
        return out if as_array else out.tolist()

    def tracker_clone_many(self, trks, as_array=False):
        out = np.zeros(len(trks), np.uint64)
        if len(trks):
            check(self._l.pvf_tracker_clone_many(self._h, ptr(handles(trks)), len(trks), ptr(out)))
        return out if as_array else out.tolist()

    def tracker_destroy_many(self, trks):
        if self._h is not None and len(trks):
            check(self._l.pvf_tracker_destroy_many(self._h, ptr(handles(trks)), len(trks)))

    def tracker_destroy(self, trk):
        if self._h is not None:
            check(self._l.pvf_tracker_destroy(self._h, trk))

    def tracker_start_many(self, trks, frames, boxes):
        if not len(trks):
            return
        b = np.ascontiguousarray(boxes, np.float64).reshape(-1, 4)
        with self._staging():
            check(self._l.pvf_tracker_start_many(self._h, ptr(handles(trks)), ptr(self._handles(frames)), ptr(b), len(trks)))

    def tracker_update_many(self, trks, frames, defer=False):
        n = len(trks)
        if not n:
            return np.zeros(0), np.zeros((0, 4))
        psr = np.zeros(n, np.float64)
        boxes = np.zeros((n, 4), np.float64)
        fn = self._l.pvf_tracker_update_many_deferred if defer else self._l.pvf_tracker_update_many
        with self._staging():
            check(fn(self._h, ptr(handles(trks)), ptr(self._handles(frames)), n, ptr(psr), ptr(boxes)))
        return psr, boxes

    def tracker_commit_many(self, trks, frames):
        n = len(trks)
        if n:
            with self._staging():
                check(self._l.pvf_tracker_commit_many(self._h, ptr(handles(trks)), ptr(self._handles(frames)), n))

    def tracker_position(self, trk):
        b = np.zeros(4, np.float64)
        check(self._l.pvf_tracker_position(self._h, trk, ptr(b)))
        return tuple(b.tolist())

    def tracker_state(self, trk):
        F = np.zeros((32, 64, 64, 2), np.float64)
        A = np.zeros((32, 64, 64, 2), np.float64)
        B = np.zeros((64, 64), np.float64)
        check(self._l.pvf_debug_tracker_state(self._h, trk, ptr(F), ptr(A), ptr(B)))
        return F, A, B

    def tracker_scale_state(self, trk):
        As = np.zeros((512, 32, 2), np.float64)
        Bs = np.zeros(32, np.float64)
        check(self._l.pvf_debug_tracker_scale_state(self._h, trk, ptr(As), ptr(Bs)))
        return As, Bs

    def landmarks(self, frames, boxes):
        n = len(boxes)
        pts = np.zeros((n, 68, 2), np.int32)
        if n == 0:
            return pts
        r = _rects(boxes, n)
        with self._staging():
            check(self._l.pvf_landmarks(self._h, ptr(self._handles(frames)), ptr(r), n, ptr(pts)))
        return pts

    def embed(self, frames, pts):
        pts = np.ascontiguousarray(pts, np.int32).reshape(-1, 68, 2)
        n = len(pts)
        out = np.zeros((n, 128), np.float32)
        if n == 0:
            return out
        with self._staging():
            check(self._l.pvf_embed(self._h, ptr(self._handles(frames)), ptr(pts), n, ptr(out)))
        return out

    def landmarks_embed(self, frames, boxes):
        n = len(boxes)
        pts = np.zeros((n, 68, 2), np.int32)
        out = np.zeros((n, 128), np.float32)
        if n == 0:
            return pts, out
        r = _rects(boxes, n)
        with self._staging():
            check(self._l.pvf_landmarks_embed(self._h, ptr(self._handles(frames)), ptr(r), n, ptr(pts), ptr(out)))
        return pts, out

    def face_chips(self, frames, pts):
        pts = np.ascontiguousarray(pts, np.int32).reshape(-1, 68, 2)
        n = len(pts)
        out = np.zeros((n, 150, 150, 3), np.uint8)
        with self._staging():
            check(self._l.pvf_face_chips(self._h, ptr(self._handles(frames)), ptr(pts), n, ptr(out)))
        return out

    def embed_chips(self, chips):
        chips = np.ascontiguousarray(chips, np.uint8).reshape(-1, 150, 150, 3)
        out = np.zeros((len(chips), 128), np.float32)
        check(self._l.pvf_embed_chips(self._h, ptr(chips), len(chips), ptr(out)))
        return out

    def extract_chip(self, frame, rect, cs, sn, rows, cols):
        f = self.stage(frame)
        r = np.asarray(rect, np.float64)
        out = np.zeros((rows, cols, 3), np.uint8)
        check(self._l.pvf_debug_extract_chip(self._h, f.handle, ptr(r), float(cs), float(sn), rows, cols, ptr(out)))
        return out

    EMBED_STAGES = 30

    def embed_stage(self, chips, stage, split):
        chips = np.ascontiguousarray(chips, np.uint8).reshape(-1, 150, 150, 3)
        n = len(chips)
        dims = np.zeros(3, np.int32)
        check(self._l.pvf_debug_embed_stage(self._h, None, n, 1 if split else 0, int(stage), None, ptr(dims), None))
        out = np.zeros((n,) + tuple(int(d) for d in dims), np.float32)
        flags = np.zeros(n, np.int32)
        check(self._l.pvf_debug_embed_stage(self._h, ptr(chips), n, 1 if split else 0, int(stage), ptr(out), ptr(dims), ptr(flags)))
        return out, flags

    def debug_conv(self, x, w, bias, gamma, beta, stride=1, pad=1, skip=None, skip_mode=0, out_hw=None, split=False, force_generic=False):
        x = np.ascontiguousarray(x, np.float32)
        w = np.ascontiguousarray(w, np.float32)
        B, H, W, cin = x.shape
# ... 229 lines not shown
```

Measured before the change: 4777.

## Write f16 FHOG copy in feature kernel and screen from it directly

The FHOG kernel now also writes a packed f16 copy of the feature map while the screening pass is enabled. The screening kernel reads this f16 map instead of loading f32 features and converting them per fragment, which halves its load traffic and removes the conversion instructions. The cost is extra stores and a second buffer in the FHOG kernel, plus zeroing of the f16 padding ring. The exact f32 scoring of listed candidates still reads the f32 map.

```diff
diff --git a/include/pvface.h b/include/pvface.h
--- a/include/pvface.h
+++ b/include/pvface.h
@@ -163,6 +163,8 @@
 int32_t pvf_debug_pyramid_batch(pvf_handle ctx, const pvf_handle* frames, int32_t n, int32_t upsample);
 int32_t pvf_debug_level_features(pvf_handle ctx, pvf_handle frame, int32_t upsample, int32_t level,
                                  float* out, int32_t* fh, int32_t* fw);
+int32_t pvf_debug_level_features_f16(pvf_handle ctx, pvf_handle frame, int32_t upsample, int32_t level,
+                                     uint16_t* out, int32_t* fh, int32_t* fw);
 int32_t pvf_debug_level_plan(pvf_handle ctx, pvf_handle frame, int32_t upsample, int32_t level, int32_t* out8);
 int32_t pvf_debug_fhog(pvf_handle ctx, const uint8_t* img, int32_t h, int32_t w, int32_t cell, int32_t pad_r,
                        int32_t pad_c, float* out, int32_t* fh, int32_t* fw);
diff --git a/pyannote-video_amd/csrc/api.hip b/pyannote-video_amd/csrc/api.hip
--- a/pyannote-video_amd/csrc/api.hip
+++ b/pyannote-video_amd/csrc/api.hip
@@ -223,6 +223,18 @@
     det_level_features(c, c->frame(frame), upsample, level, out ? &buf : nullptr, &a, &b);
     *fh = a; *fw = b;
     if (out) memcpy(out, buf.data(), buf.size() * sizeof(float));
+    API_END
+}
+
+extern "C" int32_t pvf_debug_level_features_f16(pvf_handle h, pvf_handle frame, int32_t upsample, int32_t level, uint16_t* out, int32_t* fh, int32_t* fw)
+{
+    API_BEGIN
+    ENTER_DET(c, h);
+    std::vector<uint16_t> buf;
+    int a = 0, b = 0;
+    det_level_features_f16(c, c->frame(frame), upsample, level, out ? &buf : nullptr, &a, &b);
+    *fh = a; *fw = b;
+    if (out) memcpy(out, buf.data(), buf.size() * sizeof(uint16_t));
     API_END
 }
 
diff --git a/pyannote-video_amd/csrc/ctx.hip b/pyannote-video_amd/csrc/ctx.hip
--- a/pyannote-video_amd/csrc/ctx.hip
+++ b/pyannote-video_amd/csrc/ctx.hip
@@ -256,7 +256,7 @@
     catch (const std::exception& e) { pvf_set_error(e.what()); return -1; } \
     catch (...) { pvf_set_error("unknown error"); return -2; }
 
-extern "C" int32_t pvf_version(void) { return 500; }
+extern "C" int32_t pvf_version(void) { return 510; }
 
 extern "C" int32_t pvf_device_count(int32_t* n)
 {
diff --git a/pyannote-video_amd/csrc/detect.hip b/pyannote-video_amd/csrc/detect.hip
--- a/pyannote-video_amd/csrc/detect.hip
+++ b/pyannote-video_amd/csrc/detect.hip
@@ -340,9 +340,10 @@
     return r;
 }
 
+template <bool H16>
 __global__ void __launch_bounds__(512) __attribute__((amdgpu_waves_per_eu(4, 4)))
 fhog_split_ml_k(MlStarts st, const LvDesc* __restrict__ lv, int B, const uint8_t* __restrict__ img_base, float* __restrict__ feat_base,
-                const uint8_t* __restrict__ lutw, int oy, int ox)
+                uint16_t* __restrict__ feath_base, const uint8_t* __restrict__ lutw, int oy, int ox)
 {
     constexpr int RSRC_FLAGS = 0x00020000;
     extern __shared__ __attribute__((aligned(16))) uint32_t fs_lds[];
@@ -480,6 +481,24 @@
             if (lane >= 1 && lane <= FUSED_OUT && x < d.hog_nc) {
                 float4* dst = reinterpret_cast<float4*>(feat_base + d.feat_off + (size_t)b * d.feat_stride + feat_at(yh + oy, 0, x + ox, d.fwp));
                 const size_t step = (size_t)d.fwp;
+                __amdgpu_buffer_rsrc_t hrs;
+                int hoff = 0, hstep = 0;
+                uint32_t ph0 = 0, ph1 = 0;
+                if (H16) {
+                    uint16_t* hrow = feath_base + d.feath_off + (size_t)b * d.feath_stride + feat_h_at(yh + oy, 0, 0, d.fwp);
+                    hrs = __builtin_amdgcn_make_buffer_rsrc((void*)hrow, 0, 4 * d.fwp * 16, RSRC_FLAGS);
+                    hoff = (x + ox) * 16;
+                    hstep = d.fwp * 16;
+                }
+                auto h_first = [&](float a0, float a1, float a2, float a3) {
+                    if (H16) { ph0 = pk_f16(a0, a1); ph1 = pk_f16(a2, a3); }
+                };
+                auto h_second = [&](int k, float a0, float a1, float a2, float a3) {
+                    if (H16) {
+                        const u32x4 piece = {ph0, ph1, pk_f16(a0, a1), pk_f16(a2, a3)};
+                        __builtin_amdgcn_raw_buffer_store_b128(piece, hrs, hoff, k * hstep, 0);
+                    }
+                };
                 const float eps = 0.0001f;
                 const float z1[4] = {n[4], n[1], n[3], n[0]}, z2[4] = {n[5], n[2], n[4], n[1]}, z3[4] = {n[7], n[4], n[6], n[3]}, z4[4] = {n[8], n[5], n[7], n[4]};
                 float nn[4], nv[4], t[4] = {0.f, 0.f, 0.f, 0.f};
@@ -500,10 +519,10 @@
                     }
 #pragma unroll
                     for (int k = 0; k < 4; ++k) t[k] = t[k] + ((hh[0][k] + hh[1][k]) + hh[2][k]);
-                    if (g == 3) { *dst = make_float4(o[0], o[1], o[2], o[3]); dst += step; __builtin_amdgcn_sched_barrier(0); }
-                    if (g == 6) { *dst = make_float4(o[4], o[5], o[6], o[7]); dst += step; __builtin_amdgcn_sched_barrier(0); }
-                    if (g == 9) { *dst = make_float4(o[8], o[9], o[10], o[11]); dst += step; __builtin_amdgcn_sched_barrier(0); }
-                    if (g == 15) { *dst = make_float4(o[12], o[13], o[14], o[15]); dst += step; __builtin_amdgcn_sched_barrier(0); }
+                    if (g == 3) { *dst = make_float4(o[0], o[1], o[2], o[3]); dst += step; h_first(o[0], o[1], o[2], o[3]); __builtin_amdgcn_sched_barrier(0); }
+                    if (g == 6) { *dst = make_float4(o[4], o[5], o[6], o[7]); dst += step; h_second(0, o[4], o[5], o[6], o[7]); __builtin_amdgcn_sched_barrier(0); }
+                    if (g == 9) { *dst = make_float4(o[8], o[9], o[10], o[11]); dst += step; h_first(o[8], o[9], o[10], o[11]); __builtin_amdgcn_sched_barrier(0); }
+                    if (g == 15) { *dst = make_float4(o[12], o[13], o[14], o[15]); dst += step; h_second(1, o[12], o[13], o[14], o[15]); __builtin_amdgcn_sched_barrier(0); }
                 }
                 float ci[9];
 #pragma unroll
@@ -513,14 +532,16 @@
 #pragma unroll
                     for (int k = 0; k < 4; ++k) hh[k] = fminf(s2, nn[k]) * nv[k];
                     ci[g] = (hh[0] + hh[1]) + (hh[2] + hh[3]);
-                    if (g == 1) { *dst = make_float4(o[16], o[17], ci[0], ci[1]); dst += step; __builtin_amdgcn_sched_barrier(0); }
-                    if (g == 5) { *dst = make_float4(ci[2], ci[3], ci[4], ci[5]); dst += step; __builtin_amdgcn_sched_barrier(0); }
+                    if (g == 1) { *dst = make_float4(o[16], o[17], ci[0], ci[1]); dst += step; h_first(o[16], o[17], ci[0], ci[1]); __builtin_amdgcn_sched_barrier(0); }
+                    if (g == 5) { *dst = make_float4(ci[2], ci[3], ci[4], ci[5]); dst += step; h_second(2, ci[2], ci[3], ci[4], ci[5]); __builtin_amdgcn_sched_barrier(0); }
                 }
                 const float tscale = (float)(2 * 0.2357);
 #pragma unroll
                 for (int k = 0; k < 4; ++k) t[k] = t[k] * tscale;
                 *dst = make_float4(ci[6], ci[7], ci[8], t[0]); dst += step;
+                h_first(ci[6], ci[7], ci[8], t[0]);
                 *dst = make_float4(t[1], t[2], t[3], 0.0f);
+                h_second(3, t[1], t[2], t[3], 0.0f);
             }
         }
 #pragma unroll
@@ -532,7 +553,8 @@
     }
 }
 
-__global__ void __launch_bounds__(256) feat_ring_zero_k(MlStarts st, const LvDesc* __restrict__ lv, int B, float* __restrict__ feat_base, int oy, int ox)
+__global__ void __launch_bounds__(256) feat_ring_zero_k(MlStarts st, const LvDesc* __restrict__ lv, int B, float* __restrict__ feat_base,
+                                                        uint16_t* __restrict__ feath_base, int oy, int ox)
 {
     const int g = ml_block(st);
     if (g >= st.b0[st.nl]) return;
@@ -546,9 +568,16 @@
     if (px >= d.fwp) return;
     const int x = px - ox, y = py - oy;
     if (x >= 0 && y >= 0 && x < d.hog_nc && y < d.hog_nr) return;
-    float4* dst = reinterpret_cast<float4*>(feat_base + d.feat_off + (size_t)b * d.feat_stride + feat_at(py, 0, px, d.fwp));
-#pragma unroll
-    for (int k = 0; k < 8; ++k) dst[(size_t)k * d.fwp] = make_float4(0.f, 0.f, 0.f, 0.f);
+    if (feat_base) {
+        float4* dst = reinterpret_cast<float4*>(feat_base + d.feat_off + (size_t)b * d.feat_stride + feat_at(py, 0, px, d.fwp));
+#pragma unroll
+        for (int k = 0; k < 8; ++k) dst[(size_t)k * d.fwp] = make_float4(0.f, 0.f, 0.f, 0.f);
+    }
+    if (feath_base) {
+        uint4* dh = reinterpret_cast<uint4*>(feath_base + d.feath_off + (size_t)b * d.feath_stride + feat_h_at(py, 0, px, d.fwp));
+#pragma unroll
+        for (int k = 0; k < 4; ++k) dh[(size_t)k * d.fwp] = make_uint4(0u, 0u, 0u, 0u);
+    }
 }
 
 __global__ void __launch_bounds__(128) __attribute__((amdgpu_waves_per_eu(2, 2)))
@@ -811,6 +840,7 @@
         p.img_bytes += (size_t)d.img_stride * B;
         d.fwp = feat_ok ? d.fw + FEAT_PAD_COLS : 0;
         d.feat_off = (long long)p.feat_floats; d.feat_stride = (long long)d.fh * d.fwp * PVF_FHOG_STRIDE;
+        d.feath_off = d.feat_off; d.feath_stride = d.feat_stride;
         p.feat_floats += (size_t)d.feat_stride * B;
         d.feat_bx = feat_ok ? (d.fwp + 255) / 256 : 0;
         const int out_c = d.fw - 9;
@@ -951,21 +981,33 @@
     const int oy = (m.frows - 1) / 2, ox = (m.fcols - 1) / 2;
     const void* feat_before = c->s_feat.p;
     c->s_feat.ensure(p->feat_floats * sizeof(float) + 64);
+    const bool h16 = c->det_screen && !c->det_screen_suspended;
+    const void* feath_before = c->s_feat_h.p;
+    if (h16) c->s_feat_h.ensure(p->feat_floats * sizeof(uint16_t) + 64);
     if (p->fused_blocks == 0) return p;
     check_dpp_direction(c);
     ProfScope ps(c, "fhog", c->det_stream);
-    if (c->s_feat.p != feat_before || c->feat_ring_owner != (const void*)p) {
-        hipLaunchKernelGGL(feat_ring_zero_k, dim3(ml_grid(p->feat_blocks)), dim3(256), 0, c->det_stream, p->feat, p->d_lv, B, c->s_feat.as<float>(), oy, ox);
-        c->feat_ring_owner = (const void*)p;
+    const bool ring32 = c->s_feat.p != feat_before || c->feat_ring_owner != (const void*)p;
+    const bool ring16 = h16 && (c->s_feat_h.p != feath_before || c->feat_h_ring_owner != (const void*)p);
+    if (ring32 || ring16) {
+        hipLaunchKernelGGL(feat_ring_zero_k, dim3(ml_grid(p->feat_blocks)), dim3(256), 0, c->det_stream, p->feat, p->d_lv, B,
+                           ring32 ? c->s_feat.as<float>() : nullptr, ring16 ? c->s_feat_h.as<uint16_t>() : nullptr, oy, ox);
+        if (ring32) c->feat_ring_owner = (const void*)p;
+        if (ring16) c->feat_h_ring_owner = (const void*)p;
     }
     static std::atomic<uint64_t> attr_set{0};
     const uint64_t bit = 1ull << (c->device & 63);
     if (!(attr_set.load() & bit)) {
-        HIP_CHECK(hipFuncSetAttribute(reinterpret_cast<const void*>(fhog_split_ml_k), hipFuncAttributeMaxDynamicSharedMemorySize, FS_LDS_BYTES));
+        HIP_CHECK(hipFuncSetAttribute(reinterpret_cast<const void*>(fhog_split_ml_k<false>), hipFuncAttributeMaxDynamicSharedMemorySize, FS_LDS_BYTES));
+        HIP_CHECK(hipFuncSetAttribute(reinterpret_cast<const void*>(fhog_split_ml_k<true>), hipFuncAttributeMaxDynamicSharedMemorySize, FS_LDS_BYTES));
         attr_set.fetch_or(bit);
     }
-    hipLaunchKernelGGL(fhog_split_ml_k, dim3(ml_grid(p->fused_blocks)), dim3(512), FS_LDS_BYTES, c->det_stream, p->fused, p->d_lv, B,
-                       c->s_pyr.as<uint8_t>(), c->s_feat.as<float>(), orientation_lut_wrapped(c), oy, ox);
+    if (h16)
+        hipLaunchKernelGGL(fhog_split_ml_k<true>, dim3(ml_grid(p->fused_blocks)), dim3(512), FS_LDS_BYTES, c->det_stream, p->fused, p->d_lv, B,
+                           c->s_pyr.as<uint8_t>(), c->s_feat.as<float>(), c->s_feat_h.as<uint16_t>(), orientation_lut_wrapped(c), oy, ox);
+    else
+        hipLaunchKernelGGL(fhog_split_ml_k<false>, dim3(ml_grid(p->fused_blocks)), dim3(512), FS_LDS_BYTES, c->det_stream, p->fused, p->d_lv, B,
+                           c->s_pyr.as<uint8_t>(), c->s_feat.as<float>(), (uint16_t*)nullptr, orientation_lut_wrapped(c), oy, ox);
     return p;
 }
 
@@ -979,7 +1021,7 @@
         if (!p->screen_built) { screen_plan_build(p->screen, p->lv, B); p->screen_built = true; }
         if (p->screen.usable) {
             ProfScope ps(c, "score_screened", c->det_stream);
-            screen_launch(c, p->screen, p->d_lv, B, c->s_feat.as<float>(), sp0, d_counts, d_cands, d_counts + B);
+            screen_launch(c, p->screen, p->d_lv, B, c->s_feat.as<float>(), c->s_feat_h.as<uint16_t>(), sp0, d_counts, d_cands, d_counts + B);
             ++c->screen_batches;
             return;
         }
@@ -1031,6 +1073,30 @@
             for (int j = 0; j < 8; ++j)
                 for (int x = 0; x < d.fw; ++x)
                     memcpy(out->data() + ((size_t)y * d.fw + x) * PVF_FHOG_STRIDE + 4 * j, dev.data() + feat_at(y, j, x, d.fwp), 4 * sizeof(float));
+    }
+    HIP_CHECK(hipStreamSynchronize(c->det_stream));
+}
+
+void det_level_features_f16(Ctx* c, const Frame& f, int upsample, int level, std::vector<uint16_t>* out, int* fh, int* fw)
+{
+    PVF_REQUIRE(c->det.loaded, "detector not loaded");
+    std::vector<Frame> fr{f};
+    MlPlan* p = ml_features(c, fr, upsample);
+    PVF_REQUIRE(level >= 0 && level < (int)p->lv.size(), "pyramid level out of range");
+    const LvDesc& d = p->lv[level];
+    *fh = d.fh; *fw = d.fw;
+    if (out) {
+        out->resize((size_t)d.fh * d.fw * PVF_FHOG_STRIDE);
+        PVF_REQUIRE(out->empty() || c->s_feat_h.cap >= (size_t)(d.feath_off + d.feath_stride) * sizeof(uint16_t),
+                    "f16 feature map: the screening pass has not run at this size in this context");
+        std::vector<uint16_t> dev((size_t)d.feath_stride);
+        if (!dev.empty())
+            HIP_CHECK(hipMemcpyAsync(dev.data(), c->s_feat_h.as<uint16_t>() + d.feath_off, dev.size() * sizeof(uint16_t), hipMemcpyDeviceToHost, c->det_stream));
+        HIP_CHECK(hipStreamSynchronize(c->det_stream));
+        for (int y = 0; y < d.fh; ++y)
+            for (int k = 0; k < 4; ++k)
+                for (int x = 0; x < d.fw; ++x)
+                    memcpy(out->data() + ((size_t)y * d.fw + x) * PVF_FHOG_STRIDE + 8 * k, dev.data() + feat_h_at(y, k, x, d.fwp), 8 * sizeof(uint16_t));
     }
     HIP_CHECK(hipStreamSynchronize(c->det_stream));
 }
diff --git a/pyannote-video_amd/csrc/detect_ml.h b/pyannote-video_amd/csrc/detect_ml.h
--- a/pyannote-video_amd/csrc/detect_ml.h
+++ b/pyannote-video_amd/csrc/detect_ml.h
@@ -14,11 +14,14 @@
     int strips, chunks, chunk_rows, fused_tasks;
     long long img_off, img_stride;
     long long feat_off, feat_stride;
+    long long feath_off, feath_stride;
 };
 struct MlStarts { int nl; int b0[ML_MAX + 1]; };
 
 #define FEAT_PAD_COLS 52
 __host__ __device__ __forceinline__ size_t feat_at(int row, int j, int col, int fwp) { return (((size_t)row * 8 + j) * fwp + col) * 4; }
+__host__ __device__ __forceinline__ size_t feat_h_at(int row, int k, int col, int fwp) { return (((size_t)row * 4 + k) * fwp + col) * 8; }
+__device__ __forceinline__ uint32_t pk_f16(float a, float b) { return __builtin_bit_cast(uint32_t, __builtin_amdgcn_cvt_pkrtz(a, b)); }
 
 struct ScoreParams { float thresh[8]; int n_filters; int level; int cap; };
 struct CandRec { float score; int32_t filter, level, r, c; };
@@ -42,6 +45,6 @@
     ScreenPlan& operator=(const ScreenPlan&) = delete;
 };
 void screen_plan_build(ScreenPlan& sp, const std::vector<LvDesc>& lv, int B);
-void screen_launch(Ctx* c, const ScreenPlan& sp, const LvDesc* d_lv, int B, const float* feat, const ScoreParams& thr, int* d_counts,
-                   CandRec* d_cands, int* ctl);
+void screen_launch(Ctx* c, const ScreenPlan& sp, const LvDesc* d_lv, int B, const float* feat, const uint16_t* feat_h, const ScoreParams& thr,
+                   int* d_counts, CandRec* d_cands, int* ctl);
 void screen_prepare_model(DetectorModel& d, const float* w);
diff --git a/pyannote-video_amd/csrc/pvf_internal.h b/pyannote-video_amd/csrc/pvf_internal.h
--- a/pyannote-video_amd/csrc/pvf_internal.h
+++ b/pyannote-video_amd/csrc/pvf_internal.h
@@ -232,6 +232,8 @@
     bool det_screen = true, det_screen_suspended = false, screen_attr_set = false;
     int screen_list_cap = 1 << 20;
     DevBuf s_screen;
+    DevBuf s_feat_h;
+    const void* feat_h_ring_owner = nullptr;
     int64_t screen_batches = 0, screen_listed = 0, screen_retries = 0;
     double screen_pipe_err = -1;
     bool screen_pipe_flushes_subnormals = false;
@@ -334,6 +336,7 @@
 void det_nms(const DetectorModel& m, const std::vector<RawDet>& sorted, std::vector<RawDet>& out);
 void det_pyramid_level(Ctx* c, const Frame& f, int upsample, int level, std::vector<uint8_t>* out, int* h, int* w);
 void det_level_features(Ctx* c, const Frame& f, int upsample, int level, std::vector<float>* out, int* fh, int* fw);
+void det_level_features_f16(Ctx* c, const Frame& f, int upsample, int level, std::vector<uint16_t>* out, int* fh, int* fw);
 void det_level_plan(Ctx* c, const Frame& f, int upsample, int level, int32_t out[8]);
 void det_pyramid_batch(Ctx* c, const std::vector<Frame>& frames, int upsample);
 void fhog_debug(Ctx* c, const uint8_t* himg, int h, int w, int cell, int pad_r, int pad_c, std::vector<float>& out, int* fh, int* fw);
diff --git a/pyannote-video_amd/csrc/screen.hip b/pyannote-video_amd/csrc/screen.hip
--- a/pyannote-video_amd/csrc/screen.hip
+++ b/pyannote-video_amd/csrc/screen.hip
@@ -11,13 +11,8 @@
 #define SCR_B_BYTES (10 * 12 * 64 * 16)
 #define SCR_M_STRIDE (12 * 64 * 16)
 
-__device__ __forceinline__ uint32_t pk_f16(float a, float b)
-{
-    return __builtin_bit_cast(uint32_t, __builtin_amdgcn_cvt_pkrtz(a, b));
-}
-
 template <int NG>
-__device__ __forceinline__ void screen_walk(const ScreenItem t, const LvDesc* __restrict__ lv, const float* __restrict__ feat_base,
+__device__ __forceinline__ void screen_walk(const ScreenItem t, const LvDesc* __restrict__ lv, const uint16_t* __restrict__ feath_base,
                                             const uint8_t* s_b, const float th_lane, int* __restrict__ ctl, uint2* __restrict__ list,
                                             const int list_cap, u32x4& mx)
 {
@@ -26,15 +21,14 @@
     static_assert(FC == SCR_FILTER_COLS, "detect_ml.h: SCR_FILTER_COLS is this kernel's filter width");
     const int lane = threadIdx.x & 63, i = lane & 15, kq = lane >> 4;
     const int fw = lv[t.lv].fw;
-    const long long feat_off = lv[t.lv].feat_off, feat_stride = lv[t.lv].feat_stride;
+    const long long feat_off = lv[t.lv].feath_off, feat_stride = lv[t.lv].feath_stride;
     const int fwp = lv[t.lv].fwp;
-    const float* fb = feat_base + feat_off + (size_t)t.b * feat_stride + feat_at(t.r_base, 0, t.c_base, fwp);
-    const int row_bytes = (8 * fwp - t.c_base) * 16;
+    const uint16_t* fb = feath_base + feat_off + (size_t)t.b * feat_stride + feat_h_at(t.r_base, 0, t.c_base, fwp);
+    const int row_bytes = (4 * fwp - t.c_base) * 16;
     const int fh_in = t.out_rows + FR - 1;
     const int c1 = fw - (FC - FC / 2 - 1);
-    const int voff = i * 48 + kq * 2 * fwp * 16;
-    const int voff2 = voff + fwp * 16;
-    const int voff_t = i < 3 ? voff : 0x40000000, voff2_t = i < 3 ? voff2 : 0x40000000;
+    const int voff = i * 48 + kq * fwp * 16;
+    const int voff_t = i < 3 ? voff : 0x40000000;
     f32x4 acc[10][NG];
 #pragma unroll
     for (int q = 0; q < 10; ++q)
@@ -42,19 +36,14 @@
         for (int g = 0; g < NG; ++g) acc[q][g] = (f32x4){0.f, 0.f, 0.f, 0.f};
     const uint8_t* b_lo = s_b + lane * 16;
     const uint8_t* b_hi = s_b + lane * 16 + 5 * SCR_M_STRIDE;
-    auto load_cls = [&](int row, int cls, u32x4 (&raw)[NG + 1][2]) {
-        const __amdgpu_buffer_rsrc_t rs = __builtin_amdgcn_make_buffer_rsrc((void*)(fb + (size_t)row * 8 * fwp * 4), 0,
+    auto load_cls = [&](int row, int cls, u32x4 (&raw)[NG + 1]) {
+        const __amdgpu_buffer_rsrc_t rs = __builtin_amdgcn_make_buffer_rsrc((void*)(fb + (size_t)row * 4 * fwp * 8), 0,
                                                                             row < fh_in ? row_bytes : 0, RSRC_FLAGS);
 #pragma unroll
-        for (int g = 0; g <= NG; ++g) {
-            raw[g][0] = __builtin_amdgcn_raw_buffer_load_b128(rs, (g < NG ? voff : voff_t) + cls * 16 + g * 768, 0, 0);
-            raw[g][1] = __builtin_amdgcn_raw_buffer_load_b128(rs, (g < NG ? voff2 : voff2_t) + cls * 16 + g * 768, 0, 0);
-        }
-    };
-    auto cvt_frag = [&](const u32x4 (&r)[2]) -> u32x4 {
-        u32x4 o;
-        o.x = pk_f16(__uint_as_float(r[0].x), __uint_as_float(r[0].y)); o.y = pk_f16(__uint_as_float(r[0].z), __uint_as_float(r[0].w));
-        o.z = pk_f16(__uint_as_float(r[1].x), __uint_as_float(r[1].y)); o.w = pk_f16(__uint_as_float(r[1].z), __uint_as_float(r[1].w));
+        for (int g = 0; g <= NG; ++g)
+            raw[g] = __builtin_amdgcn_raw_buffer_load_b128(rs, (g < NG ? voff : voff_t) + cls * 16 + g * 768, 0, 0);
+    };
+    auto cvt_frag = [&](const u32x4& o) -> u32x4 {
 #pragma unroll
         for (int k = 0; k < 4; ++k) mx[k] = __builtin_bit_cast(uint32_t, __builtin_elementwise_max(__builtin_bit_cast(f16x2, mx[k]), __builtin_bit_cast(f16x2, o[k])));
         return o;
@@ -96,7 +85,7 @@
 
     u32x4 A[3][NG + 1];
     {
-        u32x4 raw[NG + 1][2];
+        u32x4 raw[NG + 1];
 #pragma unroll
         for (int cls = 0; cls < 3; ++cls) {
             load_cls(0, cls, raw);
@@ -112,7 +101,7 @@
     for (int q = 0; q < 10; ++q) bn[q] = b_frag(q, 0);
     for (int s = 0; s < fh_in; ++s) {
         u32x4 An[3][NG + 1];
-        u32x4 raw[NG + 1][2];
+        u32x4 raw[NG + 1];
         f32x4 done[NG];
 #pragma unroll
         for (int j = 0; j < 12; ++j) {
@@ -154,7 +143,7 @@
 }
 
 __global__ void __launch_bounds__(256) __attribute__((amdgpu_waves_per_eu(1, 1)))
-score_screen_k(const ScreenItem* __restrict__ items, const LvDesc* __restrict__ lv, const float* __restrict__ feat_base,
+score_screen_k(const ScreenItem* __restrict__ items, const LvDesc* __restrict__ lv, const uint16_t* __restrict__ feat_base,
                const u32x4* __restrict__ Bh, ScreenParams sp, int* __restrict__ ctl, uint2* __restrict__ list)
 {
     extern __shared__ __attribute__((aligned(16))) uint8_t s_b[];
@@ -350,9 +339,11 @@
                 for (int b = 0; b < B; ++b)
                     items.push_back(ScreenItem{l, b, c0, r0, std::min(rows, out_r - r0), std::min(SCR_SG, (out_c - c0 + 47) / 48)});
     }
-    for (const ScreenItem& it : items)
+    for (const ScreenItem& it : items) {
+        PVF_REQUIRE(lv[it.lv].fwp == lv[it.lv].fw + FEAT_PAD_COLS, "screening plan: a feature row without its FEAT_PAD_COLS zero columns");
         PVF_REQUIRE(it.ng >= 1 && it.c_base + SCR_GROUP_COLS * it.ng + SCR_TAIL_CELLS - 1 < lv[it.lv].fwp,
                     "screening plan: a strip's tail read passes the FEAT_PAD_COLS zero columns of its feature row");
+    }
     std::stable_sort(items.begin(), items.end(), [](const ScreenItem& a, const ScreenItem& b) { return a.ng * (a.out_rows + 9) > b.ng * (b.out_rows + 9); });
     if (sp.d_items) (void)hipFree(sp.d_items);
     sp.d_items = nullptr;
@@ -468,9 +459,10 @@
     PVF_REQUIRE(dpp_ok, "screening: v_mov_b32_dpp row_shl:1 / row_shr:15 do not move data as the screening kernel expects on this device");
 }
 
-void screen_launch(Ctx* c, const ScreenPlan& plan, const LvDesc* d_lv, int B, const float* feat, const ScoreParams& thr, int* d_counts,
-                   CandRec* d_cands, int* ctl)
-{
+void screen_launch(Ctx* c, const ScreenPlan& plan, const LvDesc* d_lv, int B, const float* feat, const uint16_t* feat_h, const ScoreParams& thr,
+                   int* d_counts, CandRec* d_cands, int* ctl)
+{
+    PVF_REQUIRE(feat_h != nullptr, "screening: no f16 feature map (the FHOG kernel writes it while the screening pass is on)");
     const DetectorModel& m = c->det;
     if (plan.n_items == 0) return;
     if (!c->screen_attr_set) {
@@ -495,7 +487,7 @@
     c->s_screen.ensure((size_t)sp.list_cap * sizeof(uint2) + 64);
     uint2* list = c->s_screen.as<uint2>();
     const int grid = std::min(c->n_cu, (plan.n_items + 3) / 4);
-    hipLaunchKernelGGL(score_screen_k, dim3(grid), dim3(256), SCR_B_BYTES, c->det_stream, plan.d_items, d_lv, feat,
+    hipLaunchKernelGGL(score_screen_k, dim3(grid), dim3(256), SCR_B_BYTES, c->det_stream, plan.d_items, d_lv, feat_h,
                        reinterpret_cast<const u32x4*>(m.d_bscreen), sp, ctl, list);
     hipLaunchKernelGGL(score_list_k, dim3(256), dim3(256), 0, c->det_stream, list, ctl, sp.list_cap, d_lv, feat, m.d_w, thr, d_counts, d_cands);
 }
diff --git a/pyannote-video_amd/pyannote_video_amd/_lib.py b/pyannote-video_amd/pyannote_video_amd/_lib.py
--- a/pyannote-video_amd/pyannote_video_amd/_lib.py
+++ b/pyannote-video_amd/pyannote_video_amd/_lib.py
@@ -114,6 +114,7 @@
     "pvf_debug_pyramid_level": (C.c_int32, [H, H, C.c_int32, C.c_int32, P, P, P]),
     "pvf_debug_pyramid_batch": (C.c_int32, [H, P, C.c_int32, C.c_int32]),
     "pvf_debug_level_features": (C.c_int32, [H, H, C.c_int32, C.c_int32, P, P, P]),
+    "pvf_debug_level_features_f16": (C.c_int32, [H, H, C.c_int32, C.c_int32, P, P, P]),
     "pvf_debug_level_plan": (C.c_int32, [H, H, C.c_int32, C.c_int32, P]),
     "pvf_debug_fhog": (C.c_int32, [H, P, C.c_int32, C.c_int32, C.c_int32, C.c_int32, C.c_int32, P, P, P]),
     "pvf_debug_detect_raw": (C.c_int32, [H, H, C.c_int32, C.c_double, P, P, C.c_int32, P]),
diff --git a/pyannote-video_amd/pyannote_video_amd/runtime.py b/pyannote-video_amd/pyannote_video_amd/runtime.py
--- a/pyannote-video_amd/pyannote_video_amd/runtime.py
+++ b/pyannote-video_amd/pyannote_video_amd/runtime.py
@@ -531,6 +531,15 @@
         out = np.zeros((fh.value, fw.value, 32), np.float32)
         if out.size:
             check(self._l.pvf_debug_level_features(self._h, f.handle, upsample, level, ptr(out), C.byref(fh), C.byref(fw)))
+        return out
+
+    def level_features_f16(self, frame, upsample, level):
+        f = self.stage(frame)
+        fh, fw = C.c_int32(0), C.c_int32(0)
+        check(self._l.pvf_debug_level_features_f16(self._h, f.handle, upsample, level, None, C.byref(fh), C.byref(fw)))
+        out = np.zeros((fh.value, fw.value, 32), np.float16)
+        if out.size:
+            check(self._l.pvf_debug_level_features_f16(self._h, f.handle, upsample, level, ptr(out), C.byref(fh), C.byref(fw)))
         return out
 
     def level_plan(self, frame, upsample, level):
```

Result: slower. 1888 (-60.5%).
